# kubernetes-sigs/karpenter-provider-ibm-cloud

Hardware: AMD Instinct MI355X
Metric: pod×offering feasibility checks/sec + Solve latency (ms) at 100k pods, 1/2/4/8 GPU (higher is better)
Workload: dtype int64

## Files before the change

karpenter-provider-ibm-cloud_amd/csrc/batch_kernels.hip:

```cpp
#define GS_BATCH_KERNELS 1
#include <hip/hip_runtime.h>
#include <stdint.h>

#include "devutil.hpp"
#include "ffd_common.hpp"
#include "layout.hpp"

using namespace gsd;

#include "solve_kernels.hpp"
#include "queue_kernels.hpp"
#include "init_kernel.hpp"

extern "C" hipError_t gsk_init_batch(uint32_t trunc_lds_bytes) {
  return hipFuncSetAttribute((const void*)trunc_kernel_batch, hipFuncAttributeMaxDynamicSharedMemorySize,
                             (int)trunc_lds_bytes);
}

extern "C" uint32_t gsk_feas_lp(uint32_t W) {
#ifndef GS_K1_LPMAX
#define GS_K1_LPMAX 16
#endif
  if (GS_K1_LPMAX < 64 && W > GS_K1_LPMAX && W <= 32 && W * (64 / GS_K1_LPMAX) <= 256) W = GS_K1_LPMAX;
  uint32_t lp = 1;
  while (lp < W && lp < 64) lp <<= 1;
  return lp;
}

template <uint32_t LP>
static void launch_feas_batch_lp(const DevProblem* ds, uint32_t n, uint64_t max_pairs, hipStream_t s) {
  const uint64_t per_block = (BLOCK / 64) * (64 / LP);
  const uint32_t blocks = (uint32_t)((max_pairs + per_block - 1) / per_block);
  hipLaunchKernelGGL(feas_kernel_batch<LP>, dim3(blocks ? blocks : 1, n), dim3(BLOCK), 0, s, ds, 0u, 0u, ~0u);
}

extern "C" hipError_t gsk_feas_batch(const DevProblem* ds, uint32_t n, uint32_t lp, uint64_t max_cursors,
                                     uint64_t max_pairs, hipStream_t s) {
  if (!n || n > 65535) return hipErrorInvalidValue;
  const uint32_t cb = (uint32_t)((max_cursors + BLOCK - 1) / BLOCK);
  hipLaunchKernelGGL(feas_cursor_kernel_batch, dim3(cb ? cb : 1, n), dim3(BLOCK), 0, s, ds);
  switch (lp) {
    case 1: launch_feas_batch_lp<1>(ds, n, max_pairs, s); break;
    case 2: launch_feas_batch_lp<2>(ds, n, max_pairs, s); break;
    case 4: launch_feas_batch_lp<4>(ds, n, max_pairs, s); break;
    case 8: launch_feas_batch_lp<8>(ds, n, max_pairs, s); break;
    case 16: launch_feas_batch_lp<16>(ds, n, max_pairs, s); break;
    case 32: launch_feas_batch_lp<32>(ds, n, max_pairs, s); break;
    case 64: launch_feas_batch_lp<64>(ds, n, max_pairs, s); break;
    default: return hipErrorInvalidValue;
  }
  return hipGetLastError();
}

extern "C" hipError_t gsk_init_state_batch(const DevProblem* ds, uint32_t n, hipStream_t s) {
  if (!n || n > 65535) return hipErrorInvalidValue;
  hipLaunchKernelGGL(ffd_init_kernel_batch, dim3(8, n), dim3(256), 0, s, ds);
  return hipGetLastError();
}

extern "C" hipError_t gsk_queue_records_batch(const DevProblem* ds, uint32_t n, uint32_t max_pods, hipStream_t s) {
  if (!n || !max_pods) return hipSuccess;
  if (n > 65535) return hipErrorInvalidValue;
  const uint32_t blocks = (max_pods + 255) / 256;
  hipLaunchKernelGGL(queue_records_kernel_batch, dim3(blocks, n), dim3(256), 0, s, ds);
  hipLaunchKernelGGL(queue_runs_kernel_batch, dim3(blocks, n), dim3(256), 0, s, ds);
  return hipGetLastError();
}

extern "C" hipError_t gsk_trunc_batch(const DevProblem* ds, uint32_t n, uint32_t max_slots, uint32_t lds_bytes,
                                      hipStream_t s) {
  if (!n || n > 65535) return hipErrorInvalidValue;
  hipLaunchKernelGGL(trunc_kernel_batch, dim3(max_slots ? max_slots : 1, n), dim3(BLOCK), lds_bytes, s, ds, 0u, 0u);
  return hipGetLastError();
}

#define GSK_DECL(n, t)                                                                                      \
  extern "C" hipError_t gsk_ffdwb_launch_r##n##_t##t(const DevProblem* ds, uint32_t cnt, uint32_t wide, uint32_t lds, \
                                                     hipStream_t s);                                        \
  extern "C" hipError_t gsk_ffdwb_attr_r##n##_t##t(uint32_t lds_total, uint32_t* dyn_min);
#define GSK_DECL2(n) GSK_DECL(n, 0) GSK_DECL(n, 1)
GSK_DECL2(1) GSK_DECL2(2) GSK_DECL2(3) GSK_DECL2(4) GSK_DECL2(5) GSK_DECL2(6) GSK_DECL2(7) GSK_DECL2(8)
#undef GSK_DECL2
#undef GSK_DECL
static uint32_t g_ffdwb_dyn_max = 0;

extern "C" hipError_t gsk_init_ffdw_batch(uint32_t lds_total) {
  hipError_t e = hipSuccess;
  uint32_t dmin = 0;
#define GSK_ATTR(n, t) \
  if (hipError_t x = gsk_ffdwb_attr_r##n##_t##t(lds_total, &dmin); x != hipSuccess) e = x;
#define GSK_ATTR2(n) GSK_ATTR(n, 0) GSK_ATTR(n, 1)
  GSK_ATTR2(1) GSK_ATTR2(2) GSK_ATTR2(3) GSK_ATTR2(4) GSK_ATTR2(5) GSK_ATTR2(6) GSK_ATTR2(7) GSK_ATTR2(8)
#undef GSK_ATTR2
#undef GSK_ATTR
  g_ffdwb_dyn_max = dmin;
  return e;
}

extern "C" uint32_t gsk_ffdw_batch_dyn_lds_max(void) { return g_ffdwb_dyn_max; }

extern "C" hipError_t gsk_ffdw_batch(const DevProblem* ds, uint32_t n, uint32_t R, uint32_t topo, uint32_t wide,
                                     uint32_t lds, hipStream_t s) {
  if (!n || lds > g_ffdwb_dyn_max) return hipErrorInvalidConfiguration;
  switch (R * 2 + (topo ? 1 : 0)) {
#define GSK_CASE(k)                                                    \
  case 2 * k: return gsk_ffdwb_launch_r##k##_t0(ds, n, wide, lds, s); \
  case 2 * k + 1: return gsk_ffdwb_launch_r##k##_t1(ds, n, wide, lds, s);
    GSK_CASE(1) GSK_CASE(2) GSK_CASE(3) GSK_CASE(4) GSK_CASE(5) GSK_CASE(6) GSK_CASE(7) GSK_CASE(8)
#undef GSK_CASE
    default:
      return hipErrorInvalidValue;
  }
}


extern "C" __global__ __launch_bounds__(256) void sim_begin_kernel_batch(const DevProblem* __restrict__ ds,
                                                                         const uint32_t* __restrict__ blocks,
                                                                         uint32_t clear_overlays) {
  const DevProblem& d = ds[blockIdx.y];
  if (blockIdx.x == 0 && threadIdx.x == 0) *d.sim_next = 0;
  if (!clear_overlays) return;
  const size_t cells = (size_t)blocks[blockIdx.y] * d.ov_cap * (d.TGH ? d.TGH : 1u);
  for (size_t i = (size_t)blockIdx.x * 256 + threadIdx.x; i < cells; i += (size_t)gridDim.x * 256) d.ov_hn[i] = 0;
}

extern "C" hipError_t gsk_sim_begin_batch(const DevProblem* ds, const uint32_t* blocks, uint32_t n, uint32_t clear_overlays,
                                          hipStream_t s) {
  if (!n || n > 65535) return hipErrorInvalidValue;
  hipLaunchKernelGGL(sim_begin_kernel_batch, dim3(clear_overlays ? 8 : 1, n), dim3(256), 0, s, ds, blocks, clear_overlays);
  return hipGetLastError();
}

extern "C" hipError_t gsk_trunc_sims_batch(const DevProblem* ds, uint32_t n, uint32_t mv, uint32_t max_sims,
                                           uint32_t max_slots, uint32_t lds_bytes, hipStream_t s) {
  if (!n || n > 65535) return hipErrorInvalidValue;
  if (mv) {
    hipLaunchKernelGGL(trunc_kernel_batch, dim3(max_slots ? max_slots : 1, n), dim3(BLOCK), lds_bytes, s, ds, 1u, 0u);
    hipLaunchKernelGGL(sim_fix_kernel_batch, dim3((max_sims + BLOCK - 1) / BLOCK ? (max_sims + BLOCK - 1) / BLOCK : 1, n),
                       dim3(BLOCK), 0, s, ds);
  } else {
    hipLaunchKernelGGL(trunc_kernel_batch, dim3(max_sims ? max_sims : 1, n), dim3(BLOCK), lds_bytes, s, ds, 0u, 0u);
  }
  return hipGetLastError();
}

#define GSK_DECL(n, t)                                                                                                  \
  extern "C" hipError_t gsk_ffdsb_launch_r##n##_t##t(const DevProblem* ds, const uint32_t* blocks, uint32_t cnt,        \
                                                     uint32_t max_blocks, uint32_t nt, uint32_t lds, uint32_t ov_epoch, \
// ... 156 lines not shown
```

karpenter-provider-ibm-cloud_amd/csrc/capi.cpp:

```cpp
#include "ctx.hpp"

#include <set>

namespace gsc {

gs_status fail(gs_ctx* c, gs_status s, const std::string& m) {
  c->err = m;
  return s;
}

void upload_problem(gs_ctx* c, const SimPlan* sims, bool records) {
  auto& e = c->enc;
  auto& d = c->dp;
  c->plan.clear();
  c->plan_bytes = 0;
  c->free_all();
  std::memset(&d, 0, sizeof d);
  d.N = e.N;
  d.W = e.W;
  d.R = e.R;
  d.Z = e.Z;
  d.C = e.C;
  d.T = e.T;
  d.F = e.F;
  d.V = e.V;
  d.P = e.P;
  d.K = e.K;
  d.NT = e.NT;
  d.wk_slots = e.wk_slots;
  d.RQ = std::min<uint32_t>(e.R, 4);
  d.n_thr = (uint32_t)e.thr_val.size();
  if (sims) {
    d.max_claims = std::max<uint32_t>(sims->max_pods, 1);
  } else {
    const uint32_t other = gsk_ffd_lds_bytes(0, (uint32_t)e.thr_val.size(), 0, gsd::topo_lds_bytes(e.TGZ, e.ZS, e.TGH, e.n_lazy)) + 8;
    const uint32_t dyn = std::min(gsk_ffd_dyn_lds_max(), gsk_ffdw_dyn_lds_max());
    auto claims_fit = [&](uint32_t extra) {
      const uint32_t fit = dyn > other + extra ? (dyn - other - extra) / 23 : 0;
      return std::min<uint32_t>(std::min<uint32_t>(std::max<uint32_t>(e.P, 1), kMaxClaimsLds), fit);
    };
    d.max_claims = claims_fit(0);
    if (!d.max_claims) throw HipError{"topology / threshold state leaves no LDS for NodeClaims"};
    const bool wave_ok = !(c->cfg_flags & GS_CFG_BLOCK_SOLVE) && e.NN <= kWaveSolveMaxNodes;
    d.max_claims_wave = wave_ok ? claims_fit(gsd::wave_node_lds_bytes(e.NN)) : 0u;
    c->wave = d.max_claims_wave > 0;
  }
  c->upload(d.it_vid, e.it_vid);
  c->upload(d.it_dvid, e.it_dvid);
  d.it_key_unique = e.it_key_unique;
  d.any_mv = e.any_mv ? 1u : 0u;
  d.any_vol = e.any_vol ? 1u : 0u;
  c->upload(d.n_vol0, e.n_vol);
  c->alloc(d.n_vol, e.n_vol.size());
  c->upload(d.pod_vol, e.pod_vol);
  c->upload(d.pod_vfresh, e.pod_vfresh);
  c->upload(d.it_alloc, e.it_alloc);
  c->upload(d.it_cap, e.it_cap);
  c->upload(d.it_pair, e.it_pair);
  c->upload(d.it_prank, e.it_prank);
  c->upload(d.it_namerank, e.it_namerank);
  c->upload(d.rank_to_it, e.rank_to_it);
  c->upload(d.slot_set, e.slot_set);
  {
    std::vector<int64_t> tv = e.thr_val;
    tv.insert(tv.end(), 4, INT64_MAX);
    c->upload(d.thr_val, std::move(tv));
  }
  c->upload(d.thr_off, e.thr_off);
  {
    const uint32_t OW = std::max<uint32_t>(4, (e.W + 3) & ~3u);
    const size_t nrows = e.W ? e.thr_set.size() / e.W : 0;
    std::vector<uint64_t> ts(std::max<size_t>(nrows, 1) * OW, 0);
    for (size_t q = 0; q < nrows; q++)
      std::copy(e.thr_set.begin() + q * e.W, e.thr_set.begin() + (q + 1) * e.W, ts.begin() + q * OW);
    c->upload(d.thr_set, std::move(ts));
  }
  c->upload(d.fk_ival, e.fk_ival);
  c->upload(d.fk_isint, e.fk_isint);
  c->upload(d.tmpl, e.tmpl);
  c->upload(d.t_opts, e.t_opts);
  c->upload(d.t_limopts, e.t_limopts);
  c->upload(d.t_fk, e.t_fk);
  c->upload(d.pod_req, e.pod_req);
  c->upload(d.var_begin, e.var_begin);
  c->upload(d.var_count, e.var_count);
  c->upload(d.vars, e.vars);
  c->upload(d.itmask, e.itmask);
  c->upload(d.var_itclass, e.var_itclass);
  {
    std::vector<uint32_t> vp(std::max<uint32_t>(e.V, 1), 0);
    for (uint32_t v = 0; v < e.V; v++) vp[v] = e.vars[v].pod;
    c->upload(d.var_pod, std::move(vp));
  }
  c->upload(d.itclass_mask, e.itclass_mask);
  c->upload(d.fk_entries, e.fk_entries);
  c->upload(d.queue0, e.queue0);
  if (!sims) {
    c->alloc(d.qvars, std::max<uint32_t>(e.P, 1));
    c->alloc(d.qreqs, (size_t)std::max<uint32_t>(e.P, 1) * std::max<uint32_t>(e.R, 1));
    c->alloc(d.qcodes, (size_t)std::max<uint32_t>(e.P, 1) * 4);
    c->alloc(d.qrun, std::max<uint32_t>(e.P, 1));
  }
  d.NN = e.NN;
  d.TG = e.TG;
  d.TGH = e.TGH;
  d.TGZ = e.TGZ;
  d.ZS = e.ZS;
  d.NZV = e.NZV;
  d.dom_ct = e.dom_ct ? 1u : 0u;
  d.dom_np = e.dom_np ? 1u : 0u;
  d.zknown0 = e.zknown0;
  c->upload(d.tgroups, e.tgroups);
  c->upload(d.tg_list, e.tg_list);
  d.n_lazy = e.n_lazy;
  c->upload(d.lazy_slot, e.lazy_slot);
  c->upload(d.var_lz_off, e.var_lz_off);
  c->upload(d.lz_idx, e.lz_idx);
  c->upload(d.lz_mind, e.lz_mind);
  c->upload(d.zcnt0, e.zcnt0);
  c->upload(d.htot0, e.htot0);
  c->upload(d.zone_order, e.zone_order);
  c->upload(d.zone_cat, e.zone_cat);
  c->upload(d.hn0, e.hn0);
  if (sims && (e.TGH || e.TGZ) && e.NN) {
    std::vector<uint32_t> off(e.NN + 1, 0);
    for (uint32_t g = 0; g < e.TGZ; g++)
      for (uint32_t n = 0; n < e.NN; n++) off[n + 1] += e.zn_cnt[(size_t)g * e.NN + n] != 0;
    for (uint32_t g = 0; g < e.TGH; g++)
      for (uint32_t n = 0; n < e.NN; n++) off[n + 1] += e.hn0[(size_t)g * e.NN + n] != 0;
    for (uint32_t n = 0; n < e.NN; n++) off[n + 1] += off[n];
    std::vector<uint64_t> sp(std::max<uint32_t>(off[e.NN], 1));
    std::vector<uint32_t> fill(off.begin(), off.end() - 1);
    auto put = [&](uint32_t g, int32_t c, uint32_t n) { sp[fill[n]++] = (uint64_t)g << 32 | (uint32_t)c; };
    for (uint32_t g = 0; g < e.TGZ; g++)
      for (uint32_t n = 0; n < e.NN; n++)
        if (int32_t c = e.zn_cnt[(size_t)g * e.NN + n]) put(g, c, n);
    for (uint32_t g = 0; g < e.TGH; g++)
      for (uint32_t n = 0; n < e.NN; n++)
        if (int32_t c = e.hn0[(size_t)g * e.NN + n]) put(e.TGZ + g, c, n);
    c->upload(d.nsp_off, std::move(off));
    c->upload(d.nsp, std::move(sp));
  } else {
    d.nsp_off = nullptr;
    d.nsp = nullptr;
  }
  c->alloc(d.hn, e.hn0.size());
  c->upload(d.nodes0, e.nodes);
  c->upload(d.n_fk0, e.n_fk);
  c->alloc(d.nodes, sims ? 1 : std::max<uint32_t>(e.NN, 1));
  c->alloc(d.n_fk, sims ? 1 : e.n_fk.size());
  const size_t VT = (size_t)e.V * e.T, F1 = std::max<uint32_t>(e.F, 1), R1 = std::max<uint32_t>(e.R, 1);
  const size_t PA = sims ? sims->pods.size() : e.P;
  const size_t CA = sims ? sims->pods.size() : d.max_claims;
  const size_t NS = sims ? sims->evaluated.size() : 0;
  d.claim_cap = (uint32_t)CA;
  c->ch = false;
  d.OW = std::max<uint32_t>(4, (e.W + 3) & ~3u);
  c->alloc(d.rows, VT * d.OW);
  c->alloc(d.cheapest, VT);
  c->alloc(d.cheapest_key, VT);
  c->alloc(d.nfo, VT);
  c->alloc(d.fk_ok, VT);
  c->alloc(d.pair_cur, VT * R1);
  c->alloc(d.queue, PA);
  c->alloc(d.last_len, PA);
  c->alloc(d.last_epoch, PA);
  c->alloc(d.cur_var, PA);
  c->alloc(d.c_rec, CA);
  c->alloc(d.c_opts, CA * d.OW);
  c->alloc(d.c_fk, CA * F1);
  c->alloc(d.t_rem, (sims ? NS : 1) * e.T * R1);
  c->alloc(d.log, PA);
  c->alloc(d.c_sorted, sims ? 1 : CA);
  c->alloc(d.ctrl, 1);
  c->alloc(d.c_its, (sims ? NS : CA) * 60);
  c->alloc(d.c_nits, sims ? NS : CA);
  c->hc_bytes = 0;
  if (sims) {
    c->alloc_zero(d.hc, (size_t)std::max<uint32_t>(e.TGH, 1) * CA);
    c->hc_bytes = (size_t)std::max<uint32_t>(e.TGH, 1) * CA * sizeof(int32_t);
  } else {
    c->alloc(d.hc, (size_t)std::max<uint32_t>(e.TGH, 1) * CA);
  }
  if (sims) {
// ... 734 lines not shown
```

karpenter-provider-ibm-cloud_amd/csrc/ffd.hip:

```cpp
#include "ffd_block.hpp"

extern "C" uint32_t gsk_ffd_lds_bytes(uint32_t max_claims, uint32_t nthr, uint32_t nb_words,
                                      uint32_t topo_bytes) {
  const uint32_t thr = nthr + 4;
  const uint32_t base = (((23u * max_claims + 7u) & ~7u) + thr * 8u + nb_words * 4u + 7u) & ~7u;
  return base + topo_bytes;
}

static uint32_t g_ffd_dyn_max = 0;

template <uint32_t RR, bool SIM, bool TOPO = false, uint32_t NT = SIM ? FB_SIM : FB_MAX>
static hipError_t ffd_attr(uint32_t lds_total) {
  hipFuncAttributes a;
  hipError_t e = hipFuncGetAttributes(&a, (const void*)ffd_kernel<RR, SIM, NT, TOPO>);
  if (e != hipSuccess) return e;
  const uint32_t dyn = lds_total > a.sharedSizeBytes ? lds_total - (uint32_t)a.sharedSizeBytes : 0;
  if (!g_ffd_dyn_max || dyn < g_ffd_dyn_max) g_ffd_dyn_max = dyn;
  return hipFuncSetAttribute((const void*)ffd_kernel<RR, SIM, NT, TOPO>, hipFuncAttributeMaxDynamicSharedMemorySize,
                             (int)dyn);
}

template <uint32_t RR>
static hipError_t ffd_attr_all(uint32_t lds_total) {
  hipError_t e = hipSuccess;
  for (hipError_t x : {ffd_attr<RR, false>(lds_total), ffd_attr<RR, false, true>(lds_total), ffd_attr<RR, true>(lds_total),
                       ffd_attr<RR, true, false, FB_SIM_NARROW>(lds_total), ffd_attr<RR, true, true, FB_SIM>(lds_total),
                       ffd_attr<RR, true, true, FB_SIM_NARROW>(lds_total)})
    if (x != hipSuccess) e = x;
  return e;
}

extern "C" hipError_t gsk_init_ffd(uint32_t lds_total) {
  hipError_t e = hipSuccess;
  for (hipError_t x : {ffd_attr_all<1>(lds_total), ffd_attr_all<2>(lds_total), ffd_attr_all<3>(lds_total),
                       ffd_attr_all<4>(lds_total), ffd_attr_all<5>(lds_total), ffd_attr_all<6>(lds_total),
                       ffd_attr_all<7>(lds_total), ffd_attr_all<8>(lds_total)})
    if (x != hipSuccess) e = x;
  return e;
}

extern "C" uint32_t gsk_ffd_dyn_lds_max(void) { return g_ffd_dyn_max; }

template <uint32_t RR>
static hipError_t sim_occ(int* n, bool narrow, bool general, uint32_t lds) {
  if (general)
    return narrow ? hipOccupancyMaxActiveBlocksPerMultiprocessor(n, (const void*)ffd_kernel<RR, true, FB_SIM_NARROW, true>,
                                                                 FB_SIM_NARROW, lds)
                  : hipOccupancyMaxActiveBlocksPerMultiprocessor(n, (const void*)ffd_kernel<RR, true, FB_SIM, true>, FB_SIM, lds);
  return narrow ? hipOccupancyMaxActiveBlocksPerMultiprocessor(n, (const void*)ffd_kernel<RR, true, FB_SIM_NARROW, false>,
                                                               FB_SIM_NARROW, lds)
                : hipOccupancyMaxActiveBlocksPerMultiprocessor(n, (const void*)ffd_kernel<RR, true, FB_SIM, false>, FB_SIM, lds);
}

extern "C" uint32_t gsk_ffd_sim_blocks_per_cu(uint32_t R, uint32_t lds, uint32_t nt, uint32_t general) {
  int n = 0;
  hipError_t e = hipErrorInvalidValue;
  const bool narrow = nt == (uint32_t)FB_SIM_NARROW;
  switch (R) {
#define GSK_OCC(k) \
  case k: e = sim_occ<k>(&n, narrow, general != 0, lds); break;
    GSK_OCC(1) GSK_OCC(2) GSK_OCC(3) GSK_OCC(4) GSK_OCC(5) GSK_OCC(6) GSK_OCC(7) GSK_OCC(8)
#undef GSK_OCC
  }
  return e == hipSuccess && n > 0 ? (uint32_t)n : 1u;
}

extern "C" hipError_t gsk_ffd(const DevProblem* d, uint32_t blocks, hipStream_t s) {
  const uint32_t lds = gsk_ffd_lds_bytes(d->max_claims, d->n_thr, d->nb_words, topo_lds_bytes(d->TGZ, d->ZS, d->TGH, d->n_lazy)) +
                       (d->n_sims ? 8u * d->ovh_slots + (d->sim_lds ? 32u * d->max_claims : 0u) : 0u);
  if (lds > g_ffd_dyn_max) return hipErrorInvalidConfiguration;
  const bool sim = d->n_sims > 0;
  if (sim && d->sim_nt != (uint32_t)FB_SIM && d->sim_nt != (uint32_t)FB_SIM_NARROW) return hipErrorInvalidValue;
  const bool general = d->TG || d->any_mv || d->any_vol;
  const uint32_t shape = sim ? (d->sim_nt == (uint32_t)FB_SIM_NARROW ? 3u : 2u) + (general ? 2u : 0u) : (general ? 1u : 0u);
  switch (d->R * 8 + shape) {
#define GSK_CASE(n)                                                                                          \
  case 8 * n: hipLaunchKernelGGL((ffd_kernel<n, false, FB_MAX, false>), dim3(1), dim3(FB_MAX), lds, s, *d); break; \
  case 8 * n + 1: hipLaunchKernelGGL((ffd_kernel<n, false, FB_MAX, true>), dim3(1), dim3(FB_MAX), lds, s, *d); break; \
  case 8 * n + 2: hipLaunchKernelGGL((ffd_kernel<n, true, FB_SIM, false>), dim3(blocks), dim3(FB_SIM), lds, s, *d); break; \
  case 8 * n + 3:                                                                                            \
    hipLaunchKernelGGL((ffd_kernel<n, true, FB_SIM_NARROW, false>), dim3(blocks), dim3(FB_SIM_NARROW), lds, s, *d); \
    break;                                                                                                    \
  case 8 * n + 4: hipLaunchKernelGGL((ffd_kernel<n, true, FB_SIM, true>), dim3(blocks), dim3(FB_SIM), lds, s, *d); break; \
  case 8 * n + 5:                                                                                            \
    hipLaunchKernelGGL((ffd_kernel<n, true, FB_SIM_NARROW, true>), dim3(blocks), dim3(FB_SIM_NARROW), lds, s, *d); \
    break;
    GSK_CASE(1) GSK_CASE(2) GSK_CASE(3) GSK_CASE(4) GSK_CASE(5) GSK_CASE(6) GSK_CASE(7) GSK_CASE(8)
#undef GSK_CASE
    default:
      return hipErrorInvalidValue;
  }
  return hipGetLastError();
}

#include "queue_kernels.hpp"

extern "C" hipError_t gsk_queue_records(const DevProblem* d, hipStream_t s) {
  if (!d->P) return hipSuccess;
  hipLaunchKernelGGL(queue_records_kernel, dim3((d->P + 255) / 256), dim3(256), 0, s, *d);
  hipLaunchKernelGGL(queue_runs_kernel, dim3((d->P + 255) / 256), dim3(256), 0, s, *d);
  return hipGetLastError();
}
```

karpenter-provider-ibm-cloud_amd/csrc/ffd_common.hpp:

```cpp
#pragma once
#include <hip/hip_runtime.h>
#include <stdint.h>

#include "devutil.hpp"
#include "layout.hpp"

namespace gsd {
namespace {

struct Frame {
  int a, b, limit;
  int wb, wp;
  int uni;
};

typedef __attribute__((address_space(3))) uint32_t lds_u32;
typedef __attribute__((address_space(3))) uint16_t lds_u16;
typedef __attribute__((address_space(3))) Frame lds_frame;

__device__ __forceinline__ int bits_len(uint64_t x) { return x ? 64 - __clzll((long long)x) : 0; }

struct SplitAcc {
  uint16_t* sc;
  uint16_t* ord;
  __device__ __forceinline__ uint32_t key(int i) const { return sc[i]; }
  __device__ __forceinline__ void swap(int i, int j) const {
    uint16_t a = sc[i];
    sc[i] = sc[j];
    sc[j] = a;
    a = ord[i];
    ord[i] = ord[j];
    ord[j] = a;
  }
};
template <class U32>
struct PackedAccT {
  U32* so;
  __device__ __forceinline__ uint32_t key(int i) const { return so[i] & 0xFFFFu; }
  __device__ __forceinline__ void swap(int i, int j) const {
    const uint32_t a = so[i];
    so[i] = so[j];
    so[j] = a;
  }
};
using PackedAcc = PackedAccT<lds_u32>;

template <class Acc>
struct SeqSortT {
  Acc acc;
  __device__ bool less(int i, int j) const { return acc.key(i) < acc.key(j); }
  __device__ void swap(int i, int j) const { acc.swap(i, j); }
  __device__ void insertion_sort(int a, int b) const {
    for (int i = a + 1; i < b; i++)
      for (int j = i; j > a && less(j, j - 1); j--) swap(j, j - 1);
  }
  __device__ void sift_down(int lo, int hi, int first) const {
    int root = lo;
    for (;;) {
      int child = 2 * root + 1;
      if (child >= hi) return;
      if (child + 1 < hi && less(first + child, first + child + 1)) child++;
      if (!less(first + root, first + child)) return;
      swap(first + root, first + child);
      root = child;
    }
  }
  __device__ void heap_sort(int a, int b) const {
    int first = a, lo = 0, hi = b - a;
    for (int i = (hi - 1) / 2; i >= 0; i--) sift_down(i, hi, first);
    for (int i = hi - 1; i >= 0; i--) {
      swap(first, first + i);
      sift_down(lo, i, first);
    }
  }
  __device__ int partition(int a, int b, int pivot, bool* already) const {
    swap(a, pivot);
    int i = a + 1, j = b - 1;
    while (i <= j && less(i, a)) i++;
    while (i <= j && !less(j, a)) j--;
    if (i > j) {
      swap(j, a);
      *already = true;
      return j;
    }
    swap(i, j);
    i++;
    j--;
    for (;;) {
// ... 114 lines not shown
      j = median(i, j, k, &swaps);
    }
    *hint = swaps == 0 ? 1 : (swaps == 12 ? 2 : 0);
    return j;
  }
  __device__ void reverse_range(int a, int b) const {
    int i = a, j = b - 1;
    while (i < j) {
      swap(i, j);
      i++;
      j--;
    }
  }
  __device__ void pdq_frame(Frame f0) const {
    Frame st[32];
    int sp = 0;
    st[sp++] = f0;
    while (sp > 0) {
      Frame f = st[--sp];
      for (;;) {
        int length = f.b - f.a;
        if (length <= 12) {
          insertion_sort(f.a, f.b);
          break;
        }
        if (f.limit == 0) {
          heap_sort(f.a, f.b);
          break;
        }
        if (!f.wb) {
          break_patterns(f.a, f.b);
          f.limit--;
        }
        int hint;
        int pivot = choose_pivot(f.a, f.b, &hint);
        if (hint == 2) {
          reverse_range(f.a, f.b);
          pivot = (f.b - 1) - (pivot - f.a);
          hint = 1;
        }
        if (f.wb && f.wp && hint == 1) {
          if (partial_insertion_sort(f.a, f.b)) break;
        }
        if (f.a > 0 && !less(f.a - 1, pivot)) {
          f.a = partition_equal(f.a, f.b, pivot);
          continue;
        }
        bool already;
        int mid = partition(f.a, f.b, pivot, &already);
        f.wp = already;
        int leftLen = mid - f.a, rightLen = f.b - mid;
        int bal = length / 8;
        Frame child;
        if (leftLen < rightLen) {
          f.wb = leftLen >= bal;
          child = Frame{f.a, mid, f.limit, 1, 1};
          f.a = mid + 1;
        } else {
          f.wb = rightLen >= bal;
          child = Frame{mid + 1, f.b, f.limit, 1, 1};
          f.b = mid;
        }
        st[sp++] = f;
        f = child;
      }
    }
  }
};

__device__ __forceinline__ void wsync() {
  __builtin_amdgcn_fence(__ATOMIC_ACQ_REL, "wavefront");
  __builtin_amdgcn_wave_barrier();
}
template <bool G>
__device__ __forceinline__ void wsyncT() {
  if (G) __builtin_amdgcn_s_waitcnt(0);
  wsync();
}

__device__ __forceinline__ uint32_t rlane(uint32_t x, uint32_t i) {
  return (uint32_t)__builtin_amdgcn_readlane((int)x, (int)i);
}

__device__ __forceinline__ uint32_t ffs64(uint64_t m) { return (uint32_t)__ffsll((long long)m) - 1u; }


__device__ __forceinline__ uint32_t wlane(uint32_t v, int i, uint32_t x) {
  return (int)(threadIdx.x & 63u) == i ? x : v;
}
__device__ __forceinline__ uint32_t nth_bit(uint64_t m, uint32_t r) {
  uint32_t pos = 0;
#pragma unroll
  for (int w = 32; w >= 1; w >>= 1) {
    const uint32_t c = (uint32_t)__popcll(m & ((1ull << w) - 1ull));
    const bool up = r >= c;
    r = up ? r - c : r;
    m = up ? m >> w : m;
    pos += up ? (uint32_t)w : 0u;
  }
  return pos;
}
template <class U32, bool G>
struct PackedArr {
  U32* so;
  __device__ __forceinline__ uint32_t load(int i) const { return (uint32_t)so[i]; }
  __device__ __forceinline__ void store(int i, uint32_t v) const { so[i] = v; }
  __device__ __forceinline__ void heap_sort(int a, int b) const { SeqSortT<PackedAccT<U32>>{{so}}.heap_sort(a, b); }
  __device__ __forceinline__ void sync() const { wsyncT<G>(); }
};
template <class Arr>
struct RegSort {
  uint32_t v;
  uint32_t lane;
  int g;
  uint32_t prevk;

  __device__ __forceinline__ uint32_t key(int i) const { return rlane(v, (uint32_t)i) & 0xFFFFu; }
  __device__ __forceinline__ void swap(int i, int j) {
    const uint32_t x = rlane(v, (uint32_t)i), y = rlane(v, (uint32_t)j);
    v = wlane(v, i, y);
    v = wlane(v, j, x);
  }
  __device__ void insertion_sort(int a, int b) {
    const uint32_t k = v & 0xFFFFu;
    int r = a;
    for (int j = a; j < b; j++) {
      const uint32_t kj = key(j);
      r += (kj < k || (kj == k && j < (int)lane)) ? 1 : 0;
    }
    const bool in = (int)lane >= a && (int)lane < b;
    v = (uint32_t)__builtin_amdgcn_ds_permute((in ? r : (int)lane) * 4, (int)v);
  }
  __device__ void swap_misplaced(uint64_t lm, uint64_t rm) {
    const uint64_t me = 1ull << lane;
    const uint64_t below = me - 1ull;
    uint32_t partner = lane;
    if (lm & me) {
      const uint32_t r = (uint32_t)__popcll(lm & below);
      partner = nth_bit(rm, (uint32_t)__popcll(rm) - 1u - r);
    } else if (rm & me) {
      const uint32_t r = (uint32_t)__popcll(rm & ~below & ~me);
      partner = nth_bit(lm, r);
    }
    v = (uint32_t)__shfl((int)v, (int)partner);
  }
  __device__ int partition(int a, int b, int pivot, bool* already) {
    swap(a, pivot);
    const uint32_t p = key(a), k = v & 0xFFFFu;
    const bool inr = (int)lane > a && (int)lane < b;
    const bool lt = k < p;
    const int mid = a + (int)__popcll(__ballot(inr && lt));
    const bool inl = (int)lane > a && (int)lane <= mid;
    const uint64_t lm = __ballot(inl && !lt), rm = __ballot(inr && !inl && lt);
    if (lm) swap_misplaced(lm, rm);
    swap(mid, a);
    *already = lm == 0;
    return mid;
  }
  __device__ int partition_equal(int a, int b, int pivot) {
    swap(a, pivot);
    const uint32_t p = key(a), k = v & 0xFFFFu;
    const bool inr = (int)lane > a && (int)lane < b;
    const bool le = k <= p;
    const int mid = a + (int)__popcll(__ballot(inr && le));
    const bool inl = (int)lane > a && (int)lane <= mid;
    const uint64_t lm = __ballot(inl && !le), rm = __ballot(inr && !inl && le);
    if (lm) swap_misplaced(lm, rm);
    return mid + 1;
  }
  __device__ void reverse_range(int a, int b) {
    const bool in = (int)lane >= a && (int)lane < b;
    v = (uint32_t)__shfl((int)v, in ? a + b - 1 - (int)lane : (int)lane);
  }
  __device__ void rotate_up(int lo, int hi) {
    const uint32_t x = rlane(v, (uint32_t)hi);
    const bool in = (int)lane > lo && (int)lane <= hi;
    const uint32_t y = (uint32_t)__shfl((int)v, in ? (int)lane - 1 : (int)lane);
    v = (int)lane == lo ? x : y;
  }
  __device__ void rotate_down(int lo, int hi) {
    const uint32_t x = rlane(v, (uint32_t)lo);
    const bool in = (int)lane >= lo && (int)lane < hi;
    const uint32_t y = (uint32_t)__shfl((int)v, in ? (int)lane + 1 : (int)lane);
    v = (int)lane == hi ? x : y;
  }
  __device__ bool partial_insertion_sort(int a, int b) {
    int i = a + 1;
    for (int j = 0; j < 5; j++) {
      const uint32_t k = v & 0xFFFFu;
      const uint32_t pk = (uint32_t)__shfl((int)v, (int)lane - 1) & 0xFFFFu;
      const uint64_t inv = __ballot((int)lane >= i && (int)lane < b && k < pk);
      if (!inv) return true;
      i = (int)ffs64(inv);
      if (b - a < 50) return false;
      swap(i, i - 1);
      if (i - a >= 2) {
        const uint32_t x = key(i - 1);
        const uint64_t hm = __ballot((int)lane <= i - 2 && (v & 0xFFFFu) <= x);
        const int q = hm ? 63 - (int)__clzll((long long)hm) : -1;
        rotate_up(q + 1, i - 1);
      }
      if (b - i >= 2) {
        const uint32_t y = key(i);
        const uint64_t em = __ballot((int)lane > i && (int)lane < b && (v & 0xFFFFu) >= y);
        const int e = em ? (int)ffs64(em) : b;
        rotate_down(i, e - 1);
      }
    }
    return false;
  }
  __device__ void break_patterns(int a, int b) {
    const int length = b - a;
    if (length >= 8) {
      uint64_t r = (uint64_t)length;
      const uint64_t modulus = 1ull << bits_len((uint64_t)length);
      const int idx = a + (length / 4) * 2 - 1;
      for (int i = 0; i < 3; i++) {
        r ^= r << 13;
        r ^= r >> 7;
        r ^= r << 17;
        int other = (int)(r & (modulus - 1));
        if (other >= length) other -= length;
        swap(idx - 1 + i, a + other);
      }
    }
  }
  __device__ int choose_pivot(int a, int b, int* hint) const {
    const int l = b - a;
    int swaps = 0;
    int i = a + l / 4 * 1, j = a + l / 4 * 2, k = a + l / 4 * 3;
    auto med = [&](int x, int y, int z) {
      if (key(y) < key(x)) { swaps++; const int t = x; x = y; y = t; }
      if (key(z) < key(y)) { swaps++; const int t = y; y = z; z = t; }
      if (key(y) < key(x)) { swaps++; const int t = x; x = y; y = t; }
      return y;
    };
    if (l >= 8) {
      if (l >= 50) {
        i = med(i - 1, i, i + 1);
        j = med(j - 1, j, j + 1);
        k = med(k - 1, k, k + 1);
      }
      j = med(i, j, k);
    }
    *hint = swaps == 0 ? 1 : (swaps == 12 ? 2 : 0);
    return j;
  }
  __device__ void heap_sort(const Arr& arr, int a, int b) {
    if ((int)lane < b && (int)lane >= a) arr.store(g + (int)lane, v);
    arr.sync();
    if (lane == 0) arr.heap_sort(g + a, g + b);
    arr.sync();
    if ((int)lane < b && (int)lane >= a) v = arr.load(g + (int)lane);
    arr.sync();
  }
  __device__ void run(const Arr& arr, Frame f) {
    int a = f.a - g, b = f.b - g, limit = f.limit, wb = f.wb, wp = f.wp;
    uint32_t stk = 0;
    int sp = 0;
    for (;;) {
      for (;;) {
        a = __builtin_amdgcn_readfirstlane(a);
        b = __builtin_amdgcn_readfirstlane(b);
        limit = __builtin_amdgcn_readfirstlane(limit);
        wb = __builtin_amdgcn_readfirstlane(wb);
        wp = __builtin_amdgcn_readfirstlane(wp);
        const int length = b - a;
        if (length <= 12) {
          insertion_sort(a, b);
          break;
        }
        if (limit == 0) {
          heap_sort(arr, a, b);
          break;
        }
        if (!wb) {
          break_patterns(a, b);
          limit--;
        }
        int hint;
        int pivot = choose_pivot(a, b, &hint);
        if (hint == 2) {
          reverse_range(a, b);
          pivot = (b - 1) - (pivot - a);
          hint = 1;
        }
        if (wb && wp && hint == 1 && partial_insertion_sort(a, b)) break;
// ... 31 lines not shown
      const uint32_t e = rlane(stk, (uint32_t)sp);
      a = (int)(e & 0xFFu);
      b = (int)((e >> 8) & 0xFFu);
      limit = (int)((e >> 16) & 0xFFu);
      wb = (int)((e >> 24) & 1u);
      wp = (int)((e >> 25) & 1u);
    }
  }
};
template <class Arr>
__device__ __noinline__ void reg_pdq_frame(Arr arr, int fa, int fb, int limit, int wb, int wp) {
  fa = __builtin_amdgcn_readfirstlane(fa);
  fb = __builtin_amdgcn_readfirstlane(fb);
  limit = __builtin_amdgcn_readfirstlane(limit);
  wb = __builtin_amdgcn_readfirstlane(wb);
  wp = __builtin_amdgcn_readfirstlane(wp);
  const uint32_t lane = threadIdx.x & 63u;
  const int n = fb - fa;
  const uint32_t prevk = fa > 0 ? (uint32_t)__builtin_amdgcn_readfirstlane((int)arr.load(fa - 1)) & 0xFFFFu : 0u;
  RegSort<Arr> r{(int)lane < n ? arr.load(fa + (int)lane) : 0u, lane, fa, prevk};
  r.run(arr, Frame{fa, fb, limit, wb, wp, 0});
  if ((int)lane < n) arr.store(fa + (int)lane, r.v);
  arr.sync();
}

using SeqSort = SeqSortT<SplitAcc>;
using SeqSortP = SeqSortT<PackedAcc>;
using SeqSortPG = SeqSortT<PackedAccT<uint32_t>>;

__device__ __forceinline__ uint32_t thr_window(const int64_t* thr, uint32_t n, uint32_t m0, int64_t x) {
  uint32_t m = m0;
#pragma unroll
  for (uint32_t k = 0; k < 4; k++) {
    const int64_t vk = thr[m0 + k];
    m += (m0 + k < n && vk < x) ? 1u : 0u;
  }
  return m;
}

__device__ __forceinline__ uint32_t thr_search(const int64_t* thr, uint32_t n, uint32_t lo, int64_t x) {
  uint32_t hi = n;
  while (lo < hi) {
    const uint32_t mid = (lo + hi) >> 1;
    if (thr[mid] < x) lo = mid + 1;
    else hi = mid;
  }
  return lo;
}

template <class Acc>
__device__ __forceinline__ int pivot_hint_wave(const Acc& acc, int l, uint32_t lane) {
  const int i0 = l / 4 * 1, j0 = l / 4 * 2, k0 = l / 4 * 3;
  const int idx[9] = {i0 - 1, i0, i0 + 1, j0 - 1, j0, j0 + 1, k0 - 1, k0, k0 + 1};
  int mine = 0;
#pragma unroll
  for (int t = 0; t < 9; t++)
    if ((int)lane == t) mine = idx[t];
  const uint32_t kl = lane < 9 && (l >= 50 || lane % 3 == 1) ? acc.key(mine) : 0u;
  uint32_t key[9];
#pragma unroll
  for (int t = 0; t < 9; t++) key[t] = __builtin_amdgcn_readlane(kl, t);
  int swaps = 0;
  auto med = [&](uint32_t kx, uint32_t ky, uint32_t kz) {
    if (ky < kx) { swaps++; const uint32_t u = kx; kx = ky; ky = u; }
    if (kz < ky) { swaps++; const uint32_t u = ky; ky = kz; kz = u; }
    if (ky < kx) { swaps++; const uint32_t u = kx; kx = ky; ky = u; }
    return ky;
  };
  uint32_t ki = key[1], kj = key[4], kk = key[7];
  if (l >= 50) {
    ki = med(key[0], key[1], key[2]);
    kj = med(key[3], key[4], key[5]);
    kk = med(key[6], key[7], key[8]);
  }
  med(ki, kj, kk);
  return swaps == 0 ? 1 : (swaps == 12 ? 2 : 0);
}

template <class Pred>
__device__ __forceinline__ uint32_t wave_first(uint32_t lo, uint32_t hi, uint32_t lane, Pred pred) {
  while (hi - lo > 64) {
    const uint32_t step = (hi - lo + 63) / 64;
    const uint32_t k = lo + lane * step + step - 1;
    const uint64_t b = __ballot(k >= hi || pred(k));
    if (!b) return hi;
    const uint32_t i = (uint32_t)__ffsll((long long)b) - 1;
    lo = lo + i * step;
    hi = lo + step < hi ? lo + step : hi;
  }
  const uint32_t k = lo + lane;
  const uint64_t b = __ballot(k < hi && pred(k));
  return b ? lo + (uint32_t)__ffsll((long long)b) - 1 : hi;
}

__device__ __forceinline__ uint64_t phase_clock() {
#ifdef GS_FFD_PHASES
  return wall_clock64();
#else
  return 0;
#endif
}

typedef const __attribute__((address_space(4))) DevProblem* KArg;

__device__ __forceinline__ int64_t uniform_i64(int64_t x) {
  const uint32_t lo = __builtin_amdgcn_readfirstlane((uint32_t)x);
  const uint32_t hi = __builtin_amdgcn_readfirstlane((uint32_t)((uint64_t)x >> 32));
  return (int64_t)(((uint64_t)hi << 32) | lo);
}

__device__ __forceinline__ uint32_t qcode_floor(int64_t v) {
  if (v <= 0) return 0;
  const uint64_t x = (uint64_t)v;
  const uint32_t b = 64u - (uint32_t)__clzll((long long)x);
  if (b <= 10) return (uint32_t)x;
  const uint32_t s = b - 10;
  return 1024u + (s - 1) * 512u + (uint32_t)((x >> s) - 512u);
}
__device__ __forceinline__ uint32_t qcode_ceil(int64_t v) {
  if (v <= 0) return 0;
  const uint64_t x = (uint64_t)v;
  const uint32_t b = 64u - (uint32_t)__clzll((long long)x);
  if (b <= 10) return (uint32_t)x;
  const uint32_t s = b - 10;
  const uint32_t c = 1024u + (s - 1) * 512u + (uint32_t)((x >> s) - 512u);
  return c + ((x & ((1ull << s) - 1)) ? 1u : 0u);
}

__device__ __forceinline__ int64_t qcode_value(uint32_t c) {
  if (c < 1024u) return (int64_t)c;
  const uint32_t s = (c - 1024u) / 512u + 1u, m = (c - 1024u) % 512u + 512u;
  return (int64_t)((uint64_t)m << s);
}

__device__ __forceinline__ uint64_t pack_room(const int64_t* thr, const uint32_t* thoff, const uint32_t* cur,
                                              const int64_t* tot, uint32_t RQ) {
  uint64_t s = 0;
#pragma unroll
  for (uint32_t r = 0; r < 4; r++) {
    if (r >= RQ) break;
    const uint32_t o = thoff[r], n = thoff[r + 1] - o;
    const int64_t room = cur[r] < n ? thr[o + cur[r]] - tot[r] : 0;
    s |= (uint64_t)qcode_floor(room) << (16 * r);
  }
  return s;
}

template <class DP>
__device__ __forceinline__ uint64_t pack_slack(const DP& d, const int64_t* maxa, const int64_t* tot) {
  uint64_t s = 0;
#pragma unroll
  for (uint32_t r = 0; r < 4; r++) {
    if (r >= d.RQ) break;
    s |= (uint64_t)qcode_ceil(maxa[r] - tot[r]) << (16 * r);
  }
  return s;
}

template <class DP, class WordFn>
__device__ inline bool mv_ok(const DP& d, const TmplRec& tr, WordFn word) {
  for (uint32_t mm = tr.mv_mask; mm; mm &= mm - 1) {
    const uint32_t k = (uint32_t)__builtin_ctz(mm);
    const uint32_t need = tr.mv[k];
    uint32_t n = 0;
    if ((d.it_key_unique >> k) & 1) {
      for (uint32_t w = 0; w < d.W && n < need; w++) n += (uint32_t)__popcll(word(w));
    } else {
      const uint16_t* dv = d.it_dvid + (size_t)k * d.N;
      uint64_t s0 = 0, s1 = 0, s2 = 0, s3 = 0;
      for (uint32_t w = 0; w < d.W && n < need; w++)
        for (uint64_t m = word(w); m && n < need; m &= m - 1) {
          const uint32_t x = dv[w * 64 + (uint32_t)__builtin_ctzll(m)];
          const uint32_t q = x >> 6;
          const uint64_t bit = 1ull << (x & 63);
          const uint64_t cur = q == 0 ? s0 : q == 1 ? s1 : q == 2 ? s2 : s3;
          if (!(cur & bit)) {
            n++;
            s0 |= q == 0 ? bit : 0;
            s1 |= q == 1 ? bit : 0;
            s2 |= q == 2 ? bit : 0;
            s3 |= q == 3 ? bit : 0;
          }
        }
    }
    if (n < need) return false;
  }
  return true;
}

struct TopoS {
  uint64_t* known;
  int64_t* tmin;
  int32_t* zcnt;
  int32_t* htot;
  uint64_t* lazy;
  int32_t* lmind;
};
__device__ __forceinline__ TopoS topo_lds(char* base, uint32_t tgz, uint32_t zs, uint32_t tgh, uint32_t nl) {
  TopoS t;
  t.known = (uint64_t*)base;
  t.tmin = (int64_t*)(base + tgz * 8u);
  t.zcnt = (int32_t*)(base + tgz * 8u + (uint32_t)OWNMAX * 8u);
  t.htot = (int32_t*)(base + tgz * 8u + (uint32_t)OWNMAX * 8u + tgz * zs * 4u);
  t.lazy = (uint64_t*)(base + topo_lazy_off(tgz, zs, tgh));
  t.lmind = (int32_t*)(base + topo_lazy_off(tgz, zs, tgh) + ((nl + 63u) / 64u) * 8u);
  return t;
}

template <class DP>
__device__ __forceinline__ void topo_init(const DP& d, const TopoS& ts, uint64_t known0, uint32_t i, uint32_t stride) {
  for (uint32_t k = i; k < d.TGZ * d.ZS; k += stride) ts.zcnt[k] = d.zcnt0[k];
  for (uint32_t k = i; k < d.TGZ; k += stride) ts.known[k] = known0;
  for (uint32_t k = i; k < d.TGH; k += stride) ts.htot[k] = d.htot0[k];
  for (uint32_t k = i; k < (d.n_lazy + 63u) / 64u; k += stride) ts.lazy[k] = 0;
}
// ... 189 lines not shown
```

karpenter-provider-ibm-cloud_amd/csrc/ffd_wave.hpp:

```cpp
#pragma once
#include <hip/hip_runtime.h>
#include <stdint.h>

#include <type_traits>

#include "devutil.hpp"
#include "ffd_common.hpp"
#include "layout.hpp"

using namespace gsd;

namespace {

constexpr uint32_t VR_DW = sizeof(VarRec) / 4;
static_assert(VR_DW == 32, "VarRec is one dword per lane of a half wave");
static_assert(offsetof(VarRec, fk_begin) == 4 && offsetof(VarRec, fk_count) == 8 && offsetof(VarRec, ctb) == 12 &&
                  offsetof(VarRec, itmask_off) == 16 && offsetof(VarRec, zfull_off) == 48 &&
                  offsetof(VarRec, cfull_off) == 52 && offsetof(VarRec, zm) == 56 && offsetof(VarRec, cm) == 64 &&
                  offsetof(VarRec, tol) == 72 && offsetof(VarRec, tolt) == 80 && offsetof(VarRec, own_off) == 88 &&
                  offsetof(VarRec, own_n) == 92 && offsetof(VarRec, sel_off) == 96 && offsetof(VarRec, sel_n) == 100 &&
                  offsetof(VarRec, zs) == 104 && offsetof(VarRec, zn) == 112 &&
                  offsetof(VarRec, zflags) == 120 && offsetof(VarRec, vix) == 124,
              "VarRec dword map used by ffdw_kernel");
static_assert(offsetof(ClaimRec, maxa) == 128, "ClaimRec maxa after two 64-B lines");

constexpr uint32_t WREG = 4;
#ifndef GS_RING
#define GS_RING 16
#endif
constexpr uint32_t RING = GS_RING;
constexpr uint32_t RING_DW = 53;
constexpr uint32_t RING_CODES = 48;
constexpr uint32_t RING_QRUN = 52;
constexpr uint32_t WQ = 32;
constexpr uint32_t WQ_DW = 16;
enum : uint32_t { WQ_LOG = 1, WQ_FA = 2, WQ_STOP = 3, WQ_NFA = 4 };
constexpr uint32_t SPIN_MAX = 1u << 26;
constexpr uint64_t SWAR_HI = 0x8000800080008000ull;
enum : uint32_t { MOD_NONE = 0, MOD_INC = 1, MOD_APPEND = 2 };
#ifndef GS_WAVE_SEQ
#define GS_WAVE_SEQ 32
#endif

#if defined(GS_FFD_TL) && defined(GS_CAT_SEG)
#define TLW(k)                                         \
  do {                                                 \
    const uint64_t t_ = __builtin_amdgcn_s_memtime();  \
    ptl[k] += t_ - tl_last;                            \
    tl_last = t_;                                      \
  } while (0)
#elif defined(GS_FFD_TL)
#define TLW(k)                                         \
  do {                                                 \
    const uint64_t t_ = __builtin_amdgcn_s_memtime();  \
    tl[k] += t_ - tl_last;                             \
    tl_last = t_;                                      \
  } while (0)
#else
#define TLW(k) \
  do {         \
  } while (0)
#endif

typedef __attribute__((address_space(3))) uint32_t lds_u32;
__device__ __forceinline__ uint32_t vld(const uint32_t* p) { return *(const volatile lds_u32*)(const lds_u32*)p; }
__device__ __forceinline__ void vst(uint32_t* p, uint32_t x) { *(volatile lds_u32*)(lds_u32*)p = x; }

#ifdef GS_WAVE_BATCH
__device__ __forceinline__ KArg karg() {
  const uint64_t ds = *(const __attribute__((address_space(4))) uint64_t*)__builtin_amdgcn_kernarg_segment_ptr();
  KArg p = (KArg)(ds + (uint64_t)__builtin_amdgcn_readfirstlane(blockIdx.x) * sizeof(DevProblem));
  asm volatile("" : "+s"(p));
  return p;
}
#else
__device__ __forceinline__ KArg karg() {
  KArg p = (KArg)__builtin_amdgcn_kernarg_segment_ptr();
  asm volatile("" : "+s"(p));
  return p;
}
#endif
__device__ __forceinline__ uint32_t fresh(uint32_t x) {
  asm volatile("" : "+v"(x));
  return x;
}

__device__ __forceinline__ uint64_t shfl_u64(uint64_t x, uint32_t src) {
  const uint32_t lo = (uint32_t)__shfl((int)(uint32_t)x, (int)src), hi = (uint32_t)__shfl((int)(uint32_t)(x >> 32), (int)src);
  return ((uint64_t)hi << 32) | lo;
}
__device__ __forceinline__ uint64_t wave_max_u64(uint64_t x) {
  for (int m = 32; m >= 1; m >>= 1) {
    const uint64_t y = shfl_xor_u64(x, m);
    x = y > x ? y : x;
  }
  return x;
}

__device__ __forceinline__ bool swar_ge(uint64_t a, uint64_t b) {
  return (((a | SWAR_HI) - b) & SWAR_HI) == SWAR_HI;
}
__device__ __forceinline__ uint64_t swar_max(uint64_t a, uint64_t b) {
  const uint64_t m = ((((a | SWAR_HI) - b) & SWAR_HI) >> 15) * 0xFFFFull;
  return (a & m) | (b & ~m);
}
__device__ __forceinline__ uint64_t wave_swar_max(uint64_t x) {
  for (int m = 32; m >= 1; m >>= 1) x = swar_max(x, shfl_xor_u64(x, m));
  return x;
}

__device__ __forceinline__ uint32_t dpp_max_step(uint32_t x, uint32_t y) { return x > y ? x : y; }
__device__ __forceinline__ uint32_t wave_max_dpp(uint32_t x) {
  x = dpp_max_step(x, (uint32_t)__builtin_amdgcn_update_dpp(0, (int)x, 0x111, 0xF, 0xF, true));
  x = dpp_max_step(x, (uint32_t)__builtin_amdgcn_update_dpp(0, (int)x, 0x112, 0xF, 0xF, true));
  x = dpp_max_step(x, (uint32_t)__builtin_amdgcn_update_dpp(0, (int)x, 0x114, 0xF, 0xF, true));
  x = dpp_max_step(x, (uint32_t)__builtin_amdgcn_update_dpp(0, (int)x, 0x118, 0xF, 0xF, true));
  x = dpp_max_step(x, (uint32_t)__builtin_amdgcn_update_dpp(0, (int)x, 0x142, 0xA, 0xF, false));
  x = dpp_max_step(x, (uint32_t)__builtin_amdgcn_update_dpp(0, (int)x, 0x143, 0xC, 0xF, false));
  return rlane(x, 63u);
}

struct KnownPart {
  int mid;
  int flags;
};
template <class U32, bool G>
__device__ __noinline__ KnownPart known_partition(U32* so, int n, int pivot, int x) {
  n = __builtin_amdgcn_readfirstlane(n);
  pivot = __builtin_amdgcn_readfirstlane(pivot);
  x = __builtin_amdgcn_readfirstlane(x);
  const uint32_t lane = threadIdx.x & 63u;
  auto key = [&](int i) { return (uint32_t)so[i] & 0xFFFFu; };
  auto swap = [&](int i, int j) {
    const uint32_t a = so[i];
    so[i] = so[j];
    so[j] = a;
  };
  bool already_, luni_, runi_;
  bool* already = &already_;
  bool* luni = &luni_;
  bool* runi = &runi_;
  if (lane == 0) swap(0, pivot);
  wsyncT<G>();
  const uint32_t p = key(0);
  const int e0 = x >= 1 && x < n ? x : -1;
  const int e1 = pivot != x && pivot >= 1 && pivot < n ? pivot : -1;
  auto in_e = [&](int k) { return k == e0 || k == e1; };
  auto skip_e = [&](int k) {
    k += in_e(k) ? 1 : 0;
    k += in_e(k) ? 1 : 0;
    return k;
  };
  const int step = (n - 1 + 63) / 64;
  const int q = skip_e(1 + (int)lane * step);
  const bool qv = 1 + (int)lane * step < n && q < n;
  const uint64_t m1 = __ballot(qv && key(qv ? q : 0) >= p);
  int lo, hi;
  if (m1) {
    const int l = (int)ffs64(m1);
    lo = l == 0 ? 1 : (int)rlane((uint32_t)q, (uint32_t)(l - 1)) + 1;
    hi = (int)rlane((uint32_t)q, (uint32_t)l);
  } else {
    const int lv = 63 - (int)__clzll((long long)__ballot(qv));
    lo = (int)rlane((uint32_t)q, (uint32_t)lv) + 1;
    hi = n;
  }
  int t = hi;
  for (int base = lo; base < hi; base += 64) {
    const int k = base + (int)lane;
    const bool ok = k < hi && k < n && !in_e(k);
    const uint64_t m2 = __ballot(ok && key(ok ? k : 0) >= p);
    if (m2) {
      t = base + (int)ffs64(m2);
      break;
    }
  }
  const uint32_t k0 = e0 >= 0 ? key(e0) : 0u, k1 = e1 >= 0 ? key(e1) : 0u;
  const int e_lt = (e0 >= 0 && k0 < p ? 1 : 0) + (e1 >= 0 && k1 < p ? 1 : 0);
  const int e_before_t = (e0 >= 1 && e0 < t ? 1 : 0) + (e1 >= 1 && e1 < t ? 1 : 0);
  const int mid = (t - 1) - e_before_t + e_lt;
  {
    auto prev_out = [&](int k) {
      k -= in_e(k) ? 1 : 0;
      k -= in_e(k) ? 1 : 0;
      return k;
    };
    uint32_t amin = 0xFFFFu, amax = 0, bmin = 0xFFFFu, bmax = 0;
    const int f1 = skip_e(1), l1 = prev_out(t - 1);
    if (f1 < t && l1 >= 1 && f1 <= l1) {
      amin = key(f1);
      amax = key(l1);
    }
    const int l2 = prev_out(n - 1);
    if (t < n && l2 >= t) {
      bmin = key(t);
      bmax = key(l2);
    }
    if (e0 >= 0) {
      if (k0 < p) {
        amin = k0 < amin ? k0 : amin;
        amax = k0 > amax ? k0 : amax;
      } else {
        bmin = k0 < bmin ? k0 : bmin;
        bmax = k0 > bmax ? k0 : bmax;
      }
    }
    if (e1 >= 0) {
      if (k1 < p) {
        amin = k1 < amin ? k1 : amin;
        amax = k1 > amax ? k1 : amax;
      } else {
        bmin = k1 < bmin ? k1 : bmin;
        bmax = k1 > bmax ? k1 : bmax;
      }
    }
    *luni = amin >= amax;
    *runi = bmin >= bmax;
  }
  int pos = -1;
  bool left = false, right = false;
  if (lane < 4) {
    pos = t + (int)lane;
    left = pos <= mid && pos < n && !in_e(pos);
  } else if (lane < 8) {
    pos = mid + 1 + (int)(lane - 4);
    right = pos < t && pos < n && !in_e(pos);
  } else if (lane == 8 || lane == 9) {
    pos = lane == 8 ? e0 : e1;
    if (pos >= 1) {
      const uint32_t ke = lane == 8 ? k0 : k1;
      left = pos <= mid && ke >= p;
      right = pos > mid && ke < p;
    }
  }
  const uint64_t lm = __ballot(left), rm = __ballot(right);
  const uint32_t s = (uint32_t)__popcll(lm);
  if (s) {
    const uint64_t fl = lm | rm;
    int r = 0;
    for (uint64_t mm = fl; mm; mm &= mm - 1) {
      const uint32_t j = ffs64(mm);
      const int pj = (int)rlane((uint32_t)pos, j);
      const bool lj = (lm >> j) & 1ull;
      r += (left && lj && pj < pos) || (right && !lj && pj > pos) ? 1 : 0;
    }
    int partner = (int)lane;
    for (uint64_t mm = fl; mm; mm &= mm - 1) {
      const uint32_t j = ffs64(mm);
      const int rj = (int)rlane((uint32_t)r, j);
      const bool lj = (lm >> j) & 1ull;
      if (((left && !lj) || (right && lj)) && rj == r) partner = (int)j;
    }
    const uint32_t wv = (left || right) ? (uint32_t)so[pos] : 0u;
    const uint32_t pv = (uint32_t)__shfl((int)wv, partner);
    wsyncT<G>();
    if (left || right) so[pos] = pv;
    wsyncT<G>();
  }
  if (lane == 0) swap(mid, 0);
  wsyncT<G>();
  *already = s == 0;
  return KnownPart{mid, (already_ ? 1 : 0) | (luni_ ? 2 : 0) | (runi_ ? 4 : 0)};
}

template <int SEQ, class U32 = lds_u32, class U16 = lds_u16, bool G = false, bool KNOWN = false>
struct WaveSort {
  static_assert(SEQ >= 12, "ranges <= 12 must reach Go's insertion sort");
  U32* so;
  U16* scr;
  lds_frame* stk;
  uint32_t lane, half;

  __device__ __forceinline__ uint32_t key(int i) const { return so[i] & 0xFFFFu; }
  __device__ __forceinline__ void swap(int i, int j) const {
    const uint32_t a = so[i];
    so[i] = so[j];
    so[j] = a;
  }
#ifndef GS_SORT_RW
#define GS_SORT_RW 4
#endif
  static constexpr int RW = GS_SORT_RW;
  template <class Pred>
  __device__ uint32_t count(int lo, int hi, Pred pred) const {
    uint32_t c = 0;
    for (int base = lo; base < hi; base += 64 * RW) {
      bool in[RW];
#pragma unroll
      for (int u = 0; u < RW; u++) {
        const int k = base + u * 64 + (int)lane;
        in[u] = k < hi && pred(k);
      }
#pragma unroll
      for (int u = 0; u < RW; u++) c += (uint32_t)__popcll(__ballot(in[u]));
    }
    return c;
  }
  template <class Pred>
  __device__ uint32_t compact(int lo, int hi, bool desc, U16* out, Pred pred) const {
    uint32_t total = 0;
    const int n = hi - lo;
    for (int base = 0; base < n; base += 64 * RW) {
      bool in[RW];
#pragma unroll
      for (int u = 0; u < RW; u++) {
        const int idx = base + u * 64 + (int)lane;
        in[u] = idx < n && pred(desc ? hi - 1 - idx : lo + idx);
      }
#pragma unroll
      for (int u = 0; u < RW; u++) {
        const int idx = base + u * 64 + (int)lane;
        const uint64_t m = __ballot(in[u]);
        if (in[u]) out[total + (uint32_t)__popcll(m & ((1ull << lane) - 1ull))] = (uint16_t)(desc ? hi - 1 - idx : lo + idx);
        total += (uint32_t)__popcll(m);
      }
    }
    wsyncT<G>();
    return total;
  }
  __device__ void swap_lists(uint32_t s) const {
    for (uint32_t k = lane; k < s; k += 64) {
      const int x = scr[k], y = scr[half + k];
      const uint32_t a = so[x], b = so[y];
      wsyncT<G>();
      so[x] = b;
      so[y] = a;
    }
    wsyncT<G>();
  }
  template <bool LE>
  __device__ uint32_t count_split(int lo, int hi, uint32_t p, bool* lo_uni, bool* hi_uni, uint64_t* mk) const {
    constexpr int RC = 2 * RW;
    uint32_t c = 0, amax = 0, anot = 0, bmax = 0, bnot = 0;
    uint64_t mine = 0;
    for (int base = lo; base < hi; base += 64 * RC) {
      uint32_t kk[RC];
#pragma unroll
      for (int u = 0; u < RC; u++) {
        const int k = base + u * 64 + (int)lane;
        kk[u] = key(k < hi ? k : hi - 1);
      }
#pragma unroll
      for (int u = 0; u < RC; u++) {
        const int k = base + u * 64 + (int)lane;
        const bool valid = k < hi;
        const bool in = valid && (LE ? kk[u] <= p : kk[u] < p);
        const bool out = valid && !in;
        const uint64_t bi = __ballot(in);
        c += (uint32_t)__popcll(bi);
        mine = lane == (uint32_t)((base - lo) / 64 + u) ? bi : mine;
        const uint32_t nk = 0xFFFFu - kk[u];
        amax = in && kk[u] > amax ? kk[u] : amax;
        anot = in && nk > anot ? nk : anot;
        bmax = out && kk[u] > bmax ? kk[u] : bmax;
        bnot = out && nk > bnot ? nk : bnot;
      }
    }
    *mk = mine;
    amax = wave_max_dpp(amax);
    anot = wave_max_dpp(anot);
    bmax = wave_max_dpp(bmax);
    bnot = wave_max_dpp(bnot);
    *lo_uni = c == 0 || amax == 0xFFFFu - anot;
    *hi_uni = c == (uint32_t)(hi - lo) || bmax == 0xFFFFu - bnot;
    return c;
  }
  static constexpr int MASK_MAX = 64 * 64;
  __device__ uint32_t lists_from_masks(int lo, uint32_t nl, uint32_t n, uint64_t mk) const {
    const uint32_t x0 = lane * 64u;
    const uint64_t valid = x0 >= n ? 0ull : (n - x0 >= 64u ? ~0ull : ((1ull << (n - x0)) - 1ull));
    const uint64_t left = x0 >= nl ? 0ull : (nl - x0 >= 64u ? ~0ull : ((1ull << (nl - x0)) - 1ull));
    const uint64_t lm = ~mk & left & valid, rm = mk & ~left & valid;
    const uint32_t lc = (uint32_t)__popcll(lm), rc = (uint32_t)__popcll(rm);
    uint32_t x = lc | rc << 16;
    x += (uint32_t)__builtin_amdgcn_update_dpp(0, (int)x, 0x111, 0xF, 0xF, true);
    x += (uint32_t)__builtin_amdgcn_update_dpp(0, (int)x, 0x112, 0xF, 0xF, true);
    x += (uint32_t)__builtin_amdgcn_update_dpp(0, (int)x, 0x114, 0xF, 0xF, true);
    x += (uint32_t)__builtin_amdgcn_update_dpp(0, (int)x, 0x118, 0xF, 0xF, true);
    x += (uint32_t)__builtin_amdgcn_update_dpp(0, (int)x, 0x142, 0xA, 0xF, false);
    x += (uint32_t)__builtin_amdgcn_update_dpp(0, (int)x, 0x143, 0xC, 0xF, false);
    const uint32_t tot = rlane(x, 63u);
    const uint32_t lpre = x & 0xFFFFu;
    const uint32_t rsuf = (tot >> 16) - (x >> 16) + rc;
    const uint32_t total = tot & 0xFFFFu;
    uint32_t k = lpre - lc;
    for (uint64_t m = lm; m; m &= m - 1) scr[k++] = (uint16_t)(lo + (int)(x0 + ffs64(m)));
    k = rsuf - rc;
    for (uint64_t m = rm; m;) {
      const uint32_t bit = 63u - (uint32_t)__clzll((long long)m);
      scr[half + k++] = (uint16_t)(lo + (int)(x0 + bit));
      m &= ~(1ull << bit);
    }
    wsyncT<G>();
    return total;
  }
#ifdef GS_SORT_TL2
#define PTL(k)                                                                  \
  do {                                                                          \
    const uint64_t n_ = __builtin_amdgcn_s_memtime();                           \
    if (lane == 0 && stl) stl[8 + (k)] += n_ - p_last;                          \
    p_last = n_;                                                                \
  } while (0)
#else
#define PTL(k) \
  do {         \
  } while (0)
#endif
  __device__ int partition(int a, int b, int pivot, bool* already, bool* luni, bool* runi) const {
#ifdef GS_SORT_TL2
    uint64_t p_last = __builtin_amdgcn_s_memtime();
#endif
    if (lane == 0) swap(a, pivot);
    wsyncT<G>();
    const uint32_t p = key(a);
    PTL(0);
    uint64_t mk;
    const int mid = a + (int)count_split<false>(a + 1, b, p, luni, runi, &mk);
    PTL(1);
    uint32_t s;
    if (b - a - 1 <= MASK_MAX) {
      s = lists_from_masks(a + 1, (uint32_t)(mid - a), (uint32_t)(b - a - 1), mk);
    } else {
      s = compact(a + 1, mid + 1, false, scr, [&](int k) { return key(k) >= p; });
      compact(mid + 1, b, true, scr + half, [&](int k) { return key(k) < p; });
    }
    PTL(2);
    swap_lists(s);
    if (lane == 0) swap(mid, a);
    wsyncT<G>();
    PTL(3);
    *already = s == 0;
    return mid;
  }
  __device__ int partition_known(int n, int pivot, int x, bool* already, bool* luni, bool* runi) const;
  __device__ int partition_equal(int a, int b, int pivot, bool* runi) const {
    if (lane == 0) swap(a, pivot);
    wsyncT<G>();
    const uint32_t p = key(a);
    bool luni;
    uint64_t mk;
    const int mid = a + (int)count_split<true>(a + 1, b, p, &luni, runi, &mk);
    uint32_t s;
    if (b - a - 1 <= MASK_MAX) {
      s = lists_from_masks(a + 1, (uint32_t)(mid - a), (uint32_t)(b - a - 1), mk);
    } else {
      s = compact(a + 1, mid + 1, false, scr, [&](int k) { return key(k) > p; });
      compact(mid + 1, b, true, scr + half, [&](int k) { return key(k) <= p; });
    }
    swap_lists(s);
    return mid + 1;
  }
  __device__ void rotate(int lo, int hi, bool left) const {
    if (hi <= lo) return;
    const uint32_t x = so[left ? lo : hi];
    wsyncT<G>();
    constexpr int RU = 4;
    if (left) {
      for (int base = lo; base < hi; base += 64 * RU) {
        uint32_t v[RU];
#pragma unroll
        for (int u = 0; u < RU; u++) {
          const int k = base + u * 64 + (int)lane;
          v[u] = k < hi ? so[k + 1] : 0u;
        }
        wsyncT<G>();
#pragma unroll
        for (int u = 0; u < RU; u++) {
          const int k = base + u * 64 + (int)lane;
          if (k < hi) so[k] = v[u];
        }
        wsyncT<G>();
      }
      if (lane == 0) so[hi] = x;
    } else {
      for (int top = hi - 1; top >= lo; top -= 64 * RU) {
        uint32_t v[RU];
#pragma unroll
        for (int u = 0; u < RU; u++) {
          const int k = top - u * 64 - (int)lane;
          v[u] = k >= lo ? so[k] : 0u;
        }
        wsyncT<G>();
#pragma unroll
        for (int u = 0; u < RU; u++) {
          const int k = top - u * 64 - (int)lane;
          if (k >= lo) so[k + 1] = v[u];
        }
        wsyncT<G>();
      }
      if (lane == 0) so[lo] = x;
    }
    wsyncT<G>();
  }
  __device__ int first_inversion(int from, int b) const {
    for (int base = from; base < b; base += 64 * RW) {
      bool hit[RW];
      uint32_t kc[RW], kp[RW];
#pragma unroll
      for (int u = 0; u < RW; u++) {
        const int k = base + u * 64 + (int)lane, kk = k < b ? k : b - 1;
        kc[u] = key(kk);
        kp[u] = key(kk - 1);
      }
#pragma unroll
      for (int u = 0; u < RW; u++) hit[u] = base + u * 64 + (int)lane < b && kc[u] < kp[u];
#pragma unroll
      for (int u = 0; u < RW; u++) {
        const uint64_t m = __ballot(hit[u]);
        if (m) return base + u * 64 + (int)ffs64(m);
      }
    }
    return b;
  }
  __device__ bool partial_insertion_sort(int a, int b) const {
    int i = a + 1;
    for (int j = 0; j < 5; j++) {
      i = first_inversion(i, b);
      if (i == b) return true;
      if (b - a < 50) return false;
      if (lane == 0) swap(i, i - 1);
      wsyncT<G>();
      if (i - a >= 2) {
        const uint32_t x = key(i - 1);
        int q = -1;
        for (int top = i - 2; top >= 0; top -= 64) {
          const int k = top - (int)lane;
          const uint64_t m = __ballot(k >= 0 && key(k) <= x);
          if (m) {
            q = top - (int)ffs64(m);
            break;
          }
        }
        rotate(q + 1, i - 1, false);
      }
      if (b - i >= 2) {
        const uint32_t y = key(i);
        int q = b;
        for (int base = i + 1; base < b; base += 64) {
          const int k = base + (int)lane;
          const uint64_t m = __ballot(k < b && key(k) >= y);
          if (m) {
            q = base + (int)ffs64(m);
            break;
          }
        }
        rotate(i, q - 1, true);
      }
    }
    return false;
  }
  __device__ void reverse_range(int a, int b) const {
    const int n = (b - a) / 2;
    for (int k = (int)lane; k < n; k += 64) {
      const uint32_t x = so[a + k], y = so[b - 1 - k];
      wsyncT<G>();
      so[a + k] = y;
      so[b - 1 - k] = x;
    }
    wsyncT<G>();
  }
#ifdef GS_SORT_TL
  uint64_t* stl = nullptr;
#define STL(k)                                                     \
  do {                                                             \
    const uint64_t now_ = __builtin_amdgcn_s_memtime();            \
    if (lane == 0 && stl) stl[k] += now_ - t_last_;                \
    t_last_ = now_;                                                \
  } while (0)
#else
#define STL(k) \
  do {         \
  } while (0)
#endif
  __device__ __forceinline__ void pdqsort_body(int n, int x = -1) const {
#ifdef GS_SORT_TL
    uint64_t t_last_ = __builtin_amdgcn_s_memtime();
#endif
    const SeqSortT<PackedAccT<U32>> seq{{so}};
    if (n <= 64) {
      reg_pdq_frame(PackedArr<U32, G>{so}, 0, n, bits_len((uint64_t)n), 1, 1);
      return;
    }
    int sp = 0;
    uint32_t stk_ab = 0, stk_fl = 0;
    Frame f{0, n, bits_len((uint64_t)n), 1, 1};
    bool pristine = KNOWN && x >= 0;
    for (;;) {
      for (;;) {
        f.a = __builtin_amdgcn_readfirstlane(f.a);
        f.b = __builtin_amdgcn_readfirstlane(f.b);
        f.limit = __builtin_amdgcn_readfirstlane(f.limit);
        f.wb = __builtin_amdgcn_readfirstlane(f.wb);
        f.wp = __builtin_amdgcn_readfirstlane(f.wp);
        f.uni = __builtin_amdgcn_readfirstlane(f.uni);
        const int length = f.b - f.a;
        STL(6);
        if (length <= 64) {
          reg_pdq_frame(PackedArr<U32, G>{so}, f.a, f.b, f.limit, f.wb, f.wp);
          STL(0);
          break;
        }
        if (f.limit == 0) {
          if (lane == 0) seq.heap_sort(f.a, f.b);
          wsyncT<G>();
          STL(0);
          break;
        }
        if (!f.wb) {
          if (lane == 0) seq.break_patterns(f.a, f.b);
          wsyncT<G>();
          f.limit--;
          STL(0);
        }
        if (f.uni) {
          const int pivot = f.a + length / 4 * 2;
          if (f.wb && f.wp) break;
          const bool eq = f.a > 0 && !(key(f.a - 1) < key(pivot));
          if (lane == 0) swap(f.a, pivot);
          wsyncT<G>();
          if (eq) {
            f.a = f.b;
            STL(1);
            continue;
// ... 165 lines not shown
  const uint32_t nd_off = (tg_off + topo_lds_bytes(d.TGZ, d.ZS, d.TGH, d.n_lazy) + 7u) & ~7u;
  uint64_t* s_nslk = (uint64_t*)((char*)lds64 + nd_off);
  uint64_t* s_nrm = (uint64_t*)((char*)lds64 + nd_off + d.NN * 8u);
  uint8_t* s_nflag = (uint8_t*)((char*)lds64 + nd_off + d.NN * 16u);
  const int64_t* thr = s_thr;
  const uint64_t* slot = s_slot;

  for (uint32_t i = tid; i < nthr + 4; i += 128) s_thr[i] = i < nthr ? d.thr_val[i] : INT64_MAX;
  for (uint32_t i = tid; i < d.Z * d.C * W; i += 128) s_slot[i] = d.slot_set[i];
  if (tid <= R) s_thoff[tid] = d.thr_off[tid];
  for (uint32_t t = tid; t < T; t += 128) {
    s_tzm[t] = d.tmpl[t].zm;
    s_tcm[t] = d.tmpl[t].cm;
  }
  if (TOPO) topo_init(d, ts, d.zknown0, tid, 128);
  for (uint32_t n = tid; n < d.NN; n += 128) {
    const NodeRec& nr = d.nodes0[n];
    int64_t sl[RR];
#pragma unroll
    for (uint32_t r = 0; r < RR; r++) sl[r] = nr.avail[r] - nr.req[r];
    uint64_t a = 0, b = 0;
    bool plain = nr.ok && nr.taints == 0;
#pragma unroll
    for (uint32_t r = 0; r < RR; r++) {
      if (r < 4 && r < d.RQ) {
        a |= (uint64_t)qcode_ceil(sl[r]) << (16 * r);
        b |= (uint64_t)qcode_floor(sl[r]) << (16 * r);
      }
      if (r >= 4) plain = plain && sl[r] >= 0;
    }
    s_nslk[n] = a;
    s_nrm[n] = b;
    s_nflag[n] = plain ? 1u : 0u;
  }
  if (tid < RING) s_ring_seq[tid] = 0;
  if (tid < 4) s_ctl[tid] = 0;
  __syncthreads();

  if (wave == 1) {
    const uint32_t* qv_dw = (const uint32_t*)d.qvars;
    const uint32_t* qr_dw = (const uint32_t*)d.qreqs;
    uint32_t k_fill = 0, head = 0, idle = 0, beat = 0;
    for (;;) {
      bool busy = false, stop = false;
      const uint32_t tail = __builtin_amdgcn_readfirstlane(vld(&s_ctl[1]));
      while (head != tail) {
        const uint32_t x = lane < WQ_DW ? vld(&s_wq[head % WQ][lane]) : 0u;
        const uint32_t type = rlane(x, 0), idx = rlane(x, 1), tgt = rlane(x, 4);
        const uint32_t rlo = (uint32_t)__shfl((int)x, (int)(5 + 2 * (lane & 3))),
                       rhi = (uint32_t)__shfl((int)x, (int)(6 + 2 * (lane & 3)));
        if (type == WQ_STOP) {
          stop = true;
        } else {
          if (lane == 0) d.log[idx] = LogRec{rlane(x, 2), rlane(x, 3), type == WQ_NFA ? tgt | 0x80000000u : tgt, 0};
          const uint64_t a = (uint64_t)rlo | ((uint64_t)rhi << 32);
          if (type == WQ_FA && lane < R && lane < 4 && a)
            atomicAdd((unsigned long long*)&d.c_rec[tgt].tot_lo[lane], (unsigned long long)a);
          if (type == WQ_NFA && lane < R && lane < 4 && a)
            atomicAdd((unsigned long long*)&d.nodes[tgt].req[lane], (unsigned long long)a);
        }
        head++;
        busy = true;
      }
      if (busy) {
        __builtin_amdgcn_s_waitcnt(0x0F70);
        wsyncT<CH>();
        if (lane == 0) vst(&s_ctl[2], head);
      }
      if (stop) break;
      const uint32_t sq = __builtin_amdgcn_readfirstlane(vld(&s_ctl[0]));
      const uint32_t lim = P < sq + RING ? P : sq + RING;
      if (k_fill < lim) {
        constexpr uint32_t KB = 8;
        const uint32_t n = lim - k_fill < KB ? lim - k_fill : KB;
        uint32_t val[KB];
#pragma unroll
        for (uint32_t i = 0; i < KB; i++) {
          const size_t k = k_fill + i;
          val[i] = 0;
          if (i < n) {
            if (lane < VR_DW) val[i] = qv_dw[k * VR_DW + lane];
            else if (lane < 32 + 2 * R) val[i] = qr_dw[k * 2 * R + (lane - 32)];
            else if (lane >= RING_CODES && lane < RING_CODES + 4) val[i] = d.qcodes[k * 4 + (lane - RING_CODES)];
            else if (lane == RING_QRUN) val[i] = d.qrun[k];
          }
        }
#pragma unroll
        for (uint32_t i = 0; i < KB; i++)
          if (i < n && lane < RING_DW) s_ring[(k_fill + i) % RING][lane] = val[i];
        wsyncT<CH>();
#pragma unroll
        for (uint32_t i = 0; i < KB; i++)
          if (i < n && lane == 0) vst(&s_ring_seq[(k_fill + i) % RING], k_fill + i + 1);
        k_fill += n;
        busy = true;
      }
      const uint32_t hb = __builtin_amdgcn_readfirstlane(vld(&s_ctl[3]));
      if (busy || hb != beat) {
        idle = 0;
        beat = hb;
      } else {
        __builtin_amdgcn_s_sleep(1);
        if (++idle > SPIN_MAX) break;
      }
    }
    return;
  }

  using U32 = std::conditional_t<CH, uint32_t, lds_u32>;
  using U16 = std::conditional_t<CH, uint16_t, lds_u16>;
  const WaveSort<GS_WAVE_SEQ, U32, U16, CH> ws{(U32*)s_so, (U16*)s_scr, (lds_frame*)s_stk, lane, MC / 2};
  const PackedAccT<U32> acc{(U32*)s_so};
  uint32_t wq_tail = 0;
  uint32_t wq_seen = 0;
  uint32_t hint = 0;
  bool hint_ok = false;
  uint64_t hint_tolt = 0;
  int64_t hint_rq = 0;
  uint32_t nhint = 0;
  bool nhint_ok = false;
  uint64_t nhint_tol = 0;
  int64_t hint_nrq = 0;
  bool chan_err = false;
  auto post = [&](uint32_t type, uint32_t idx, uint32_t pod, uint32_t var, uint32_t tgt, uint32_t rqd_) {
    if (wq_tail - wq_seen >= WQ) {
      for (uint32_t spin = 0;; spin++) {
        wq_seen = __builtin_amdgcn_readfirstlane(vld(&s_ctl[2]));
        if (wq_tail - wq_seen < WQ) break;
        __builtin_amdgcn_s_sleep(1);
        if (spin > SPIN_MAX) {
          chan_err = true;
          break;
        }
      }
    }
    const uint32_t x = lane == 0 ? type : lane == 1 ? idx : lane == 2 ? pod : lane == 3 ? var : lane == 4 ? tgt : rqd_;
    const bool rqw = (type == WQ_FA || type == WQ_NFA) && lane >= 32 && lane < 40;
    if (lane < 5 || rqw) s_wq[wq_tail % WQ][lane < 5 ? lane : lane - 27] = x;
    wsyncT<CH>();
    if (lane == 0) vst(&s_ctl[1], wq_tail + 1);
    wq_tail++;
  };
  auto drain = [&]() {
    for (uint32_t spin = 0; __builtin_amdgcn_readfirstlane(vld(&s_ctl[2])) != wq_tail; spin++) {
      __builtin_amdgcn_s_sleep(1);
      if (spin > SPIN_MAX) {
        chan_err = true;
        break;
      }
    }
  };

  auto emit = [&](uint32_t type, uint32_t idx, uint32_t pod, uint32_t var, uint32_t tgt, uint32_t rqd_, int64_t rql) {
    if (false) {
      post(type, idx, pod, var, tgt, rqd_);
      return;
    }
    const auto& KD = *karg();
    if (lane == 0) KD.log[idx] = LogRec{pod, var, type == WQ_NFA ? tgt | 0x80000000u : tgt, 0};
    if ((type == WQ_FA || type == WQ_NFA) && lane < R && lane < 4 && rql != 0) {
      unsigned long long* a = type == WQ_FA ? (unsigned long long*)&KD.c_rec[tgt].tot_lo[lane]
                                            : (unsigned long long*)&KD.nodes[tgt].req[lane];
      atomicAdd(a, (unsigned long long)rql);
    }
  };

  uint32_t qhead = 0, qlen = P, epoch = 1, M = 0, modkind = MOD_NONE, modpos = 0, nlog = 0, status = 0;
  bool wrapped = false;
  uint64_t pops = 0;
  enum { C_GEN = 0, C_FAST, C_CAND, C_FULL, C_NEV, C_NPRE, C_FA, C_ALG,
         C_RPODS, C_RENTER, C_RX_PIVOT, C_RX_WIN, C_RX_SPEC, C_RX_SCAN, C_RX_XC, C_RBATCH, C_RBPODS };
  uint64_t ctr = 0;
#define CTR(k, x) (ctr += lane == (k) ? (uint64_t)(x) : 0ull)
  const uint64_t max_pops = ((uint64_t)(d.V - d.P) + 2) * (uint64_t)P + P + 16;

#ifdef GS_FFD_TL
#ifdef GS_CAT_SEG
  uint64_t ptl[8] = {0, 0, 0, 0, 0, 0, 0, 0}, n_cat = 0;
#endif
  uint64_t tl[8] = {0, 0, 0, 0, 0, 0, 0, 0}, tl_last = __builtin_amdgcn_s_memtime();
  uint64_t n_fsum = 0, n_xns = 0, n_xb = 0, n_xwin = 0, n_nonsimple = 0, n_rot = 0, n_rotlen = 0, n_gen_cyc = 0;
#endif
  uint32_t pf_x = 0, pf_seq = 0;
#ifdef GS_RUN_TL
  uint64_t run_cyc = 0;
#endif
#ifdef GS_CAT_TL
  uint64_t cat_cyc = 0, cat_n = 0, cat_t = __builtin_amdgcn_s_memtime();
  uint32_t cat_k = 7;
#define CAT(k) (cat_k = (k))
#else
#define CAT(k) ((void)0)
#endif
  bool run_prev = false;
  uint32_t run_rec = 0;
  for (;;) {
    TLW(7);
#ifdef GS_CAT_TL
    {
      const uint64_t t_ = __builtin_amdgcn_s_memtime();
      cat_cyc += lane == cat_k ? t_ - cat_t : 0ull;
      cat_n += lane == cat_k && cat_k != 0 ? 1ull : 0ull;
      cat_t = t_;
#if defined(GS_FFD_TL) && defined(GS_CAT_SEG)
      if (cat_k == GS_CAT_SEG) {
        n_cat++;
#pragma unroll
        for (int q = 0; q < 8; q++) tl[q] += ptl[q];
      }
#pragma unroll
      for (int q = 0; q < 8; q++) ptl[q] = 0;
#endif
      cat_k = 7;
    }
#endif
    if (status) break;
    if (pops > max_pops) {
      status = 2;
      break;
    }
    if (qlen == 0) break;
    if (!TOPO && !WIDE && run_prev && !wrapped && modkind == MOD_INC && M >= 50 &&
        (d.NN == 0 || (nhint_ok && nhint >= d.NN))) {
      run_prev = false;
      auto same_spec = [&](uint32_t x) {
        return __ballot(lane >= 1 && lane < RING_QRUN && lane != VR_DW - 1 && x != run_rec) == 0;
      };
      if (__builtin_amdgcn_readfirstlane(pf_seq) == qhead + 1 && same_spec(pf_x)) {
        const uint64_t r_tolt = (uint64_t)rlane(run_rec, 20) | ((uint64_t)rlane(run_rec, 21) << 32);
        const uint64_t r_rqq = (uint64_t)rlane(run_rec, RING_CODES) | ((uint64_t)rlane(run_rec, RING_CODES + 1) << 32);
        const uint64_t r_rqc = (uint64_t)rlane(run_rec, RING_CODES + 2) | ((uint64_t)rlane(run_rec, RING_CODES + 3) << 32);
        int64_t r_rq = 0;
        {
          const uint32_t lo = (uint32_t)__shfl((int)run_rec, (int)(32 + 2 * (lane & 7))),
                         hi = (uint32_t)__shfl((int)run_rec, (int)(33 + 2 * (lane & 7)));
          if (lane < RR) r_rq = (int64_t)(((uint64_t)hi << 32) | lo);
        }
        uint32_t base = modpos;
        uint32_t wpos = base + lane;
        bool valid = wpos < M;
        uint32_t ow = 0;
        uint64_t wsl = 0, wrm = 0;
        uint32_t wtok = 0;
        auto load_window = [&]() {
          wpos = base + lane;
          valid = wpos < M;
          ow = valid ? (uint32_t)s_so[wpos] : 0xFFFFu;
          wsl = wrm = 0;
          wtok = 0;
          if (valid) {
            const uint32_t je = ow >> 16;
            wsl = s_slk[je];
            wrm = s_rm[je];
            wtok = (uint32_t)((r_tolt >> (T > 1 ? (uint32_t)s_tmpl[je] : 0u)) & 1u);
          }
        };
        load_window();
        uint32_t lf = 0;
        bool dirty = false;
        CTR(C_RENTER, 1);
        CAT(0);
#ifdef GS_RUN_TL
        const uint64_t rt0 = __builtin_amdgcn_s_memtime();
#endif
        for (;;) {
          const uint32_t x = rlane(ow, lf) & 0xFFFFu;
          const bool ptouch = pivot_touched(MOD_INC, modpos, M);
          const uint64_t b = ptouch ? 0ull : __ballot(lane > lf && (ow & 0xFFFFu) >= x);
          const uint32_t eo = b ? ffs64(b) : 64u;
          if (!b) {
            CTR(ptouch ? C_RX_PIVOT : C_RX_WIN, 1);
            wsyncT<CH>();
            if (dirty && valid) {
              s_so[wpos] = ow;
              s_slk[ow >> 16] = wsl;
              s_rm[ow >> 16] = wrm;
            }
            wsyncT<CH>();
            dirty = false;
            const uint32_t e2 = wave_first(modpos + 1, M, lane, [&](uint32_t k) { return acc.key(k) >= x; });
            if (e2 > modpos + 1) {
              if (ptouch && pivot_hint_wave(acc, (int)M, lane) != 1) break;
              CTR(C_FAST, 1);
              ws.rotate((int)modpos, (int)e2 - 1, true);
              if (modpos < hint && e2 - 1 >= hint) hint--;
            }
            base = modpos;
            load_window();
            lf = 0;
          } else if (eo > lf + 1) {
            CTR(C_FAST, 1);
            auto rot = [&](uint32_t y) -> uint32_t {
              const uint32_t sh = (uint32_t)__builtin_amdgcn_update_dpp(0, (int)y, 0x130, 0xF, 0xF, false);
              const uint32_t y0 = rlane(y, lf);
              return lane + 1 == eo ? y0 : (lane >= lf && lane + 1 < eo) ? sh : y;
            };
            ow = rot(ow);
            wsl = ((uint64_t)rot((uint32_t)(wsl >> 32)) << 32) | rot((uint32_t)wsl);
            wrm = ((uint64_t)rot((uint32_t)(wrm >> 32)) << 32) | rot((uint32_t)wrm);
            wtok = rot(wtok);
            dirty = true;
          }
          modkind = MOD_NONE;
          if (!(__builtin_amdgcn_readfirstlane(pf_seq) == qhead + 1 && same_spec(pf_x))) {
            CTR(C_RX_SPEC, 1);
            break;
          }
          if (pops + 1 > max_pops || qhead + 1 == P) break;
          const uint32_t lo = modpos - base;
          const bool lp = (lane >= lo) & valid & (wtok != 0) & swar_ge(wsl, r_rqq);
          const uint64_t lpb = __ballot(lp), fab = __ballot(lp & swar_ge(wrm, r_rqc));
          if (!lpb) {
            CTR(C_RX_SCAN, 1);
            break;
          }
          uint32_t fl = ffs64(lpb);
          bool xwin = false;
          uint64_t x_nx[WREG] = {0, 0, 0, 0};
          int64_t x_tot[RR], x_ma[RR];
          uint32_t x_mrow[RR];
          uint64_t x_zm = 0;
#pragma unroll
          for (uint32_t r = 0; r < RR; r++) {
            x_tot[r] = 0;
            x_ma[r] = 0;
            x_mrow[r] = 0;
          }
          const uint64_t vzm = (uint64_t)rlane(run_rec, 14) | ((uint64_t)rlane(run_rec, 15) << 32);
          const uint64_t vcm = (uint64_t)rlane(run_rec, 16) | ((uint64_t)rlane(run_rec, 17) << 32);
          auto RQV = [&](uint32_t r) -> int64_t {
            return (int64_t)((uint64_t)rlane(run_rec, 32 + 2 * r) | ((uint64_t)rlane(run_rec, 33 + 2 * r) << 32));
          };
          if (!(fab & 1ull << fl)) {
            if (rlane(run_rec, 2) != 0) {
              CTR(C_RX_SCAN, 1);
              break;
            }
            const uint32_t mfl = fab ? ffs64(fab) : 64u;
            const uint64_t ex = lpb & ~fab & (mfl == 64 ? ~0ull : ((1ull << mfl) - 1ull));
            const auto& KD = *karg();
            const uint32_t pvx = rlane(pf_x, VR_DW - 1);
            bool feas = false;
            if ((ex >> lane) & 1) {
              const uint32_t j = ow >> 16;
              const uint32_t t = T > 1 ? (uint32_t)s_tmpl[j] : 0u;
              const ClaimRec* cr = KD.c_rec + j;
              uint32_t cur[RR];
#pragma unroll
              for (uint32_t r = 0; r < RR; r++) x_ma[r] = cr->maxa[r];
              uint64_t x_cm;
              {
                const uint4* q = (const uint4*)cr;
                const uint4 h0 = q[0], h1 = q[1], h2 = q[2], h3 = q[3];
                const int64_t tl4[4] = {(int64_t)(((uint64_t)h0.y << 32) | h0.x), (int64_t)(((uint64_t)h0.w << 32) | h0.z),
                                        (int64_t)(((uint64_t)h1.y << 32) | h1.x), (int64_t)(((uint64_t)h1.w << 32) | h1.z)};
                const uint32_t cl[4] = {h2.x & 0xFFFFu, h2.x >> 16, h2.y & 0xFFFFu, h2.y >> 16};
                x_zm = ((uint64_t)h2.w << 32) | h2.z;
                x_cm = ((uint64_t)h3.y << 32) | h3.x;
#pragma unroll
                for (uint32_t r = 0; r < RR; r++) {
                  x_tot[r] = r < 4 ? tl4[r] : cr->tot_hi[r - 4];
                  cur[r] = r < 4 ? cl[r] : cr->thr_hi[r - 4];
                }
              }
              const uint64_t* row = KD.rows + ((size_t)pvx * T + t) * OW;
              const uint64_t* opts = KD.c_opts + (size_t)j * OW;
              {
                const uint4* oq = (const uint4*)opts;
                const uint4* rq4 = (const uint4*)row;
                const uint4 o0 = oq[0], o1 = oq[1], r0 = rq4[0], r1 = rq4[1];
                const uint64_t a[4] = {(((uint64_t)o0.y << 32) | o0.x) & (((uint64_t)r0.y << 32) | r0.x),
                                       (((uint64_t)o0.w << 32) | o0.z) & (((uint64_t)r0.w << 32) | r0.z),
                                       (((uint64_t)o1.y << 32) | o1.x) & (((uint64_t)r1.y << 32) | r1.x),
                                       (((uint64_t)o1.w << 32) | o1.z) & (((uint64_t)r1.w << 32) | r1.z)};
#pragma unroll
                for (uint32_t w = 0; w < WREG; w++) x_nx[w] = w < W ? a[w] : 0;
              }
              const uint64_t G = grid_of(x_zm & vzm, x_cm & vcm, KD.Z, KD.C);
              const uint64_t Gt = grid_of(s_tzm[t] & vzm, s_tcm[t] & vcm, KD.Z, KD.C);
              uint32_t mm[RR];
#pragma unroll
              for (uint32_t r = 0; r < RR; r++) {
                const uint32_t o = s_thoff[r], n = s_thoff[r + 1] - o;
                mm[r] = thr_window(thr + o, n, cur[r], x_tot[r] + RQV(r));
              }
#pragma unroll
              for (uint32_t r = 0; r < RR; r++) {
                const uint32_t o = s_thoff[r], n = s_thoff[r + 1] - o;
                if (mm[r] == cur[r] + 4 && mm[r] < n) mm[r] = thr_search(thr + o, n, mm[r], x_tot[r] + RQV(r));
                x_mrow[r] = o + r + mm[r];
              }
#pragma unroll
              for (uint32_t r = 0; r < RR; r++) {
                if (mm[r] != cur[r]) {
                  const uint4* tq = (const uint4*)(KD.thr_set + (size_t)x_mrow[r] * OW);
                  const uint4 t0 = tq[0], t1 = tq[1];
                  x_nx[0] &= ((uint64_t)t0.y << 32) | t0.x;
                  x_nx[1] &= ((uint64_t)t0.w << 32) | t0.z;
                  x_nx[2] &= ((uint64_t)t1.y << 32) | t1.x;
                  x_nx[3] &= ((uint64_t)t1.w << 32) | t1.z;
                }
              }
              if (G != Gt) {
                uint64_t off[WREG] = {};
                for (uint64_t gm = G; gm; gm &= gm - 1) {
                  const uint32_t g = ffs64(gm);
#pragma unroll
                  for (uint32_t w = 0; w < WREG; w++)
                    if (w < W) off[w] |= slot[g * W + w];
                }
#pragma unroll
                for (uint32_t w = 0; w < WREG; w++) x_nx[w] &= off[w];
              }
              uint64_t accw = 0;
#pragma unroll
              for (uint32_t w = 0; w < WREG; w++) accw |= x_nx[w];
              feas = accw != 0;
            }
            CTR(C_FULL, __popcll(ex));
            CTR(C_RX_XC, 1);
            const uint64_t fm = __ballot(feas);
            if (fm) {
              fl = ffs64(fm);
              xwin = true;
            } else if (fab) {
              fl = mfl;
            } else {
              CTR(C_RX_SCAN, 1);
              break;
            }
          }
          const uint32_t e = rlane(ow, fl);
          if ((e & 0xFFFFu) == 0xFFFFu) {
            status = 3;
            break;
          }
          const uint32_t x_rec = pf_x;
          const uint32_t pp = rlane(x_rec, 0), pv = rlane(x_rec, VR_DW - 1);
          wsyncT<CH>();
          if (lane == 0) vst(&s_ctl[0], qhead + 1);
          qhead++;
          qlen--;
          pops++;
          if ((pops & 15) == 0 && lane == 0) vst(&s_ctl[3], (uint32_t)pops);
          pf_seq = vld(&s_ring_seq[qhead % RING]);
          pf_x = lane < RING_DW ? vld(&s_ring[qhead % RING][lane]) : 0u;
          if (xwin) {
            const auto& KD = *karg();
            const uint32_t vctb = rlane(run_rec, 3);
            if (lane == fl) {
              const uint32_t j = ow >> 16;
              ClaimRec* cr = KD.c_rec + j;
              uint64_t* opts = KD.c_opts + (size_t)j * OW;
#pragma unroll
              for (uint32_t w = 0; w < WREG; w++)
                if (w < W) opts[w] = x_nx[w];
              int64_t nt[RR];
              uint32_t cu[RR];
#pragma unroll
              for (uint32_t r = 0; r < RR; r++) {
                nt[r] = x_tot[r] + RQV(r);
                cu[r] = x_mrow[r] - s_thoff[r] - r;
                cr->tot(r) = nt[r];
                cr->thr(r) = (uint16_t)cu[r];
              }
              wsl = pack_slack(d, x_ma, nt);
              wrm = pack_room(thr, s_thoff, cu, nt, KD.RQ);
              s_slk[j] = wsl;
              s_rm[j] = wrm;
              cr->zm = x_zm & vzm;
              cr->cm &= vcm;
              cr->ctb &= vctb;
              ow = e + 1u;
            }
            dirty = true;
            const uint32_t f = base + fl;
            wsyncT<CH>();
            emit(WQ_LOG, nlog, pp, pv, e >> 16, 0, 0);
            nlog++;
            CTR(C_CAND, M - modpos < 64 ? M - modpos : 64);
            CTR(C_ALG, f + 1);
            CTR(C_NPRE, d.NN);
            CTR(C_RPODS, 1);
#ifdef GS_CAT_TL
            cat_n += lane == 0 ? 1ull : 0ull;
#endif
            hint = f;
            modkind = MOD_INC;
            modpos = f;
            lf = fl;
            continue;
          }
          const uint64_t rm = ((uint64_t)rlane((uint32_t)(wrm >> 32), fl) << 32) | rlane((uint32_t)wrm, fl);
          const uint64_t sl = ((uint64_t)rlane((uint32_t)(wsl >> 32), fl) << 32) | rlane((uint32_t)wsl, fl);
          uint32_t c_rm = 0, c_sl = 0;
          if (lane < d.RQ) {
            const uint32_t sh = 16 * lane;
            c_rm = qcode_floor(qcode_value((uint32_t)(rm >> sh) & 0xFFFFu) - r_rq);
            c_sl = qcode_ceil(qcode_value((uint32_t)(sl >> sh) & 0xFFFFu) - r_rq);
          }
          uint32_t prm = (lane & 1u) ? c_rm << 16 : c_rm, psl = (lane & 1u) ? c_sl << 16 : c_sl;
          prm |= (uint32_t)__builtin_amdgcn_update_dpp(0, (int)prm, 0xB1, 0xF, 0xF, false);
          psl |= (uint32_t)__builtin_amdgcn_update_dpp(0, (int)psl, 0xB1, 0xF, 0xF, false);
          const uint32_t hrm = (uint32_t)__builtin_amdgcn_update_dpp(0, (int)prm, 0x102, 0xF, 0xF, false);
          const uint32_t hsl = (uint32_t)__builtin_amdgcn_update_dpp(0, (int)psl, 0x102, 0xF, 0xF, false);
          const uint64_t nrm = (uint64_t)rlane(prm, 0) | ((uint64_t)rlane(hrm, 0) << 32);
          const uint64_t nsl = (uint64_t)rlane(psl, 0) | ((uint64_t)rlane(hsl, 0) << 32);
          if (lane == fl) {
            wrm = nrm;
            wsl = nsl;
            ow = e + 1u;
          }
          dirty = true;
          const uint32_t f = base + fl;
          emit(WQ_FA, nlog, pp, pv, e >> 16, run_rec, r_rq);
          nlog++;
          CTR(C_CAND, M - modpos < 64 ? M - modpos : 64);
          CTR(C_FA, 1);
          CTR(C_ALG, f + 1);
          CTR(C_NPRE, d.NN);
          CTR(C_RPODS, 1);
#ifdef GS_CAT_TL
          cat_n += lane == 0 ? 1ull : 0ull;
#endif
          hint = f;
          modkind = MOD_INC;
          modpos = f;
          lf = fl;
        }
        if (dirty) {
          wsyncT<CH>();
          if (valid) {
            s_so[wpos] = ow;
            s_slk[ow >> 16] = wsl;
            s_rm[ow >> 16] = wrm;
          }
          wsyncT<CH>();
        }
#ifdef GS_RUN_TL
        run_cyc += __builtin_amdgcn_s_memtime() - rt0;
#endif
        continue;
      }
    }
    uint32_t vrd, rqd, p, v;
    uint64_t rqq_p = 0, rqc_p = 0;
    const bool from_ring = !wrapped;
    if (from_ring) {
      const uint32_t rs = qhead % RING;
      uint32_t x = pf_x;
      if (__builtin_amdgcn_readfirstlane(pf_seq) != qhead + 1) {
        for (uint32_t spin = 0;; spin++) {
          const uint32_t sq = vld(&s_ring_seq[rs]);
          x = lane < RING_DW ? vld(&s_ring[rs][lane]) : 0u;
          if (__builtin_amdgcn_readfirstlane(sq) == qhead + 1) break;
          __builtin_amdgcn_s_sleep(0);
          if (spin > SPIN_MAX) {
            chan_err = true;
            break;
          }
        }
      }
      if (chan_err) {
        status = 2;
        break;
      }
      wsyncT<CH>();
      if (lane == 0) vst(&s_ctl[0], qhead + 1);
      vrd = x;
      rqd = x;
      p = rlane(vrd, 0);
      v = rlane(vrd, VR_DW - 1);
      rqq_p = (uint64_t)rlane(x, RING_CODES) | ((uint64_t)rlane(x, RING_CODES + 1) << 32);
      rqc_p = (uint64_t)rlane(x, RING_CODES + 2) | ((uint64_t)rlane(x, RING_CODES + 3) << 32);
    } else {
      p = __builtin_amdgcn_readfirstlane(d.queue[qhead]);
      const uint32_t le = __builtin_amdgcn_readfirstlane(d.last_epoch[p]);
      const uint32_t ll = __builtin_amdgcn_readfirstlane(d.last_len[p]);
      v = __builtin_amdgcn_readfirstlane(d.cur_var[p]);
      if (le == epoch && ll == qlen) break;
      vrd = lane < VR_DW ? ((const uint32_t*)(d.vars + v))[lane] : 0u;
      rqd = lane >= 32 && lane < 32 + 2 * R ? ((const uint32_t*)(d.pod_req + (size_t)p * R))[lane - 32] : 0u;
    }
    if (qhead + 1 == P) wrapped = true;
    qhead = qhead + 1 == P ? 0 : qhead + 1;
    qlen--;
    pops++;
    if ((pops & 15) == 0 && lane == 0) vst(&s_ctl[3], (uint32_t)pops);
    if (!wrapped) {
      pf_seq = vld(&s_ring_seq[qhead % RING]);
      pf_x = lane < RING_DW ? vld(&s_ring[qhead % RING][lane]) : 0u;
    }
    const uint32_t gp = p;
    auto VD = [&](uint32_t i) -> uint32_t { return rlane(vrd, i); };
    auto VD64 = [&](uint32_t i) -> uint64_t { return (uint64_t)VD(i) | ((uint64_t)VD(i + 1) << 32); };
    const uint32_t vctb = VD(3);
    const uint64_t vtolt = VD64(20);
    const uint32_t own_off = TOPO ? VD(22) : 0u, own_n = TOPO ? VD(23) : 0u;
    const uint32_t sel_off = TOPO ? VD(24) : 0u, sel_n = TOPO ? VD(25) : 0u;
    uint32_t og_e = 0, og_skew = 0, og_slot = 0, og_kind = 0;
    if (TOPO && own_n) {
      const auto& KD = *karg();
      if (lane < own_n) {
        og_e = KD.tg_list[own_off + lane];
        const TGroupRec& tg = KD.tgroups[og_e & TL_GID];
        og_skew = (uint32_t)tg.skew;
        og_slot = tg.slot;
        og_kind = tg.kind;
      }
    }
    auto OWN = [&](uint32_t k) -> OwnG {
      return OwnG{rlane(og_e, k), (int32_t)rlane(og_skew, k), rlane(og_slot, k), rlane(og_kind, k)};
    };
#define GS_RQ_AT(name)                                                                                \
  const uint32_t name##_x = fresh(rqd);                                                               \
  auto name = [&](uint32_t r) -> int64_t {                                                            \
    return (int64_t)((uint64_t)rlane(name##_x, 32 + 2 * r) | ((uint64_t)rlane(name##_x, 33 + 2 * r) << 32)); \
  }
    int64_t rq_lane = 0;
    {
      const uint32_t lo = (uint32_t)__shfl((int)rqd, (int)(32 + 2 * (lane & 7))),
                     hi = (uint32_t)__shfl((int)rqd, (int)(33 + 2 * (lane & 7)));
      if (lane < RR) rq_lane = (int64_t)(((uint64_t)hi << 32) | lo);
    }
    const bool rq_hi = RR > 4 && __ballot(lane >= 4 && lane < RR && rq_lane != 0) != 0;
    if (!from_ring) {
      GS_RQ_AT(RQ);
#pragma unroll
      for (uint32_t r = 0; r < 4; r++)
        if (r < d.RQ && r < RR) {
          rqq_p |= (uint64_t)qcode_floor(RQ(r)) << (16 * r);
          rqc_p |= (uint64_t)qcode_ceil(RQ(r)) << (16 * r);
        }
    }

    TLW(0);
    if (TOPO && own_n && (vctb & VF_ZSPREAD)) {
      const auto& KD = *karg();
      const uint64_t vzs = rlane(vrd, 26) | ((uint64_t)rlane(vrd, 27) << 32);
      topo_tmin(KD, ts, own_off, own_n, vzs, lane);
      wsyncT<CH>();
    }

    if (d.NN) {
      const auto& KD = *karg();
      const uint32_t vx = fresh(vrd);
      auto VX = [&](uint32_t i) -> uint32_t { return rlane(vx, i); };
      auto VX64 = [&](uint32_t i) -> uint64_t { return (uint64_t)VX(i) | ((uint64_t)VX(i + 1) << 32); };
      const uint32_t fk_begin = VX(1), fk_count = VX(2), zfull_off = VX(12), cfull_off = VX(13);
      const uint64_t vtol = VX64(18);
      uint64_t pvol[VDMAX] = {0, 0, 0, 0};
      uint32_t pfresh[VDMAX] = {0, 0, 0, 0};
      if (TOPO && KD.any_vol)
#pragma unroll
        for (uint32_t q = 0; q < VDMAX; q++) {
          pvol[q] = KD.pod_vol[(size_t)gp * VDMAX + q];
          pfresh[q] = KD.pod_vfresh[(size_t)gp * VDMAX + q];
        }
      bool pvany = false;
#pragma unroll
      for (uint32_t q = 0; q < VDMAX; q++) pvany = pvany || pvol[q] || pfresh[q];
      bool nplain = (vctb & VF_SIMPLE) && !pvany;
      nplain = nplain && !rq_hi;
      const uint64_t nrqq = rqq_p, nrqc = rqc_p;
      uint32_t nlo = 0;
      if (nhint_ok && (vtol & ~nhint_tol) == 0) {
        const bool ge = lane >= R || rq_lane >= hint_nrq;
        if (__ballot(!ge) == 0) nlo = nhint;
      }
      uint32_t fn = INF;
      bool nfa_win = false;
      GS_RQ_AT(RQ);
      for (uint32_t base = nlo & ~63u; base < KD.NN; base += 64) {
        const uint32_t n = base + lane;
        const bool in = (n < KD.NN) & (n >= nlo);
        const uint32_t nc = in ? n : 0u;
        const uint64_t nsl = s_nslk[nc], nrm = s_nrm[nc];
        const uint32_t nfl = s_nflag[nc];
        const bool lp = in & swar_ge(nsl, nrqq);
        const bool fa = lp & nplain & (bool)(nfl & 1u) & swar_ge(nrm, nrqc);
        const uint64_t lpb = __ballot(lp);
        CTR(C_NEV, KD.NN - base < 64 ? KD.NN - base : 64);
        if (!lpb) continue;
        const uint64_t fab = __ballot(fa);
        const uint32_t mfl = fab ? ffs64(fab) : 64u;
        const bool need = lp & !fa & (lane < mfl);
        bool feas = fa;
        if (__ballot(need)) {
          if (need) {
            const NodeRec& nr = KD.nodes[n];
            const FK* nfk = KD.n_fk + (size_t)n * F;
            feas = nr.ok && (nr.taints & ~vtol) == 0;
#pragma unroll
            for (uint32_t r = 0; r < RR; r++) feas = feas && nr.req[r] + RQ(r) <= nr.avail[r];
#pragma unroll
            for (uint32_t k = 0; k < KMAX_IT; k++) {
              const uint32_t off = VX(4 + k);
              if (k >= KD.K || !feas || off == NONE) continue;
              const uint32_t vid = nr.vid[k];
              feas = vid != NONE && ((KD.itmask[off + (vid >> 6)] >> (vid & 63)) & 1);
            }
            if (feas && zfull_off != NONE)
              feas = nr.zvid != NONE && ((KD.itmask[zfull_off + (nr.zvid >> 6)] >> (nr.zvid & 63)) & 1);
            if (feas && cfull_off != NONE)
              feas = nr.cvid != NONE && ((KD.itmask[cfull_off + (nr.cvid >> 6)] >> (nr.cvid & 63)) & 1);
            if (feas && fk_count) feas = fk_ok_range(d, fk_begin, fk_count, nfk, true);
            if (TOPO && feas && own_n)
              feas = topo_node_ok_g(KD, ts, own_n, nr.dvid,
                                    [&](uint32_t hs) -> int64_t { return KD.hn[(size_t)hs * KD.NN + n]; }, OWN);
            if (TOPO && feas && KD.any_vol) {
              const NodeVol& nv = KD.n_vol[n];
#pragma unroll
              for (uint32_t q = 0; q < VDMAX; q++)
                if (pvol[q] | pfresh[q]) feas = feas && nv.cnt[q] + (int32_t)pfresh[q] + __popcll(pvol[q] & ~nv.present) <= nv.lim[q];
            }
          }
        }
        const uint64_t b = __ballot(feas);
        if (b) {
          fn = base + ffs64(b);
          nfa_win = ((fab >> ffs64(b)) & 1) != 0;
          break;
        }
      }
      CTR(C_NPRE, fn != INF ? fn + 1 : KD.NN);
      if (nplain) {
        nhint = fn != INF ? fn : KD.NN;
        nhint_ok = true;
        nhint_tol = vtol;
        hint_nrq = rq_lane;
      }
      if (fn != INF && nfa_win) {
        const uint64_t sl = s_nslk[fn], rm = s_nrm[fn];
        uint32_t c_sl = 0, c_rm = 0;
        if (lane < KD.RQ) {
          const uint32_t sh = 16 * lane;
          c_sl = qcode_ceil(qcode_value((uint32_t)(sl >> sh) & 0xFFFFu) - rq_lane);
          c_rm = qcode_floor(qcode_value((uint32_t)(rm >> sh) & 0xFFFFu) - rq_lane);
        }
        uint64_t sl2 = 0, rm2 = 0;
#pragma unroll
        for (uint32_t r = 0; r < 4; r++)
          if (r < KD.RQ) {
            sl2 |= (uint64_t)rlane(c_sl, r) << (16 * r);
            rm2 |= (uint64_t)rlane(c_rm, r) << (16 * r);
          }
        if (lane == 0) {
          s_nslk[fn] = sl2;
          s_nrm[fn] = rm2;
          if (TOPO && sel_n) {
            const uint32_t z = KD.nodes0[fn].dvid;
            topo_record(KD, ts, sel_off, sel_n, z < 64u ? 1ull << z : 0ull, 0u,
                        [&](uint32_t hs) { KD.hn[(size_t)hs * KD.NN + fn]++; });
          }
        }
        wsyncT<CH>();
        emit(WQ_NFA, nlog, gp, v, fn, rqd, rq_lane);
        nlog++;
        CAT(6);
        continue;
      }
      if (fn != INF) {
        int64_t* areq = KD.nodes[fn].req;
        FK* afk = KD.n_fk + (size_t)fn * F;
        int64_t nreq = 0, navl = 0;
        if (lane < R) {
          nreq = areq[lane] + rq_lane;
          navl = KD.nodes[fn].avail[lane];
          areq[lane] = nreq;
        }
        if (lane < fk_count) {
          const FKEntry& e = KD.fk_entries[fk_begin + lane];
          FK* nf = afk + e.slot;
          const FK cur = *nf;
          *nf = (cur.flags & FK_PRESENT) ? fk_intersect(cur, e.st, KD.fk_ival + (size_t)e.slot * FKV, KD.fk_isint + (size_t)e.slot * FKW)
                                         : e.st;
        }
        {
          const int64_t sl = navl - nreq;
          const uint32_t c_sl = lane < KD.RQ ? qcode_ceil(sl) : 0u, c_rm = lane < KD.RQ ? qcode_floor(sl) : 0u;
          const bool over = lane >= 4 && lane < R && sl < 0;
          uint64_t sl2 = 0, rm2 = 0;
#pragma unroll
          for (uint32_t r = 0; r < 4; r++) {
            sl2 |= (uint64_t)rlane(c_sl, r) << (16 * r);
            rm2 |= (uint64_t)rlane(c_rm, r) << (16 * r);
          }
          const bool anyover = __ballot(over) != 0;
          if (lane == 0) {
            s_nslk[fn] = sl2;
            s_nrm[fn] = rm2;
            if (anyover) s_nflag[fn] = 0;
          }
        }
        if (lane == 0) {
          if (TOPO && KD.any_vol) {
            NodeVol& nv = KD.n_vol[fn];
            uint64_t all = 0;
#pragma unroll
            for (uint32_t q = 0; q < VDMAX; q++) {
              nv.cnt[q] += (int32_t)pfresh[q] + __popcll(pvol[q] & ~nv.present);
              all |= pvol[q];
            }
            nv.present |= all;
          }
          if (TOPO && sel_n) {
            const uint32_t z = KD.nodes0[fn].dvid;
            topo_record(KD, ts, sel_off, sel_n, z < 64u ? 1ull << z : 0ull, 0u,
                        [&](uint32_t hs) { KD.hn[(size_t)hs * KD.NN + fn]++; });
          }
        }
        wsyncT<CH>();
        emit(WQ_LOG, nlog, gp, v, fn | 0x80000000u, 0, 0);
        nlog++;
        CAT(6);
        continue;
      }
    }

    TLW(1);
    uint32_t win_base = INF, win_v = 0;
    if (M >= 50 && modkind == MOD_INC && !pivot_touched(modkind, modpos, M)) {
      const uint32_t k = modpos + lane;
      const uint32_t w = k < M ? (uint32_t)acc.so[k] : 0xFFFFu;
      const uint32_t w0 = rlane(w, 0), x = w0 & 0xFFFFu;
      const uint64_t b = __ballot(lane >= 1 && (w & 0xFFFFu) >= x);
      if (b) {
        const uint32_t eo = ffs64(b);
        if (eo > 1) {
          CTR(C_FAST, 1);
          const uint32_t sh = (uint32_t)__builtin_amdgcn_update_dpp(0, (int)w, 0x130, 0xF, 0xF, false);
          const uint32_t nw = lane + 1 == eo ? w0 : sh;
          wsyncT<CH>();
          if (lane < eo) acc.so[k] = nw;
          wsyncT<CH>();
          win_v = lane < eo ? nw : w;
#ifdef GS_FFD_TL
          n_rot++;
          n_rotlen += eo - 1;
#endif
          if (modpos < hint && modpos + eo - 1 >= hint) hint--;
        } else {
          win_v = w;
        }
        win_base = modpos;
        modkind = MOD_NONE;
      }
    }
    if (M > 1 && modkind != MOD_NONE) {
      bool inversion = false;
      if (modkind == MOD_INC) inversion = modpos + 1 < M && acc.key(modpos + 1) < acc.key(modpos);
      else if (modkind == MOD_APPEND) inversion = acc.key(M - 2) > acc.key(M - 1);
      inversion = __builtin_amdgcn_readfirstlane(inversion ? 1u : 0u) != 0;
      if (inversion) {
        if (M <= 12) {
          reg_pdq_frame(PackedArr<U32, CH>{(U32*)s_so}, 0, (int)M, bits_len((uint64_t)M), 1, 1);
          hint_ok = false;
        } else if (M >= 50 && (!pivot_touched(modkind, modpos, M) || pivot_hint_wave(acc, (int)M, lane) == 1)) {
          CTR(C_FAST, 1);
          if (modkind == MOD_INC) {
            const uint32_t x = acc.key(modpos);
            const uint32_t e = wave_first(modpos + 1, M, lane, [&](uint32_t k) { return acc.key(k) >= x; });
            ws.rotate((int)modpos, (int)e - 1, true);
#ifdef GS_FFD_TL
            n_rot++;
            n_rotlen += e - 1 - modpos;
#endif
            if (modpos < hint && e - 1 >= hint) hint--;
          } else {
            const uint32_t x = acc.key(M - 1);
            const uint32_t lo = wave_first(0, M - 1, lane, [&](uint32_t k) { return acc.key(k) > x; });
            ws.rotate((int)lo, (int)M - 1, false);
#ifdef GS_FFD_TL
            n_rot++;
            n_rotlen += M - 1 - lo;
#endif
            if (lo < hint) hint = lo;
          }
        } else {
          CTR(C_GEN, 1);
          const int known_x = modkind == MOD_INC ? (int)modpos : (int)M - 1;
#ifdef GS_FFD_TL
          const uint64_t g0_ = __builtin_amdgcn_s_memtime();
#endif
#ifdef GS_SORT_TL
          wave_pdqsort<GS_WAVE_SEQ, U32, U16, CH, true>(ws.so, ws.scr, ws.stk, ws.lane, ws.half, (int)M, known_x, s_stl);
#else
          wave_pdqsort<GS_WAVE_SEQ, U32, U16, CH, true>(ws.so, ws.scr, ws.stk, ws.lane, ws.half, (int)M, known_x);
#endif
#ifdef GS_FFD_TL
          n_gen_cyc += __builtin_amdgcn_s_memtime() - g0_;
#endif
          hint_ok = false;
        }
      }
      modkind = MOD_NONE;
    }

    TLW(2);
    bool simple = (vctb & VF_SIMPLE) != 0;
    simple = simple && !rq_hi;
    const bool hostfa = TOPO && !rq_hi && (vctb & VF_HOSTFA) != 0;
#ifdef GS_FFD_TL
    n_nonsimple += simple ? 0u : 1u;
#endif

    uint32_t f = INF;
    bool ovf = false;
    uint32_t lo_bound = 0;
    if (hint_ok && (vtolt & ~hint_tolt) == 0) {
      const bool ge = lane >= 4 || lane >= R || rq_lane >= hint_rq;
      if (__ballot(!ge) == 0) lo_bound = hint;
    }
    uint32_t scan_from = lo_bound;
    for (;;) {
      uint32_t nex = 0, fa_pos = INF, fa_j = 0, resume = INF;
      uint32_t fa_ev = 0, fa_l = 0;
      uint64_t fa_sq = 0, fa_rv = 0;
      constexpr bool SPF = WIDE || !TOPO;
      uint32_t ev_next = 0;
      bool have_next = false;
      for (uint32_t cb = scan_from; cb < M; cb += 64) {
        const uint32_t pos = cb + lane;
        const uint32_t ev = cb == win_base ? win_v : (SPF && have_next) ? ev_next : s_so[pos < M ? pos : M - 1], je = ev >> 16;
        if (SPF) {
          const uint32_t pn = pos + 64u;
          ev_next = s_so[pn < M ? pn : M - 1];
          have_next = true;
        }
        const uint64_t sq = s_slk[je], rmv = s_rm[je];
        const uint32_t tt = T > 1 ? (uint32_t)s_tmpl[je] : 0u;
        bool lp = (pos >= lo_bound) & (pos < M) & (bool)((vtolt >> tt) & 1) & swar_ge(sq, rqq_p);
        if (TOPO && hostfa && lp) {
          const auto& KD = *karg();
          const int32_t* hrow = KD.hc + (size_t)je * KD.TGH;
          for (uint32_t k = 0; k < own_n; k++) {
            const int64_t c = hrow[rlane(og_slot, k)] + ((rlane(og_e, k) & TL_SELF) ? 1 : 0);
            lp = lp && c <= (int64_t)(int32_t)rlane(og_skew, k);
          }
        }
        const bool fa = lp & (simple | hostfa) & swar_ge(rmv, rqc_p);
        const uint64_t fab = __ballot(fa), exb = __ballot(lp & !fa);
        const uint32_t mfl = fab ? ffs64(fab) : 64u;
        const uint64_t ex = exb & (mfl == 64 ? ~0ull : ((1ull << mfl) - 1ull));
        const uint32_t cnt = (uint32_t)__popcll(ex);
        if (nex + cnt > 64) {
          resume = cb;
          break;
        }
        CTR(C_CAND, M - cb < 64 ? M - cb : 64);
        if (ex) {
          if ((ex >> lane) & 1) s_exl[nex + (uint32_t)__popcll(ex & ((1ull << lane) - 1ull))] = (pos & 0xFFFFu) | (je << 16);
          nex += cnt;
        }
        if (fab) {
          fa_pos = cb + mfl;
          fa_j = rlane(je, mfl);
          fa_ev = ev;
          fa_l = mfl;
          fa_sq = sq;
          fa_rv = rmv;
          break;
        }
      }
      wsyncT<CH>();
      TLW(5);
      if (nex) {
        const auto& KD = *karg();
        const uint32_t vx = fresh(vrd);
        auto VX = [&](uint32_t i) -> uint32_t { return rlane(vx, i); };
        auto VX64 = [&](uint32_t i) -> uint64_t { return (uint64_t)VX(i) | ((uint64_t)VX(i + 1) << 32); };
        const uint32_t fk_begin = VX(1), fk_count = VX(2), vzflags = VX(30);
        const uint64_t vzm = VX64(14), vcm = VX64(16), vzn = VX64(28);
        CTR(C_FULL, nex);
#ifdef GS_FFD_TL
        n_xns += simple ? 0u : nex;
        n_xb++;
#endif
        const uint32_t lgL = !WIDE ? 0u : nex <= 8 ? 3u : nex <= 16 ? 2u : nex <= 32 ? 1u : 0u;
        const uint32_t lgW = W <= 4 ? 0u : W <= 8 ? 1u : W <= 16 ? 2u : 3u;
        const uint32_t lg = lgL < lgW ? lgL : lgW;
        const uint32_t cx = lane >> lg, sub = lane & ((1u << lg) - 1u);
        const uint32_t xe = cx < nex ? s_exl[cx] : 0u;
        const uint32_t j = xe >> 16, xpos = xe & 0xFFFFu;
        const uint32_t t = cx < nex ? (uint32_t)s_tmpl[j] : 0u;
        GS_RQ_AT(RQ);
      bool feas = false;
      uint64_t zset = ~0ull;
      uint64_t zm = 0, cm = 0, czf = 0;
      uint32_t czfl = 0;
      uint32_t mrow[RR];
      int64_t tot[RR];
      int64_t maxa_pre[RR];
#pragma unroll
      for (uint32_t r = 0; r < RR; r++) maxa_pre[r] = 0;
      uint64_t nx[WREG] = {0, 0, 0, 0};
      uint64_t G = 0, Gt = 0;
      if (cx < nex) {
        const ClaimRec* cr = KD.c_rec + j;
        uint32_t cur[RR];
#pragma unroll
        for (uint32_t r = 0; r < RR; r++) maxa_pre[r] = cr->maxa[r];
        {
          const uint4* q = (const uint4*)cr;
          const uint4 h0 = q[0], h1 = q[1], h2 = q[2], h3 = q[3];
          const int64_t lo[4] = {(int64_t)(((uint64_t)h0.y << 32) | h0.x), (int64_t)(((uint64_t)h0.w << 32) | h0.z),
                                 (int64_t)(((uint64_t)h1.y << 32) | h1.x), (int64_t)(((uint64_t)h1.w << 32) | h1.z)};
          const uint32_t cl[4] = {h2.x & 0xFFFFu, h2.x >> 16, h2.y & 0xFFFFu, h2.y >> 16};
          zm = ((uint64_t)h2.w << 32) | h2.z;
          cm = ((uint64_t)h3.y << 32) | h3.x;
#pragma unroll
          for (uint32_t r = 0; r < RR; r++) {
            tot[r] = r < 4 ? lo[r] : cr->tot_hi[r - 4];
            cur[r] = r < 4 ? cl[r] : cr->thr_hi[r - 4];
          }
        }
        const uint64_t* row = KD.rows + ((size_t)v * T + t) * OW;
        const uint64_t* opts = KD.c_opts + (size_t)j * OW;
        if (!WIDE) {
          const uint4* oq = (const uint4*)opts;
          const uint4* rq4 = (const uint4*)row;
          const uint4 o0 = oq[0], o1 = oq[1], r0 = rq4[0], r1 = rq4[1];
          const uint64_t a[4] = {(((uint64_t)o0.y << 32) | o0.x) & (((uint64_t)r0.y << 32) | r0.x),
                                 (((uint64_t)o0.w << 32) | o0.z) & (((uint64_t)r0.w << 32) | r0.z),
                                 (((uint64_t)o1.y << 32) | o1.x) & (((uint64_t)r1.y << 32) | r1.x),
                                 (((uint64_t)o1.w << 32) | o1.z) & (((uint64_t)r1.w << 32) | r1.z)};
#pragma unroll
          for (uint32_t w = 0; w < WREG; w++) nx[w] = w < W ? a[w] : 0;
        }
        bool pre = true;
        if (fk_count) pre = fk_ok_range(d, fk_begin, fk_count, KD.c_fk + (size_t)j * F, false);
        if (TOPO && pre && own_n) {
          czf = cr->zfull;
          czfl = cr->zflags;
          const int32_t* hrow = KD.hc + (size_t)j * KD.TGH;
          zset = topo_claim_g(KD, ts, own_n, czf & vzn, [&](uint32_t hs) -> int64_t { return hrow[hs]; }, OWN);
          pre = zset != 0;
          if (pre && zset != ~0ull) {
            const uint64_t dcat = topo_catmask(KD, zset);
            if (KD.dom_ct) cm &= dcat;
            else if (!KD.dom_np) zm &= dcat;
          }
        }
        if (pre) {
          G = grid_of(zm & vzm, cm & vcm, KD.Z, KD.C);
          Gt = grid_of(s_tzm[t] & vzm, s_tcm[t] & vcm, KD.Z, KD.C);
          uint32_t mm[RR];
#pragma unroll
          for (uint32_t r = 0; r < RR; r++) {
            const uint32_t o = s_thoff[r], n = s_thoff[r + 1] - o;
            mm[r] = thr_window(thr + o, n, cur[r], tot[r] + RQ(r));
          }
#pragma unroll
          for (uint32_t r = 0; r < RR; r++) {
            const uint32_t o = s_thoff[r], n = s_thoff[r + 1] - o;
            if (mm[r] == cur[r] + 4 && mm[r] < n) mm[r] = thr_search(thr + o, n, mm[r], tot[r] + RQ(r));
            mrow[r] = o + r + mm[r];
          }
          uint64_t accw = 0;
          if (!WIDE) {
#pragma unroll
            for (uint32_t r = 0; r < RR; r++) {
              if (mm[r] != cur[r]) {
                const uint4* tq = (const uint4*)(KD.thr_set + (size_t)mrow[r] * OW);
                const uint4 t0 = tq[0], t1 = tq[1];
                nx[0] &= ((uint64_t)t0.y << 32) | t0.x;
                nx[1] &= ((uint64_t)t0.w << 32) | t0.z;
                nx[2] &= ((uint64_t)t1.y << 32) | t1.x;
                nx[3] &= ((uint64_t)t1.w << 32) | t1.z;
              }
            }
            if (G != Gt) {
              uint64_t off[WREG] = {};
              for (uint64_t gm = G; gm; gm &= gm - 1) {
                const uint32_t g = ffs64(gm);
#pragma unroll
                for (uint32_t w = 0; w < WREG; w++)
                  if (w < W) off[w] |= slot[g * W + w];
              }
#pragma unroll
              for (uint32_t w = 0; w < WREG; w++) nx[w] &= off[w];
            }
#pragma unroll
            for (uint32_t w = 0; w < WREG; w++) accw |= nx[w];
          } else {
#ifndef GS_XC
#define GS_XC 2
#endif
            for (uint32_t w0 = sub * 4; w0 < W && !accw; w0 += (4u * GS_XC) << lg) {
              uint4 o[GS_XC][2], rw[GS_XC][2], tt[GS_XC][RR][2];
#pragma unroll
              for (uint32_t c = 0; c < GS_XC; c++) {
                const uint32_t wc = w0 + (c * 4u << lg);
                if (wc < W) {
                  const uint4* oq = (const uint4*)(opts + wc);
                  const uint4* rq4 = (const uint4*)(row + wc);
                  o[c][0] = oq[0];
                  o[c][1] = oq[1];
                  rw[c][0] = rq4[0];
                  rw[c][1] = rq4[1];
#pragma unroll
                  for (uint32_t r = 0; r < RR; r++) {
                    if (mm[r] == cur[r]) continue;
                    const uint4* tq = (const uint4*)(KD.thr_set + (size_t)mrow[r] * OW + wc);
                    tt[c][r][0] = tq[0];
                    tt[c][r][1] = tq[1];
                  }
                }
              }
#pragma unroll
              for (uint32_t c = 0; c < GS_XC; c++) {
                const uint32_t wc = w0 + (c * 4u << lg);
                if (wc >= W) continue;
                uint64_t x[4] = {(((uint64_t)o[c][0].y << 32) | o[c][0].x) & (((uint64_t)rw[c][0].y << 32) | rw[c][0].x),
                                 (((uint64_t)o[c][0].w << 32) | o[c][0].z) & (((uint64_t)rw[c][0].w << 32) | rw[c][0].z),
                                 (((uint64_t)o[c][1].y << 32) | o[c][1].x) & (((uint64_t)rw[c][1].y << 32) | rw[c][1].x),
                                 (((uint64_t)o[c][1].w << 32) | o[c][1].z) & (((uint64_t)rw[c][1].w << 32) | rw[c][1].z)};
#pragma unroll
                for (uint32_t r = 0; r < RR; r++) {
                  if (mm[r] == cur[r]) continue;
                  x[0] &= ((uint64_t)tt[c][r][0].y << 32) | tt[c][r][0].x;
                  x[1] &= ((uint64_t)tt[c][r][0].w << 32) | tt[c][r][0].z;
                  x[2] &= ((uint64_t)tt[c][r][1].y << 32) | tt[c][r][1].x;
                  x[3] &= ((uint64_t)tt[c][r][1].w << 32) | tt[c][r][1].z;
                }
#pragma unroll
                for (uint32_t w = 0; w < 4; w++) {
                  if (wc + w >= W) x[w] = 0;
                  if (x[w] && G != Gt) {
                    uint64_t off = 0;
                    for (uint64_t gm = G; gm; gm &= gm - 1) off |= slot[(size_t)ffs64(gm) * W + wc + w];
                    x[w] &= off;
                  }
                  accw |= x[w];
                }
              }
            }
          }
          const uint64_t gb = __ballot(accw != 0);
          feas = ((gb >> (lane & ~((1u << lg) - 1u))) & ((1ull << (1u << lg)) - 1ull)) != 0;
          if (TOPO && feas && KD.tmpl[t].mv_mask) {
            feas = mv_ok(KD, KD.tmpl[t], [&](uint32_t w) -> uint64_t {
              if (!WIDE) return w == 0 ? nx[0] : w == 1 ? nx[1] : w == 2 ? nx[2] : nx[3];
              uint64_t x = opts[w] & row[w];
#pragma unroll
              for (uint32_t r = 0; r < RR; r++) x &= KD.thr_set[(size_t)mrow[r] * OW + w];
              if (G != Gt) {
                uint64_t off = 0;
                for (uint64_t gm = G; gm; gm &= gm - 1) off |= slot[(size_t)ffs64(gm) * W + w];
                x &= off;
              }
              return x;
            });
          }
        }
      }
        const uint64_t fm = __ballot(feas);
        TLW(6);
        if (fm) {
          const uint32_t wl = ffs64(fm);
          f = rlane(xpos, wl);
#ifdef GS_FFD_TL
          n_xwin++;
#endif
        if (WIDE) {
          const uint32_t jw = rlane(j, wl), tw = rlane(t, wl);
          uint32_t mw[RR];
  #pragma unroll
          for (uint32_t r = 0; r < RR; r++) mw[r] = rlane(mrow[r], wl);
          const uint64_t Gw = ((uint64_t)rlane((uint32_t)(G >> 32), wl) << 32) | rlane((uint32_t)G, wl);
          const uint64_t Gtw = ((uint64_t)rlane((uint32_t)(Gt >> 32), wl) << 32) | rlane((uint32_t)Gt, wl);
          uint64_t* wopts = KD.c_opts + (size_t)jw * OW;
          const uint64_t* row = KD.rows + ((size_t)v * T + tw) * OW;
          for (uint32_t w = lane; w < W; w += 64) {
            uint64_t x = wopts[w] & row[w];
  #pragma unroll
            for (uint32_t r = 0; r < RR; r++) x &= KD.thr_set[(size_t)mw[r] * OW + w];
            if (Gw != Gtw) {
              uint64_t off = 0;
              for (uint64_t gm = Gw; gm; gm &= gm - 1) off |= slot[(size_t)ffs64(gm) * W + w];
              x &= off;
            }
            wopts[w] = x;
          }
        }
        if (lane == wl) {
          ClaimRec* cr = KD.c_rec + j;
          uint64_t* opts = KD.c_opts + (size_t)j * OW;
          if (!WIDE) {
  #pragma unroll
            for (uint32_t w = 0; w < WREG; w++)
              if (w < W) opts[w] = nx[w];
          }
          int64_t nt[RR], ma[RR];
          uint32_t cu[RR];
  #pragma unroll
          for (uint32_t r = 0; r < RR; r++) {
            nt[r] = tot[r] + RQ(r);
            ma[r] = maxa_pre[r];
            cu[r] = mrow[r] - s_thoff[r] - r;
            cr->tot(r) = nt[r];
            cr->thr(r) = (uint16_t)cu[r];
          }
          s_slk[j] = pack_slack(d, ma, nt);
          s_rm[j] = pack_room(thr, s_thoff, cu, nt, KD.RQ);
          cr->zm = zm & vzm;
          cr->cm = cm & vcm;
          cr->ctb &= vctb;
          if (TOPO) {
            if (!own_n) {
              czf = cr->zfull;
              czfl = cr->zflags;
            }
            const uint64_t zf = czf & vzn & zset;
            const uint32_t zl = zset != ~0ull ? 0u : (czfl & vzflags);
            cr->zfull = zf;
            cr->zflags = zl;
            int32_t* hrow = KD.hc + (size_t)j * KD.TGH;
            topo_record(KD, ts, sel_off, sel_n, zf, zl, [&](uint32_t hs) { hrow[hs] = (hrow[hs] & HC_COUNT) + 1; });
          }
          FK* cf = KD.c_fk + (size_t)j * F;
          for (uint32_t k = 0; k < fk_count; k++) {
            const FKEntry& e = KD.fk_entries[fk_begin + k];
            const FK cur = cf[e.slot];
            cf[e.slot] = (cur.flags & FK_PRESENT)
                             ? fk_intersect(cur, e.st, KD.fk_ival + (size_t)e.slot * FKV, KD.fk_isint + (size_t)e.slot * FKW)
                             : e.st;
          }
          const uint32_t e = s_so[f];
          if ((e & 0xFFFFu) == 0xFFFFu) ovf = true;
          s_so[f] = e + 1u;
        }
          wsyncT<CH>();
          emit(WQ_LOG, nlog, gp, v, rlane(j, wl), 0, 0);
          break;
        }
      }
      if (fa_pos != INF) {
        f = fa_pos;
        const uint32_t j = fa_j;
        {
          const uint32_t fl = fa_l;
          const uint64_t rm = ((uint64_t)rlane((uint32_t)(fa_rv >> 32), fl) << 32) | rlane((uint32_t)fa_rv, fl);
          const uint64_t sl = ((uint64_t)rlane((uint32_t)(fa_sq >> 32), fl) << 32) | rlane((uint32_t)fa_sq, fl);
          const uint32_t e = rlane(fa_ev, fl);
          uint32_t c_rm = 0, c_sl = 0;
          if (lane < d.RQ) {
            const uint32_t sh = 16 * lane;
            c_rm = qcode_floor(qcode_value((uint32_t)(rm >> sh) & 0xFFFFu) - rq_lane);
            c_sl = qcode_ceil(qcode_value((uint32_t)(sl >> sh) & 0xFFFFu) - rq_lane);
          }
          uint32_t prm = (lane & 1u) ? c_rm << 16 : c_rm, psl = (lane & 1u) ? c_sl << 16 : c_sl;
          prm |= (uint32_t)__builtin_amdgcn_update_dpp(0, (int)prm, 0xB1, 0xF, 0xF, false);
          psl |= (uint32_t)__builtin_amdgcn_update_dpp(0, (int)psl, 0xB1, 0xF, 0xF, false);
          const uint32_t hrm = (uint32_t)__builtin_amdgcn_update_dpp(0, (int)prm, 0x102, 0xF, 0xF, false);
          const uint32_t hsl = (uint32_t)__builtin_amdgcn_update_dpp(0, (int)psl, 0x102, 0xF, 0xF, false);
          if ((e & 0xFFFFu) == 0xFFFFu) ovf = true;
          if (lane == 0) {
            s_rm[j] = (uint64_t)prm | ((uint64_t)hrm << 32);
            s_slk[j] = (uint64_t)psl | ((uint64_t)hsl << 32);
            s_so[f] = e + 1u;
            if (TOPO && sel_n) {
              const auto& KD = *karg();
              const ClaimRec* cr = KD.c_rec + j;
              int32_t* hrow = KD.hc + (size_t)j * KD.TGH;
              topo_record(KD, ts, sel_off, sel_n, cr->zfull, cr->zflags, [&](uint32_t hs) { hrow[hs] = (hrow[hs] & HC_COUNT) + 1; });
            }
          }
        }
        wsyncT<CH>();
        emit(WQ_FA, nlog, gp, v, j, rqd, rq_lane);
        CTR(C_FA, 1);
        break;
      }
      if (resume == INF) break;
      scan_from = resume;
    }
    if (__ballot(ovf)) status = 3;
    CTR(C_ALG, f != INF ? f + 1 : M);
    TLW(3);
#ifdef GS_FFD_TL
    n_fsum += f != INF ? f : 0;
#endif
    if (simple) {
      hint = f != INF ? f : M;
      hint_ok = true;
      hint_tolt = vtolt;
      hint_rq = rq_lane;
    }
    if (f != INF) {
      wsyncT<CH>();
      modkind = MOD_INC;
      modpos = f;
      nlog++;
      run_prev = !TOPO && !WIDE && from_ring && simple && !__ballot(ovf);
      CAT(simple ? 1 : 3);
      run_rec = vrd;
      continue;
    }

    bool opened = false;
    {
      const auto& KD = *karg();
      const uint32_t vx = fresh(vrd);
      auto VX = [&](uint32_t i) -> uint32_t { return rlane(vx, i); };
      auto VX64 = [&](uint32_t i) -> uint64_t { return (uint64_t)VX(i) | ((uint64_t)VX(i + 1) << 32); };
      const uint32_t fk_begin = VX(1), fk_count = VX(2), vzflags = VX(30);
      const uint64_t vzm = VX64(14), vcm = VX64(16), vzn = VX64(28);
    for (uint32_t t = 0; t < T; t++) {
      const TmplRec& tr = KD.tmpl[t];
      const uint64_t* row = KD.rows + ((size_t)v * T + t) * OW;
      uint64_t tzs = ~0ull, tzcat = ~0ull;
      if (TOPO && own_n) {
        tzs = topo_claim_g(KD, ts, own_n, tr.zfull & vzn, [](uint32_t) -> int64_t { return 0; }, OWN);
        if (tzs != 0 && tzs != ~0ull && !KD.dom_np) tzcat = topo_catmask(KD, tzs);
        tzs = (uint64_t)uniform_i64((int64_t)tzs);
        tzcat = (uint64_t)uniform_i64((int64_t)tzcat);
        if (tzs == 0 || tzcat == 0) continue;
      }
      const bool dct = KD.dom_ct != 0;
      const uint64_t tcm = tr.cm & vcm & (dct ? tzcat : ~0ull), tzsel = dct ? tr.zm & vzm : tzcat;
      const bool dnp = KD.dom_np != 0;
      auto rowx = [&](uint32_t w) -> uint64_t {
        uint64_t x = row[w];
        if (tzs != ~0ull && !dnp) {
          uint64_t off = 0;
          for (uint64_t zm_ = tzsel; zm_; zm_ &= zm_ - 1) {
            const uint32_t zc = ffs64(zm_);
            for (uint32_t c = 0; c < KD.C; c++)
              if ((tcm >> c) & 1) off |= slot[(zc * KD.C + c) * W + w];
          }
          x &= off;
        }
        return x;
      };
      bool anyl = false;
      if (KD.fk_ok[(size_t)v * T + t])
        for (uint32_t w = lane; w < W; w += 64) anyl = anyl || rowx(w) != 0;
      if (!__ballot(anyl)) continue;
      if (tr.has_limits) {
        bool hit = false;
        for (uint32_t i = lane; i < KD.N; i += 64) {
          if (!((rowx(i >> 6) >> (i & 63)) & 1)) continue;
          bool ok = true;
          for (uint32_t r = 0; r < R; r++)
            if ((tr.limit_rmask >> r) & 1) ok = ok && KD.it_cap[(size_t)r * KD.N + i] <= KD.t_rem[(size_t)t * R + r];
          hit = hit || ok;
        }
        if (!__ballot(hit)) continue;
      }
      int64_t tot_l = 0;
      uint32_t c0_l = 0;
      if (lane < R) {
        tot_l = tr.daemon[lane] + rq_lane;
        const uint32_t o = s_thoff[lane], n = s_thoff[lane + 1] - o;
        c0_l = thr_search(thr + o, n, 0, tot_l);
      }
      uint32_t c0[RR];
#pragma unroll
      for (uint32_t r = 0; r < RR; r++) c0[r] = (uint32_t)__shfl((int)c0_l, (int)r);
      uint64_t xw[2] = {0, 0};
#pragma unroll
      for (uint32_t h = 0; h < 2; h++) {
        const uint32_t w = lane + 64 * h;
        if (w >= W) continue;
        uint64_t x = rowx(w);
#pragma unroll
        for (uint32_t r = 0; r < RR; r++) x &= KD.thr_set[(size_t)(s_thoff[r] + r + c0[r]) * OW + w];
        if (tr.has_limits) {
          uint64_t y = 0;
          for (uint64_t m = x; m; m &= m - 1) {
            const uint32_t b = ffs64(m);
            const uint32_t i = w * 64 + b;
            bool ok = true;
            for (uint32_t r = 0; r < R; r++)
              if ((tr.limit_rmask >> r) & 1) ok = ok && KD.it_cap[(size_t)r * KD.N + i] <= KD.t_rem[(size_t)t * R + r];
            if (ok) y |= 1ull << b;
          }
          x = y;
        }
        xw[h] = x;
      }
      if (TOPO && tr.mv_mask && !mv_ok(KD, tr, [&](uint32_t w) { return shfl_u64(xw[w >> 6], w & 63); })) continue;
      if (M >= MC) {
        status = 1;
        break;
      }
      const uint32_t j = M;
      ClaimRec* cr = KD.c_rec + j;
#pragma unroll
      for (uint32_t h = 0; h < 2; h++)
        if (lane + 64 * h < W) KD.c_opts[(size_t)j * OW + lane + 64 * h] = xw[h];
      if (lane < RR) {
        cr->tot(lane) = tot_l;
        cr->thr(lane) = (uint16_t)c0_l;
      }
      uint64_t mxa[RR], mxc[RR];
#pragma unroll
      for (uint32_t r = 0; r < RR; r++) mxa[r] = mxc[r] = 0;
      for (uint32_t w = 0; w < W; w++) {
        const uint64_t word = shfl_u64(xw[w >> 6], w & 63);
        if (!((word >> lane) & 1)) continue;
        const uint32_t i = w * 64 + lane;
#pragma unroll
        for (uint32_t r = 0; r < RR; r++) {
          const uint64_t a = (uint64_t)KD.it_alloc[(size_t)r * KD.N + i];
          mxa[r] = a > mxa[r] ? a : mxa[r];
          if (tr.has_limits && ((tr.limit_rmask >> r) & 1)) {
            const uint64_t c = (uint64_t)(KD.it_cap[(size_t)r * KD.N + i] + (1ll << 62));
            mxc[r] = c > mxc[r] ? c : mxc[r];
          }
        }
      }
      int64_t ma[RR], nt[RR];
      GS_RQ_AT(RQ);
#pragma unroll
      for (uint32_t r = 0; r < RR; r++) {
        ma[r] = (int64_t)wave_max_u64(mxa[r]);
        if (tr.has_limits) mxc[r] = wave_max_u64(mxc[r]);
        nt[r] = tr.daemon[r] + RQ(r);
      }
      if (TOPO)
        for (uint32_t h = lane; h < KD.TGH; h += 64) KD.hc[(size_t)j * KD.TGH + h] = 0;
      const uint64_t n_sl = pack_slack(d, ma, nt), n_rm = pack_room(thr, s_thoff, c0, nt, KD.RQ);
      wsyncT<CH>();
      if (lane == 0) {
        cr->tmpl = t;
        cr->count = 1;
        cr->zm = tr.zm & vzm & (dct ? ~0ull : tzcat);
        cr->cm = tcm;
        cr->ctb = tr.ctb & vctb;
        cr->zfull = tr.zfull & vzn & tzs;
// ... 143 lines not shown
```

karpenter-provider-ibm-cloud_amd/csrc/layout.hpp:

```cpp
#pragma once
#include <stdint.h>
#include <stddef.h>

#ifndef __HIPCC__
#ifndef __host__
#define __host__
#endif
#ifndef __device__
#define __device__
#endif
#endif

namespace gsd {

constexpr int RMAX = 8;
constexpr int KMAX_IT = 8;
constexpr uint32_t OVH_MAX = 128;
inline uint32_t ovh_slots_for(uint32_t ov_cap) {
  if (ov_cap > OVH_MAX) return 0;
  uint32_t s = 16;
  while (s < 2 * ov_cap) s <<= 1;
  return s;
}
constexpr int FMAX = 16;
// ... 160 lines not shown
  uint64_t pad;
};
static_assert(sizeof(SimOut) == 64, "SimOut layout");
struct OptPair {
  uint32_t it, minp;
};
struct SlotOut {
  uint64_t node_evals, node_prefix, pops;
  uint32_t opt_base, n_opt;
};
static_assert(sizeof(SlotOut) == 32, "SlotOut layout");
constexpr uint32_t SIM_OPTS_MAX = 60;

__host__ __device__ inline uint64_t pair_grid(uint64_t zm, uint64_t cm, uint32_t Z, uint32_t C) {
  const uint64_t cmask = C >= 64 ? ~0ull : ((1ull << C) - 1);
  uint64_t g = 0;
  for (uint32_t z = 0; z < Z && z * C < 64; z++)
    if ((zm >> z) & 1) g |= (cm & cmask) << (z * C);
  return g;
}
__host__ __device__ inline uint32_t option_min_rank(const uint64_t* it_pair, const uint32_t* it_prank, uint32_t it,
                                                    uint64_t G) {
  uint32_t minp = NONE;
  uint64_t m = it_pair[it] & G;
  while (m) {
    const uint32_t g = (uint32_t)__builtin_ctzll(m);
    m &= m - 1;
    const uint32_t r = it_prank[(size_t)it * 64 + g];
    minp = r < minp ? r : minp;
  }
  return minp;
}

struct DevProblem {
  uint32_t N, W, R, Z, C, T, F, V, P, K, NT;
  uint32_t NN;
  uint32_t RQ;
  uint32_t OW;
  uint32_t n_thr;
  uint32_t max_claims;
  uint32_t max_claims_wave;
  uint32_t claim_cap;
  uint64_t wk_slots;
  const uint32_t* it_vid;
  const uint16_t* it_dvid;
  uint32_t it_key_unique;
  uint32_t any_mv;
  const int64_t* it_alloc;
  const int64_t* it_cap;
  const uint64_t* it_pair;
  const uint32_t* it_prank;
  const uint32_t* it_namerank;
  const uint32_t* rank_to_it;
  const uint64_t* slot_set;
  const uint64_t* grid_list;
  const uint32_t* grid_off;
  const uint64_t* grid_keys;
  const uint32_t* grid_its;
  const uint64_t* grid_planes;
  const uint64_t* grid_blocks;
  uint32_t n_grids, n_planes, grid_nb;
  const int64_t* thr_val;
  const uint32_t* thr_off;
  const uint64_t* thr_set;
  const int64_t* fk_ival;
  const uint64_t* fk_isint;
  const TmplRec* tmpl;
  const uint64_t* t_opts;
  const uint64_t* t_limopts;
  const FK* t_fk;
  const int64_t* pod_req;
  const uint32_t* var_begin;
  const uint32_t* var_count;
  const VarRec* vars;
  const uint64_t* itmask;
  const uint32_t* var_itclass;
  const uint32_t* var_pod;
  const uint64_t* itclass_mask;
  const FKEntry* fk_entries;
  const uint32_t* queue0;
  const VarRec* qvars;
  const int64_t* qreqs;
  const uint32_t* qcodes;
  const uint32_t* qrun;
  const NodeRec* nodes0;
  const FK* n_fk0;
  NodeRec* nodes;
  const NodeVol* n_vol0;
  NodeVol* n_vol;
  const uint64_t* pod_vol;
  const uint32_t* pod_vfresh;
  uint32_t any_vol;
  FK* n_fk;
  uint64_t* rows;
  uint32_t* cheapest;
  uint64_t* cheapest_key;
  uint32_t* nfo;
  uint32_t* fk_ok;
  uint32_t* pair_cur;
  uint32_t* queue;
  uint32_t* last_len;
  uint32_t* last_epoch;
  uint32_t* cur_var;
  ClaimRec* c_rec;
  uint64_t* c_opts;
  FK* c_fk;
  int64_t* t_rem;
  LogRec* log;
  uint32_t* c_sorted;
  uint64_t* ch_slk;
  uint64_t* ch_rm;
  uint32_t* ch_so;
  uint16_t* ch_scr;
  uint8_t* ch_tmpl;
  Ctrl* ctrl;
  uint32_t TG, TGH, NZV;
  uint32_t TGZ, ZS;
  uint32_t dom_ct;
  uint32_t dom_np;
  uint32_t n_lazy;
  uint64_t zknown0;
  const TGroupRec* tgroups;
  const uint32_t* tg_list;
  const uint32_t* lazy_slot;
  const uint32_t* var_lz_off;
  const uint32_t* lz_idx;
  const int32_t* lz_mind;
  const int32_t* zcnt0;
  const int32_t* htot0;
  const uint32_t* zone_order;
  const uint32_t* zone_cat;
  const int32_t* hn0;
  const uint32_t* nsp_off;
  const uint64_t* nsp;
  int32_t* hn;
  int32_t* hc;
  uint32_t* c_its;
  uint32_t* c_nits;
  uint32_t* slot_its;
  uint32_t* slot_nits;
  uint32_t* slot_drop;
  uint32_t n_sims;
  uint32_t sim_nt;
  uint32_t ov_cap;
  uint32_t nb_words;
  uint32_t n_pending;
  const uint32_t* sim_pod_off;
  const uint32_t* sim_pods;
  const uint32_t* sim_cand_off;
  const uint32_t* sim_cands;
  int64_t* ov_req;
  FK* ov_fk;
  SimCtrl* sim_ctrl;
  Ctrl* sim_blk;
  ClaimRec* sim_hdr;
  uint32_t* sim_next;
  const uint64_t* sim_known;
  uint64_t* ov_hn;
  NodeVol* ov_vol;
  uint32_t ov_epoch;
  uint32_t* ov_map;
  uint32_t ovh_slots;
  uint32_t sim_lds;
};

constexpr int SHARDS_MAX = 16;
struct ShardSrc {
// ... 18 lines not shown
```

karpenter-provider-ibm-cloud_amd/csrc/queue_kernels.hpp:

```cpp
#pragma once
#include "kernel_problem.hpp"

__global__ __launch_bounds__(256) void GS_KNAME(queue_records_kernel)(GS_KPROBLEM_ARG) {
  GS_KPROBLEM
  const uint32_t k = blockIdx.x * 256 + threadIdx.x;
  if (k >= d.P) return;
  const uint32_t p = d.queue0[k];
  const uint4* src = (const uint4*)(d.vars + d.var_begin[p]);
  uint4* dst = (uint4*)(const_cast<VarRec*>(d.qvars) + k);
#pragma unroll
  for (uint32_t q = 0; q < sizeof(VarRec) / sizeof(uint4); q++) dst[q] = src[q];
  int64_t* qr = const_cast<int64_t*>(d.qreqs) + (size_t)k * d.R;
  uint64_t fl = 0, ce = 0;
  for (uint32_t r = 0; r < d.R; r++) {
    const int64_t v = d.pod_req[(size_t)p * d.R + r];
    qr[r] = v;
    if (r < 4) {
      fl |= (uint64_t)qcode_floor(v) << (16 * r);
      ce |= (uint64_t)qcode_ceil(v) << (16 * r);
    }
  }
  uint4 c;
  c.x = (uint32_t)fl;
  c.y = (uint32_t)(fl >> 32);
  c.z = (uint32_t)ce;
  c.w = (uint32_t)(ce >> 32);
  ((uint4*)const_cast<uint32_t*>(d.qcodes))[k] = c;
}

__device__ __forceinline__ bool queue_record_same(const DevProblem& d, uint32_t a, uint32_t b) {
  const uint4* va = (const uint4*)(d.qvars + a);
  const uint4* vb = (const uint4*)(d.qvars + b);
  bool same = true;
#pragma unroll
  for (uint32_t q = 0; q < sizeof(VarRec) / 16; q++) {
    const uint4 x = va[q], y = vb[q];
    same = same && (q == 0 || x.x == y.x) && x.y == y.y && x.z == y.z && (q == sizeof(VarRec) / 16 - 1 || x.w == y.w);
  }
  for (uint32_t r = 0; r < d.R; r++) same = same && d.qreqs[(size_t)a * d.R + r] == d.qreqs[(size_t)b * d.R + r];
  return same;
}
__global__ __launch_bounds__(256) void GS_KNAME(queue_runs_kernel)(GS_KPROBLEM_ARG) {
  GS_KPROBLEM
  GS_KPROBLEM_EXIT(blockIdx.x * 256 >= d.P)
  __shared__ uint8_t s_same[256 + 16];
  const uint32_t b0 = blockIdx.x * 256;
  for (uint32_t t = threadIdx.x; t < 256 + 16; t += 256) {
    const uint32_t x = b0 + t;
    s_same[t] = x + 1 < d.P && queue_record_same(d, x, x + 1);
  }
  __syncthreads();
  const uint32_t k = b0 + threadIdx.x;
  if (k >= d.P) return;
  uint32_t n = 1;
  while (n < 16 && s_same[threadIdx.x + n - 1]) n++;
  const_cast<uint32_t*>(d.qrun)[k] = n;
}
```

Measured before the change: 451.6 million.

## Drop queue run kernel, cache hot pointers in lanes, branchless qcode helpers

Removes the queue_runs kernel, the qrun buffer and its ring slot, which also shrinks the ring record by one dword. Hot kernel-argument pointers and scalars are parked in lane registers and read back with readlane instead of re-dereferencing the argument struct. The qcode helpers move to a shared header with branchless arithmetic. Ballots are wrapped in an explicit 64-bit wave ballot with masks applied afterwards, and per-iteration counters are accumulated locally. Together these cut a launch and reduce register and scalar-load pressure in the hot FFD loop, but they touch many separate code paths, so a behavioural change in any of them is possible.

After: 475.9 million (median of 6 runs). 5.4% higher.

```diff
diff --git a/karpenter-provider-ibm-cloud_amd/csrc/batch_kernels.hip b/karpenter-provider-ibm-cloud_amd/csrc/batch_kernels.hip
--- a/karpenter-provider-ibm-cloud_amd/csrc/batch_kernels.hip
+++ b/karpenter-provider-ibm-cloud_amd/csrc/batch_kernels.hip
@@ -63,7 +63,6 @@
   if (n > 65535) return hipErrorInvalidValue;
   const uint32_t blocks = (max_pods + 255) / 256;
   hipLaunchKernelGGL(queue_records_kernel_batch, dim3(blocks, n), dim3(256), 0, s, ds);
-  hipLaunchKernelGGL(queue_runs_kernel_batch, dim3(blocks, n), dim3(256), 0, s, ds);
   return hipGetLastError();
 }
 
diff --git a/karpenter-provider-ibm-cloud_amd/csrc/capi.cpp b/karpenter-provider-ibm-cloud_amd/csrc/capi.cpp
--- a/karpenter-provider-ibm-cloud_amd/csrc/capi.cpp
+++ b/karpenter-provider-ibm-cloud_amd/csrc/capi.cpp
@@ -99,7 +99,6 @@
     c->alloc(d.qvars, std::max<uint32_t>(e.P, 1));
     c->alloc(d.qreqs, (size_t)std::max<uint32_t>(e.P, 1) * std::max<uint32_t>(e.R, 1));
     c->alloc(d.qcodes, (size_t)std::max<uint32_t>(e.P, 1) * 4);
-    c->alloc(d.qrun, std::max<uint32_t>(e.P, 1));
   }
   d.NN = e.NN;
   d.TG = e.TG;
diff --git a/karpenter-provider-ibm-cloud_amd/csrc/ffd.hip b/karpenter-provider-ibm-cloud_amd/csrc/ffd.hip
--- a/karpenter-provider-ibm-cloud_amd/csrc/ffd.hip
+++ b/karpenter-provider-ibm-cloud_amd/csrc/ffd.hip
@@ -98,6 +98,5 @@
 extern "C" hipError_t gsk_queue_records(const DevProblem* d, hipStream_t s) {
   if (!d->P) return hipSuccess;
   hipLaunchKernelGGL(queue_records_kernel, dim3((d->P + 255) / 256), dim3(256), 0, s, *d);
-  hipLaunchKernelGGL(queue_runs_kernel, dim3((d->P + 255) / 256), dim3(256), 0, s, *d);
   return hipGetLastError();
 }
diff --git a/karpenter-provider-ibm-cloud_amd/csrc/ffd_common.hpp b/karpenter-provider-ibm-cloud_amd/csrc/ffd_common.hpp
--- a/karpenter-provider-ibm-cloud_amd/csrc/ffd_common.hpp
+++ b/karpenter-provider-ibm-cloud_amd/csrc/ffd_common.hpp
@@ -4,6 +4,7 @@
 
 #include "devutil.hpp"
 #include "layout.hpp"
+#include "qcode.hpp"
 
 namespace gsd {
 namespace {
@@ -284,6 +285,8 @@
   return (uint32_t)__builtin_amdgcn_readlane((int)x, (int)i);
 }
 
+__device__ __forceinline__ uint64_t ballot64(bool p) { return __builtin_amdgcn_ballot_w64(p); }
+
 __device__ __forceinline__ uint32_t ffs64(uint64_t m) { return (uint32_t)__ffsll((long long)m) - 1u; }
 
 
@@ -351,9 +354,9 @@
     const uint32_t p = key(a), k = v & 0xFFFFu;
     const bool inr = (int)lane > a && (int)lane < b;
     const bool lt = k < p;
-    const int mid = a + (int)__popcll(__ballot(inr && lt));
+    const int mid = a + (int)__popcll(ballot64(inr && lt));
     const bool inl = (int)lane > a && (int)lane <= mid;
-    const uint64_t lm = __ballot(inl && !lt), rm = __ballot(inr && !inl && lt);
+    const uint64_t lm = ballot64(inl && !lt), rm = ballot64(inr && !inl && lt);
     if (lm) swap_misplaced(lm, rm);
     swap(mid, a);
     *already = lm == 0;
@@ -364,9 +367,9 @@
     const uint32_t p = key(a), k = v & 0xFFFFu;
     const bool inr = (int)lane > a && (int)lane < b;
     const bool le = k <= p;
-    const int mid = a + (int)__popcll(__ballot(inr && le));
+    const int mid = a + (int)__popcll(ballot64(inr && le));
     const bool inl = (int)lane > a && (int)lane <= mid;
-    const uint64_t lm = __ballot(inl && !le), rm = __ballot(inr && !inl && le);
+    const uint64_t lm = ballot64(inl && !le), rm = ballot64(inr && !inl && le);
     if (lm) swap_misplaced(lm, rm);
     return mid + 1;
   }
@@ -391,20 +394,20 @@
     for (int j = 0; j < 5; j++) {
       const uint32_t k = v & 0xFFFFu;
       const uint32_t pk = (uint32_t)__shfl((int)v, (int)lane - 1) & 0xFFFFu;
-      const uint64_t inv = __ballot((int)lane >= i && (int)lane < b && k < pk);
+      const uint64_t inv = ballot64((int)lane >= i && (int)lane < b && k < pk);
       if (!inv) return true;
       i = (int)ffs64(inv);
       if (b - a < 50) return false;
       swap(i, i - 1);
       if (i - a >= 2) {
         const uint32_t x = key(i - 1);
-        const uint64_t hm = __ballot((int)lane <= i - 2 && (v & 0xFFFFu) <= x);
+        const uint64_t hm = ballot64((int)lane <= i - 2 && (v & 0xFFFFu) <= x);
         const int q = hm ? 63 - (int)__clzll((long long)hm) : -1;
         rotate_up(q + 1, i - 1);
       }
       if (b - i >= 2) {
         const uint32_t y = key(i);
-        const uint64_t em = __ballot((int)lane > i && (int)lane < b && (v & 0xFFFFu) >= y);
+        const uint64_t em = ballot64((int)lane > i && (int)lane < b && (v & 0xFFFFu) >= y);
         const int e = em ? (int)ffs64(em) : b;
         rotate_down(i, e - 1);
       }
@@ -602,14 +605,14 @@
   while (hi - lo > 64) {
     const uint32_t step = (hi - lo + 63) / 64;
     const uint32_t k = lo + lane * step + step - 1;
-    const uint64_t b = __ballot(k >= hi || pred(k));
+    const uint64_t b = ballot64(k >= hi || pred(k));
     if (!b) return hi;
     const uint32_t i = (uint32_t)__ffsll((long long)b) - 1;
     lo = lo + i * step;
     hi = lo + step < hi ? lo + step : hi;
   }
   const uint32_t k = lo + lane;
-  const uint64_t b = __ballot(k < hi && pred(k));
+  const uint64_t b = ballot64(k < hi && pred(k));
   return b ? lo + (uint32_t)__ffsll((long long)b) - 1 : hi;
 }
 
@@ -627,30 +630,6 @@
   const uint32_t lo = __builtin_amdgcn_readfirstlane((uint32_t)x);
   const uint32_t hi = __builtin_amdgcn_readfirstlane((uint32_t)((uint64_t)x >> 32));
   return (int64_t)(((uint64_t)hi << 32) | lo);
-}
-
-__device__ __forceinline__ uint32_t qcode_floor(int64_t v) {
-  if (v <= 0) return 0;
-  const uint64_t x = (uint64_t)v;
-  const uint32_t b = 64u - (uint32_t)__clzll((long long)x);
-  if (b <= 10) return (uint32_t)x;
-  const uint32_t s = b - 10;
-  return 1024u + (s - 1) * 512u + (uint32_t)((x >> s) - 512u);
-}
-__device__ __forceinline__ uint32_t qcode_ceil(int64_t v) {
-  if (v <= 0) return 0;
-  const uint64_t x = (uint64_t)v;
-  const uint32_t b = 64u - (uint32_t)__clzll((long long)x);
-  if (b <= 10) return (uint32_t)x;
-  const uint32_t s = b - 10;
-  const uint32_t c = 1024u + (s - 1) * 512u + (uint32_t)((x >> s) - 512u);
-  return c + ((x & ((1ull << s) - 1)) ? 1u : 0u);
-}
-
-__device__ __forceinline__ int64_t qcode_value(uint32_t c) {
-  if (c < 1024u) return (int64_t)c;
-  const uint32_t s = (c - 1024u) / 512u + 1u, m = (c - 1024u) % 512u + 512u;
-  return (int64_t)((uint64_t)m << s);
 }
 
 __device__ __forceinline__ uint64_t pack_room(const int64_t* thr, const uint32_t* thoff, const uint32_t* cur,
diff --git a/karpenter-provider-ibm-cloud_amd/csrc/ffd_wave.hpp b/karpenter-provider-ibm-cloud_amd/csrc/ffd_wave.hpp
--- a/karpenter-provider-ibm-cloud_amd/csrc/ffd_wave.hpp
+++ b/karpenter-provider-ibm-cloud_amd/csrc/ffd_wave.hpp
@@ -29,9 +29,8 @@
 #define GS_RING 16
 #endif
 constexpr uint32_t RING = GS_RING;
-constexpr uint32_t RING_DW = 53;
+constexpr uint32_t RING_DW = 52;
 constexpr uint32_t RING_CODES = 48;
-constexpr uint32_t RING_QRUN = 52;
 constexpr uint32_t WQ = 32;
 constexpr uint32_t WQ_DW = 16;
 enum : uint32_t { WQ_LOG = 1, WQ_FA = 2, WQ_STOP = 3, WQ_NFA = 4 };
@@ -80,6 +79,10 @@
   return p;
 }
 #endif
+template <class T>
+__device__ __forceinline__ T* global_ptr(uint64_t a) {
+  return (T*)(__attribute__((address_space(1))) T*)a;
+}
 __device__ __forceinline__ uint32_t fresh(uint32_t x) {
   asm volatile("" : "+v"(x));
   return x;
@@ -154,14 +157,14 @@
   const int step = (n - 1 + 63) / 64;
   const int q = skip_e(1 + (int)lane * step);
   const bool qv = 1 + (int)lane * step < n && q < n;
-  const uint64_t m1 = __ballot(qv && key(qv ? q : 0) >= p);
+  const uint64_t m1 = ballot64(qv && key(qv ? q : 0) >= p);
   int lo, hi;
   if (m1) {
     const int l = (int)ffs64(m1);
     lo = l == 0 ? 1 : (int)rlane((uint32_t)q, (uint32_t)(l - 1)) + 1;
     hi = (int)rlane((uint32_t)q, (uint32_t)l);
   } else {
-    const int lv = 63 - (int)__clzll((long long)__ballot(qv));
+    const int lv = 63 - (int)__clzll((long long)ballot64(qv));
     lo = (int)rlane((uint32_t)q, (uint32_t)lv) + 1;
     hi = n;
   }
@@ -169,7 +172,7 @@
   for (int base = lo; base < hi; base += 64) {
     const int k = base + (int)lane;
     const bool ok = k < hi && k < n && !in_e(k);
-    const uint64_t m2 = __ballot(ok && key(ok ? k : 0) >= p);
+    const uint64_t m2 = ballot64(ok && key(ok ? k : 0) >= p);
     if (m2) {
       t = base + (int)ffs64(m2);
       break;
@@ -233,7 +236,7 @@
       right = pos > mid && ke < p;
     }
   }
-  const uint64_t lm = __ballot(left), rm = __ballot(right);
+  const uint64_t lm = ballot64(left), rm = ballot64(right);
   const uint32_t s = (uint32_t)__popcll(lm);
   if (s) {
     const uint64_t fl = lm | rm;
@@ -292,7 +295,7 @@
         in[u] = k < hi && pred(k);
       }
 #pragma unroll
-      for (int u = 0; u < RW; u++) c += (uint32_t)__popcll(__ballot(in[u]));
+      for (int u = 0; u < RW; u++) c += (uint32_t)__popcll(ballot64(in[u]));
     }
     return c;
   }
@@ -310,7 +313,7 @@
 #pragma unroll
       for (int u = 0; u < RW; u++) {
         const int idx = base + u * 64 + (int)lane;
-        const uint64_t m = __ballot(in[u]);
+        const uint64_t m = ballot64(in[u]);
         if (in[u]) out[total + (uint32_t)__popcll(m & ((1ull << lane) - 1ull))] = (uint16_t)(desc ? hi - 1 - idx : lo + idx);
         total += (uint32_t)__popcll(m);
       }
@@ -346,7 +349,7 @@
         const bool valid = k < hi;
         const bool in = valid && (LE ? kk[u] <= p : kk[u] < p);
         const bool out = valid && !in;
-        const uint64_t bi = __ballot(in);
+        const uint64_t bi = ballot64(in);
         c += (uint32_t)__popcll(bi);
         mine = lane == (uint32_t)((base - lo) / 64 + u) ? bi : mine;
         const uint32_t nk = 0xFFFFu - kk[u];
@@ -506,7 +509,7 @@
       for (int u = 0; u < RW; u++) hit[u] = base + u * 64 + (int)lane < b && kc[u] < kp[u];
 #pragma unroll
       for (int u = 0; u < RW; u++) {
-        const uint64_t m = __ballot(hit[u]);
+        const uint64_t m = ballot64(hit[u]);
         if (m) return base + u * 64 + (int)ffs64(m);
       }
     }
@@ -525,7 +528,7 @@
         int q = -1;
         for (int top = i - 2; top >= 0; top -= 64) {
           const int k = top - (int)lane;
-          const uint64_t m = __ballot(k >= 0 && key(k) <= x);
+          const uint64_t m = ballot64(k >= 0 && key(k) <= x);
           if (m) {
             q = top - (int)ffs64(m);
             break;
@@ -538,7 +541,7 @@
         int q = b;
         for (int base = i + 1; base < b; base += 64) {
           const int k = base + (int)lane;
-          const uint64_t m = __ballot(k < b && key(k) >= y);
+          const uint64_t m = ballot64(k < b && key(k) >= y);
           if (m) {
             q = base + (int)ffs64(m);
             break;
@@ -870,7 +873,6 @@
             if (lane < VR_DW) val[i] = qv_dw[k * VR_DW + lane];
             else if (lane < 32 + 2 * R) val[i] = qr_dw[k * 2 * R + (lane - 32)];
             else if (lane >= RING_CODES && lane < RING_CODES + 4) val[i] = d.qcodes[k * 4 + (lane - RING_CODES)];
-            else if (lane == RING_QRUN) val[i] = d.qrun[k];
           }
         }
 #pragma unroll
@@ -939,16 +941,47 @@
     }
   };
 
+  enum : uint32_t { HP_LOG = 0, HP_CREC, HP_COPTS, HP_ROWS, HP_THRSET, HP_NODES, HP_N,
+                    HU_Z = 8, HU_C, HU_RQ, HU_NN };
+  uint32_t hp_lo = 0, hp_hi = 0;
+  {
+    const uint64_t hp[HP_N] = {(uint64_t)d.log,  (uint64_t)d.c_rec,   (uint64_t)d.c_opts,
+                               (uint64_t)d.rows, (uint64_t)d.thr_set, (uint64_t)d.nodes};
+#pragma unroll
+    for (uint32_t k = 0; k < HP_N; k++)
+      if (lane == k) {
+        hp_lo = (uint32_t)hp[k];
+        hp_hi = (uint32_t)(hp[k] >> 32);
+      }
+    hp_lo = lane == HU_Z ? d.Z : lane == HU_C ? d.C : lane == HU_RQ ? d.RQ : lane == HU_NN ? d.NN : hp_lo;
+  }
+  auto HP = [&](uint32_t k) -> uint64_t { return (uint64_t)rlane(hp_lo, k) | ((uint64_t)rlane(hp_hi, k) << 32); };
+  auto HU = [&](uint32_t k) -> uint32_t { return rlane(hp_lo, k); };
+  struct HotRQ {
+    uint32_t RQ;
+  };
+  struct HotKD {
+    ClaimRec* c_rec;
+    uint64_t* c_opts;
+    const uint64_t* rows;
+    const uint64_t* thr_set;
+    uint32_t Z, C, RQ;
+  };
+  auto hot = [&]() -> HotKD {
+    return HotKD{global_ptr<ClaimRec>(HP(HP_CREC)),      global_ptr<uint64_t>(HP(HP_COPTS)),
+                 global_ptr<const uint64_t>(HP(HP_ROWS)), global_ptr<const uint64_t>(HP(HP_THRSET)),
+                 HU(HU_Z), HU(HU_C), HU(HU_RQ)};
+  };
+
   auto emit = [&](uint32_t type, uint32_t idx, uint32_t pod, uint32_t var, uint32_t tgt, uint32_t rqd_, int64_t rql) {
     if (false) {
       post(type, idx, pod, var, tgt, rqd_);
       return;
     }
-    const auto& KD = *karg();
-    if (lane == 0) KD.log[idx] = LogRec{pod, var, type == WQ_NFA ? tgt | 0x80000000u : tgt, 0};
+    if (lane == 0) global_ptr<LogRec>(HP(HP_LOG))[idx] = LogRec{pod, var, type == WQ_NFA ? tgt | 0x80000000u : tgt, 0};
     if ((type == WQ_FA || type == WQ_NFA) && lane < R && lane < 4 && rql != 0) {
-      unsigned long long* a = type == WQ_FA ? (unsigned long long*)&KD.c_rec[tgt].tot_lo[lane]
-                                            : (unsigned long long*)&KD.nodes[tgt].req[lane];
+      unsigned long long* a = type == WQ_FA ? (unsigned long long*)&global_ptr<ClaimRec>(HP(HP_CREC))[tgt].tot_lo[lane]
+                                            : (unsigned long long*)&global_ptr<NodeRec>(HP(HP_NODES))[tgt].req[lane];
       atomicAdd(a, (unsigned long long)rql);
     }
   };
@@ -1012,7 +1045,8 @@
         (d.NN == 0 || (nhint_ok && nhint >= d.NN))) {
       run_prev = false;
       auto same_spec = [&](uint32_t x) {
-        return __ballot(lane >= 1 && lane < RING_QRUN && lane != VR_DW - 1 && x != run_rec) == 0;
+        constexpr uint64_t spec_lanes = ((1ull << RING_DW) - 1ull) & ~1ull & ~(1ull << (VR_DW - 1));
+        return (ballot64(x != run_rec) & spec_lanes) == 0;
       };
       if (__builtin_amdgcn_readfirstlane(pf_seq) == qhead + 1 && same_spec(pf_x)) {
         const uint64_t r_tolt = (uint64_t)rlane(run_rec, 20) | ((uint64_t)rlane(run_rec, 21) << 32);
@@ -1046,6 +1080,8 @@
         load_window();
         uint32_t lf = 0;
         bool dirty = false;
+        uint64_t rc_cand = 0, rc_alg = 0;
+        uint32_t rc_fa = 0, rc_pods = 0;
         CTR(C_RENTER, 1);
         CAT(0);
 #ifdef GS_RUN_TL
@@ -1054,7 +1090,7 @@
         for (;;) {
           const uint32_t x = rlane(ow, lf) & 0xFFFFu;
           const bool ptouch = pivot_touched(MOD_INC, modpos, M);
-          const uint64_t b = ptouch ? 0ull : __ballot(lane > lf && (ow & 0xFFFFu) >= x);
+          const uint64_t b = ptouch ? 0ull : ballot64((ow & 0xFFFFu) >= x) & (~1ull << lf);
           const uint32_t eo = b ? ffs64(b) : 64u;
           if (!b) {
             CTR(ptouch ? C_RX_PIVOT : C_RX_WIN, 1);
@@ -1096,8 +1132,8 @@
           }
           if (pops + 1 > max_pops || qhead + 1 == P) break;
           const uint32_t lo = modpos - base;
-          const bool lp = (lane >= lo) & valid & (wtok != 0) & swar_ge(wsl, r_rqq);
-          const uint64_t lpb = __ballot(lp), fab = __ballot(lp & swar_ge(wrm, r_rqc));
+          const uint64_t lpb = ballot64(lane >= lo) & ballot64(wpos < M) & ballot64(wtok != 0) & ballot64(swar_ge(wsl, r_rqq));
+          const uint64_t fab = lpb & ballot64(swar_ge(wrm, r_rqc));
           if (!lpb) {
             CTR(C_RX_SCAN, 1);
             break;
@@ -1126,7 +1162,7 @@
             }
             const uint32_t mfl = fab ? ffs64(fab) : 64u;
             const uint64_t ex = lpb & ~fab & (mfl == 64 ? ~0ull : ((1ull << mfl) - 1ull));
-            const auto& KD = *karg();
+            const HotKD KD = hot();
             const uint32_t pvx = rlane(pf_x, VR_DW - 1);
             bool feas = false;
             if ((ex >> lane) & 1) {
@@ -1207,7 +1243,7 @@
             }
             CTR(C_FULL, __popcll(ex));
             CTR(C_RX_XC, 1);
-            const uint64_t fm = __ballot(feas);
+            const uint64_t fm = ballot64(feas);
             if (fm) {
               fl = ffs64(fm);
               xwin = true;
@@ -1234,7 +1270,7 @@
           pf_seq = vld(&s_ring_seq[qhead % RING]);
           pf_x = lane < RING_DW ? vld(&s_ring[qhead % RING][lane]) : 0u;
           if (xwin) {
-            const auto& KD = *karg();
+            const HotKD KD = hot();
             const uint32_t vctb = rlane(run_rec, 3);
             if (lane == fl) {
               const uint32_t j = ow >> 16;
@@ -1252,7 +1288,7 @@
                 cr->tot(r) = nt[r];
                 cr->thr(r) = (uint16_t)cu[r];
               }
-              wsl = pack_slack(d, x_ma, nt);
+              wsl = pack_slack(HotRQ{KD.RQ}, x_ma, nt);
               wrm = pack_room(thr, s_thoff, cu, nt, KD.RQ);
               s_slk[j] = wsl;
               s_rm[j] = wrm;
@@ -1266,10 +1302,9 @@
             wsyncT<CH>();
             emit(WQ_LOG, nlog, pp, pv, e >> 16, 0, 0);
             nlog++;
-            CTR(C_CAND, M - modpos < 64 ? M - modpos : 64);
-            CTR(C_ALG, f + 1);
-            CTR(C_NPRE, d.NN);
-            CTR(C_RPODS, 1);
+            rc_cand += M - modpos < 64 ? M - modpos : 64;
+            rc_alg += f + 1;
+            rc_pods++;
 #ifdef GS_CAT_TL
             cat_n += lane == 0 ? 1ull : 0ull;
 #endif
@@ -1281,12 +1316,10 @@
           }
           const uint64_t rm = ((uint64_t)rlane((uint32_t)(wrm >> 32), fl) << 32) | rlane((uint32_t)wrm, fl);
           const uint64_t sl = ((uint64_t)rlane((uint32_t)(wsl >> 32), fl) << 32) | rlane((uint32_t)wsl, fl);
-          uint32_t c_rm = 0, c_sl = 0;
-          if (lane < d.RQ) {
-            const uint32_t sh = 16 * lane;
-            c_rm = qcode_floor(qcode_value((uint32_t)(rm >> sh) & 0xFFFFu) - r_rq);
-            c_sl = qcode_ceil(qcode_value((uint32_t)(sl >> sh) & 0xFFFFu) - r_rq);
-          }
+          const uint32_t sh = 16 * (lane & 3u);
+          const bool rl = lane < HU(HU_RQ);
+          const uint32_t c_rm = rl ? qcode_floor(qcode_value((uint32_t)(rm >> sh) & 0xFFFFu) - r_rq) : 0u;
+          const uint32_t c_sl = rl ? qcode_ceil(qcode_value((uint32_t)(sl >> sh) & 0xFFFFu) - r_rq) : 0u;
           uint32_t prm = (lane & 1u) ? c_rm << 16 : c_rm, psl = (lane & 1u) ? c_sl << 16 : c_sl;
           prm |= (uint32_t)__builtin_amdgcn_update_dpp(0, (int)prm, 0xB1, 0xF, 0xF, false);
           psl |= (uint32_t)__builtin_amdgcn_update_dpp(0, (int)psl, 0xB1, 0xF, 0xF, false);
@@ -1303,11 +1336,10 @@
           const uint32_t f = base + fl;
           emit(WQ_FA, nlog, pp, pv, e >> 16, run_rec, r_rq);
           nlog++;
-          CTR(C_CAND, M - modpos < 64 ? M - modpos : 64);
-          CTR(C_FA, 1);
-          CTR(C_ALG, f + 1);
-          CTR(C_NPRE, d.NN);
-          CTR(C_RPODS, 1);
+          rc_cand += M - modpos < 64 ? M - modpos : 64;
+          rc_fa++;
+          rc_alg += f + 1;
+          rc_pods++;
 #ifdef GS_CAT_TL
           cat_n += lane == 0 ? 1ull : 0ull;
 #endif
@@ -1316,6 +1348,12 @@
           modpos = f;
           lf = fl;
         }
+        ctr += lane == C_CAND    ? rc_cand
+               : lane == C_FA    ? (uint64_t)rc_fa
+               : lane == C_ALG   ? rc_alg
+               : lane == C_NPRE  ? (uint64_t)rc_pods * d.NN
+               : lane == C_RPODS ? (uint64_t)rc_pods
+                                 : 0ull;
         if (dirty) {
           wsyncT<CH>();
           if (valid) {
@@ -1411,7 +1449,7 @@
                      hi = (uint32_t)__shfl((int)rqd, (int)(33 + 2 * (lane & 7)));
       if (lane < RR) rq_lane = (int64_t)(((uint64_t)hi << 32) | lo);
     }
-    const bool rq_hi = RR > 4 && __ballot(lane >= 4 && lane < RR && rq_lane != 0) != 0;
+    const bool rq_hi = RR > 4 && ballot64(lane >= 4 && lane < RR && rq_lane != 0) != 0;
     if (!from_ring) {
       GS_RQ_AT(RQ);
 #pragma unroll
@@ -1432,6 +1470,7 @@
 
     if (d.NN) {
       const auto& KD = *karg();
+      const uint32_t nn = HU(HU_NN);
       const uint32_t vx = fresh(vrd);
       auto VX = [&](uint32_t i) -> uint32_t { return rlane(vx, i); };
       auto VX64 = [&](uint32_t i) -> uint64_t { return (uint64_t)VX(i) | ((uint64_t)VX(i + 1) << 32); };
@@ -1453,28 +1492,27 @@
       const uint64_t nrqq = rqq_p, nrqc = rqc_p;
       uint32_t nlo = 0;
       if (nhint_ok && (vtol & ~nhint_tol) == 0) {
-        const bool ge = lane >= R || rq_lane >= hint_nrq;
-        if (__ballot(!ge) == 0) nlo = nhint;
+        if ((ballot64(rq_lane < hint_nrq) & ((1ull << RR) - 1ull)) == 0) nlo = nhint;
       }
       uint32_t fn = INF;
       bool nfa_win = false;
       GS_RQ_AT(RQ);
-      for (uint32_t base = nlo & ~63u; base < KD.NN; base += 64) {
+      for (uint32_t base = nlo & ~63u; base < nn; base += 64) {
         const uint32_t n = base + lane;
-        const bool in = (n < KD.NN) & (n >= nlo);
+        const bool in = (n < nn) & (n >= nlo);
         const uint32_t nc = in ? n : 0u;
         const uint64_t nsl = s_nslk[nc], nrm = s_nrm[nc];
         const uint32_t nfl = s_nflag[nc];
         const bool lp = in & swar_ge(nsl, nrqq);
         const bool fa = lp & nplain & (bool)(nfl & 1u) & swar_ge(nrm, nrqc);
-        const uint64_t lpb = __ballot(lp);
-        CTR(C_NEV, KD.NN - base < 64 ? KD.NN - base : 64);
+        const uint64_t lpb = ballot64(lp);
+        CTR(C_NEV, nn - base < 64 ? nn - base : 64);
         if (!lpb) continue;
-        const uint64_t fab = __ballot(fa);
+        const uint64_t fab = ballot64(fa);
         const uint32_t mfl = fab ? ffs64(fab) : 64u;
         const bool need = lp & !fa & (lane < mfl);
         bool feas = fa;
-        if (__ballot(need)) {
+        if (ballot64(need)) {
           if (need) {
             const NodeRec& nr = KD.nodes[n];
             const FK* nfk = KD.n_fk + (size_t)n * F;
@@ -1504,16 +1542,16 @@
             }
           }
         }
-        const uint64_t b = __ballot(feas);
+        const uint64_t b = ballot64(feas);
         if (b) {
           fn = base + ffs64(b);
           nfa_win = ((fab >> ffs64(b)) & 1) != 0;
           break;
         }
       }
-      CTR(C_NPRE, fn != INF ? fn + 1 : KD.NN);
+      CTR(C_NPRE, fn != INF ? fn + 1 : nn);
       if (nplain) {
-        nhint = fn != INF ? fn : KD.NN;
+        nhint = fn != INF ? fn : nn;
         nhint_ok = true;
         nhint_tol = vtol;
         hint_nrq = rq_lane;
@@ -1521,7 +1559,8 @@
       if (fn != INF && nfa_win) {
         const uint64_t sl = s_nslk[fn], rm = s_nrm[fn];
         uint32_t c_sl = 0, c_rm = 0;
-        if (lane < KD.RQ) {
+        const uint32_t hrq = HU(HU_RQ);
+        if (lane < hrq) {
           const uint32_t sh = 16 * lane;
           c_sl = qcode_ceil(qcode_value((uint32_t)(sl >> sh) & 0xFFFFu) - rq_lane);
           c_rm = qcode_floor(qcode_value((uint32_t)(rm >> sh) & 0xFFFFu) - rq_lane);
@@ -1529,7 +1568,7 @@
         uint64_t sl2 = 0, rm2 = 0;
 #pragma unroll
         for (uint32_t r = 0; r < 4; r++)
-          if (r < KD.RQ) {
+          if (r < hrq) {
             sl2 |= (uint64_t)rlane(c_sl, r) << (16 * r);
             rm2 |= (uint64_t)rlane(c_rm, r) << (16 * r);
           }
@@ -1574,7 +1613,7 @@
             sl2 |= (uint64_t)rlane(c_sl, r) << (16 * r);
             rm2 |= (uint64_t)rlane(c_rm, r) << (16 * r);
           }
-          const bool anyover = __ballot(over) != 0;
+          const bool anyover = ballot64(over) != 0;
           if (lane == 0) {
             s_nslk[fn] = sl2;
             s_nrm[fn] = rm2;
@@ -1612,7 +1651,7 @@
       const uint32_t k = modpos + lane;
       const uint32_t w = k < M ? (uint32_t)acc.so[k] : 0xFFFFu;
       const uint32_t w0 = rlane(w, 0), x = w0 & 0xFFFFu;
-      const uint64_t b = __ballot(lane >= 1 && (w & 0xFFFFu) >= x);
+      const uint64_t b = ballot64((w & 0xFFFFu) >= x) & ~1ull;
       if (b) {
         const uint32_t eo = ffs64(b);
         if (eo > 1) {
@@ -1697,8 +1736,7 @@
     bool ovf = false;
     uint32_t lo_bound = 0;
     if (hint_ok && (vtolt & ~hint_tolt) == 0) {
-      const bool ge = lane >= 4 || lane >= R || rq_lane >= hint_rq;
-      if (__ballot(!ge) == 0) lo_bound = hint;
+      if ((ballot64(rq_lane < hint_rq) & ((1ull << (RR < 4 ? RR : 4u)) - 1ull)) == 0) lo_bound = hint;
     }
     uint32_t scan_from = lo_bound;
     for (;;) {
@@ -1727,8 +1765,11 @@
             lp = lp && c <= (int64_t)(int32_t)rlane(og_skew, k);
           }
         }
-        const bool fa = lp & (simple | hostfa) & swar_ge(rmv, rqc_p);
-        const uint64_t fab = __ballot(fa), exb = __ballot(lp & !fa);
+        const uint64_t lpb = TOPO ? ballot64(lp)
+                                  : ballot64(pos >= lo_bound) & ballot64(pos < M) & ballot64(((vtolt >> tt) & 1) != 0) &
+                                        ballot64(swar_ge(sq, rqq_p));
+        const uint64_t fab = (simple | hostfa) ? lpb & ballot64(swar_ge(rmv, rqc_p)) : 0ull;
+        const uint64_t exb = lpb & ~fab;
         const uint32_t mfl = fab ? ffs64(fab) : 64u;
         const uint64_t ex = exb & (mfl == 64 ? ~0ull : ((1ull << mfl) - 1ull));
         const uint32_t cnt = (uint32_t)__popcll(ex);
@@ -1755,6 +1796,7 @@
       TLW(5);
       if (nex) {
         const auto& KD = *karg();
+        const HotKD HK = hot();
         const uint32_t vx = fresh(vrd);
         auto VX = [&](uint32_t i) -> uint32_t { return rlane(vx, i); };
         auto VX64 = [&](uint32_t i) -> uint64_t { return (uint64_t)VX(i) | ((uint64_t)VX(i + 1) << 32); };
@@ -1785,7 +1827,7 @@
       uint64_t nx[WREG] = {0, 0, 0, 0};
       uint64_t G = 0, Gt = 0;
       if (cx < nex) {
-        const ClaimRec* cr = KD.c_rec + j;
+        const ClaimRec* cr = HK.c_rec + j;
         uint32_t cur[RR];
 #pragma unroll
         for (uint32_t r = 0; r < RR; r++) maxa_pre[r] = cr->maxa[r];
@@ -1803,8 +1845,8 @@
             cur[r] = r < 4 ? cl[r] : cr->thr_hi[r - 4];
           }
         }
-        const uint64_t* row = KD.rows + ((size_t)v * T + t) * OW;
-        const uint64_t* opts = KD.c_opts + (size_t)j * OW;
+        const uint64_t* row = HK.rows + ((size_t)v * T + t) * OW;
+        const uint64_t* opts = HK.c_opts + (size_t)j * OW;
         if (!WIDE) {
           const uint4* oq = (const uint4*)opts;
           const uint4* rq4 = (const uint4*)row;
@@ -1831,8 +1873,8 @@
           }
         }
         if (pre) {
-          G = grid_of(zm & vzm, cm & vcm, KD.Z, KD.C);
-          Gt = grid_of(s_tzm[t] & vzm, s_tcm[t] & vcm, KD.Z, KD.C);
+          G = grid_of(zm & vzm, cm & vcm, HK.Z, HK.C);
+          Gt = grid_of(s_tzm[t] & vzm, s_tcm[t] & vcm, HK.Z, HK.C);
           uint32_t mm[RR];
 #pragma unroll
           for (uint32_t r = 0; r < RR; r++) {
@@ -1850,7 +1892,7 @@
 #pragma unroll
             for (uint32_t r = 0; r < RR; r++) {
               if (mm[r] != cur[r]) {
-                const uint4* tq = (const uint4*)(KD.thr_set + (size_t)mrow[r] * OW);
+                const uint4* tq = (const uint4*)(HK.thr_set + (size_t)mrow[r] * OW);
                 const uint4 t0 = tq[0], t1 = tq[1];
                 nx[0] &= ((uint64_t)t0.y << 32) | t0.x;
                 nx[1] &= ((uint64_t)t0.w << 32) | t0.z;
@@ -1890,7 +1932,7 @@
 #pragma unroll
                   for (uint32_t r = 0; r < RR; r++) {
                     if (mm[r] == cur[r]) continue;
-                    const uint4* tq = (const uint4*)(KD.thr_set + (size_t)mrow[r] * OW + wc);
+                    const uint4* tq = (const uint4*)(HK.thr_set + (size_t)mrow[r] * OW + wc);
                     tt[c][r][0] = tq[0];
                     tt[c][r][1] = tq[1];
                   }
@@ -1925,14 +1967,14 @@
               }
             }
           }
-          const uint64_t gb = __ballot(accw != 0);
+          const uint64_t gb = ballot64(accw != 0);
           feas = ((gb >> (lane & ~((1u << lg) - 1u))) & ((1ull << (1u << lg)) - 1ull)) != 0;
           if (TOPO && feas && KD.tmpl[t].mv_mask) {
             feas = mv_ok(KD, KD.tmpl[t], [&](uint32_t w) -> uint64_t {
               if (!WIDE) return w == 0 ? nx[0] : w == 1 ? nx[1] : w == 2 ? nx[2] : nx[3];
               uint64_t x = opts[w] & row[w];
 #pragma unroll
-              for (uint32_t r = 0; r < RR; r++) x &= KD.thr_set[(size_t)mrow[r] * OW + w];
+              for (uint32_t r = 0; r < RR; r++) x &= HK.thr_set[(size_t)mrow[r] * OW + w];
               if (G != Gt) {
                 uint64_t off = 0;
                 for (uint64_t gm = G; gm; gm &= gm - 1) off |= slot[(size_t)ffs64(gm) * W + w];
@@ -1943,7 +1985,7 @@
           }
         }
       }
-        const uint64_t fm = __ballot(feas);
+        const uint64_t fm = ballot64(feas);
         TLW(6);
         if (fm) {
           const uint32_t wl = ffs64(fm);
@@ -1958,12 +2000,12 @@
           for (uint32_t r = 0; r < RR; r++) mw[r] = rlane(mrow[r], wl);
           const uint64_t Gw = ((uint64_t)rlane((uint32_t)(G >> 32), wl) << 32) | rlane((uint32_t)G, wl);
           const uint64_t Gtw = ((uint64_t)rlane((uint32_t)(Gt >> 32), wl) << 32) | rlane((uint32_t)Gt, wl);
-          uint64_t* wopts = KD.c_opts + (size_t)jw * OW;
-          const uint64_t* row = KD.rows + ((size_t)v * T + tw) * OW;
+          uint64_t* wopts = HK.c_opts + (size_t)jw * OW;
+          const uint64_t* row = HK.rows + ((size_t)v * T + tw) * OW;
           for (uint32_t w = lane; w < W; w += 64) {
             uint64_t x = wopts[w] & row[w];
   #pragma unroll
-            for (uint32_t r = 0; r < RR; r++) x &= KD.thr_set[(size_t)mw[r] * OW + w];
+            for (uint32_t r = 0; r < RR; r++) x &= HK.thr_set[(size_t)mw[r] * OW + w];
             if (Gw != Gtw) {
               uint64_t off = 0;
               for (uint64_t gm = Gw; gm; gm &= gm - 1) off |= slot[(size_t)ffs64(gm) * W + w];
@@ -1973,8 +2015,8 @@
           }
         }
         if (lane == wl) {
-          ClaimRec* cr = KD.c_rec + j;
-          uint64_t* opts = KD.c_opts + (size_t)j * OW;
+          ClaimRec* cr = HK.c_rec + j;
+          uint64_t* opts = HK.c_opts + (size_t)j * OW;
           if (!WIDE) {
   #pragma unroll
             for (uint32_t w = 0; w < WREG; w++)
@@ -1990,8 +2032,8 @@
             cr->tot(r) = nt[r];
             cr->thr(r) = (uint16_t)cu[r];
           }
-          s_slk[j] = pack_slack(d, ma, nt);
-          s_rm[j] = pack_room(thr, s_thoff, cu, nt, KD.RQ);
+          s_slk[j] = pack_slack(HotRQ{HK.RQ}, ma, nt);
+          s_rm[j] = pack_room(thr, s_thoff, cu, nt, HK.RQ);
           cr->zm = zm & vzm;
           cr->cm = cm & vcm;
           cr->ctb &= vctb;
@@ -2032,12 +2074,10 @@
           const uint64_t rm = ((uint64_t)rlane((uint32_t)(fa_rv >> 32), fl) << 32) | rlane((uint32_t)fa_rv, fl);
           const uint64_t sl = ((uint64_t)rlane((uint32_t)(fa_sq >> 32), fl) << 32) | rlane((uint32_t)fa_sq, fl);
           const uint32_t e = rlane(fa_ev, fl);
-          uint32_t c_rm = 0, c_sl = 0;
-          if (lane < d.RQ) {
-            const uint32_t sh = 16 * lane;
-            c_rm = qcode_floor(qcode_value((uint32_t)(rm >> sh) & 0xFFFFu) - rq_lane);
-            c_sl = qcode_ceil(qcode_value((uint32_t)(sl >> sh) & 0xFFFFu) - rq_lane);
-          }
+          const uint32_t sh = 16 * (lane & 3u);
+          const bool rl = lane < HU(HU_RQ);
+          const uint32_t c_rm = rl ? qcode_floor(qcode_value((uint32_t)(rm >> sh) & 0xFFFFu) - rq_lane) : 0u;
+          const uint32_t c_sl = rl ? qcode_ceil(qcode_value((uint32_t)(sl >> sh) & 0xFFFFu) - rq_lane) : 0u;
           uint32_t prm = (lane & 1u) ? c_rm << 16 : c_rm, psl = (lane & 1u) ? c_sl << 16 : c_sl;
           prm |= (uint32_t)__builtin_amdgcn_update_dpp(0, (int)prm, 0xB1, 0xF, 0xF, false);
           psl |= (uint32_t)__builtin_amdgcn_update_dpp(0, (int)psl, 0xB1, 0xF, 0xF, false);
@@ -2064,7 +2104,7 @@
       if (resume == INF) break;
       scan_from = resume;
     }
-    if (__ballot(ovf)) status = 3;
+    if (ballot64(ovf)) status = 3;
     CTR(C_ALG, f != INF ? f + 1 : M);
     TLW(3);
 #ifdef GS_FFD_TL
@@ -2081,7 +2121,7 @@
       modkind = MOD_INC;
       modpos = f;
       nlog++;
-      run_prev = !TOPO && !WIDE && from_ring && simple && !__ballot(ovf);
+      run_prev = !TOPO && !WIDE && from_ring && simple && !ballot64(ovf);
       CAT(simple ? 1 : 3);
       run_rec = vrd;
       continue;
@@ -2125,7 +2165,7 @@
       bool anyl = false;
       if (KD.fk_ok[(size_t)v * T + t])
         for (uint32_t w = lane; w < W; w += 64) anyl = anyl || rowx(w) != 0;
-      if (!__ballot(anyl)) continue;
+      if (!ballot64(anyl)) continue;
       if (tr.has_limits) {
         bool hit = false;
         for (uint32_t i = lane; i < KD.N; i += 64) {
@@ -2135,7 +2175,7 @@
             if ((tr.limit_rmask >> r) & 1) ok = ok && KD.it_cap[(size_t)r * KD.N + i] <= KD.t_rem[(size_t)t * R + r];
           hit = hit || ok;
         }
-        if (!__ballot(hit)) continue;
+        if (!ballot64(hit)) continue;
       }
       int64_t tot_l = 0;
       uint32_t c0_l = 0;
diff --git a/karpenter-provider-ibm-cloud_amd/csrc/layout.hpp b/karpenter-provider-ibm-cloud_amd/csrc/layout.hpp
--- a/karpenter-provider-ibm-cloud_amd/csrc/layout.hpp
+++ b/karpenter-provider-ibm-cloud_amd/csrc/layout.hpp
@@ -266,7 +266,6 @@
   const VarRec* qvars;
   const int64_t* qreqs;
   const uint32_t* qcodes;
-  const uint32_t* qrun;
   const NodeRec* nodes0;
   const FK* n_fk0;
   NodeRec* nodes;
diff --git a/karpenter-provider-ibm-cloud_amd/csrc/qcode.hpp b/karpenter-provider-ibm-cloud_amd/csrc/qcode.hpp
--- /dev/null
+++ b/karpenter-provider-ibm-cloud_amd/csrc/qcode.hpp
@@ -0,0 +1,32 @@
+#pragma once
+#include <stdint.h>
+
+#if defined(__HIPCC__) || defined(__CUDACC__)
+#define GS_QCODE_FN __host__ __device__ __forceinline__
+#else
+#define GS_QCODE_FN static inline
+#endif
+
+GS_QCODE_FN uint32_t qcode_shift(uint64_t x) {
+  const uint32_t b = 64u - (uint32_t)__builtin_clzll((unsigned long long)(x | 1ull));
+  return (b > 10u ? b : 10u) - 10u;
+}
+
+GS_QCODE_FN uint32_t qcode_floor(int64_t v) {
+  const uint64_t x = v > 0 ? (uint64_t)v : 0ull;
+  const uint32_t s = qcode_shift(x);
+  return 512u * s + (uint32_t)(x >> s);
+}
+
+GS_QCODE_FN uint32_t qcode_ceil(int64_t v) {
+  const uint64_t x = v > 0 ? (uint64_t)v : 0ull;
+  const uint32_t s = qcode_shift(x);
+  return 512u * s + (uint32_t)(x >> s) + ((x & ((1ull << s) - 1ull)) ? 1u : 0u);
+}
+
+GS_QCODE_FN int64_t qcode_value(uint32_t c) {
+  const bool big = c >= 1024u;
+  const uint32_t s = big ? (c >> 9) - 1u : 0u;
+  const uint32_t m = big ? (c & 511u) + 512u : c;
+  return (int64_t)((uint64_t)m << (s & 63u));
+}
diff --git a/karpenter-provider-ibm-cloud_amd/csrc/queue_kernels.hpp b/karpenter-provider-ibm-cloud_amd/csrc/queue_kernels.hpp
--- a/karpenter-provider-ibm-cloud_amd/csrc/queue_kernels.hpp
+++ b/karpenter-provider-ibm-cloud_amd/csrc/queue_kernels.hpp
@@ -27,32 +27,3 @@
   c.w = (uint32_t)(ce >> 32);
   ((uint4*)const_cast<uint32_t*>(d.qcodes))[k] = c;
 }
-
-__device__ __forceinline__ bool queue_record_same(const DevProblem& d, uint32_t a, uint32_t b) {
-  const uint4* va = (const uint4*)(d.qvars + a);
-  const uint4* vb = (const uint4*)(d.qvars + b);
-  bool same = true;
-#pragma unroll
-  for (uint32_t q = 0; q < sizeof(VarRec) / 16; q++) {
-    const uint4 x = va[q], y = vb[q];
-    same = same && (q == 0 || x.x == y.x) && x.y == y.y && x.z == y.z && (q == sizeof(VarRec) / 16 - 1 || x.w == y.w);
-  }
-  for (uint32_t r = 0; r < d.R; r++) same = same && d.qreqs[(size_t)a * d.R + r] == d.qreqs[(size_t)b * d.R + r];
-  return same;
-}
-__global__ __launch_bounds__(256) void GS_KNAME(queue_runs_kernel)(GS_KPROBLEM_ARG) {
-  GS_KPROBLEM
-  GS_KPROBLEM_EXIT(blockIdx.x * 256 >= d.P)
-  __shared__ uint8_t s_same[256 + 16];
-  const uint32_t b0 = blockIdx.x * 256;
-  for (uint32_t t = threadIdx.x; t < 256 + 16; t += 256) {
-    const uint32_t x = b0 + t;
-    s_same[t] = x + 1 < d.P && queue_record_same(d, x, x + 1);
-  }
-  __syncthreads();
-  const uint32_t k = b0 + threadIdx.x;
-  if (k >= d.P) return;
-  uint32_t n = 1;
-  while (n < 16 && s_same[threadIdx.x + n - 1]) n++;
-  const_cast<uint32_t*>(d.qrun)[k] = n;
-}
```
